# davnords/octic-vits

Measured on AMD Instinct MI355X. Metric: images/sec Hybrid Octic ViT-H/14 224² bf16 train step @1/2/4/8 MI355X, higher is better.
Workload: dtype bf16; 1 GPU; hybrid_deit_huge_patch14 (16 octic + 16 standard blocks, drop_path 0.5) DeiT-III train step: bf16-autocast fwd + bwd + LAMB + EMA, 224x224, batch 64/GPU (BASELINE configs[1]), data parallel over 1 GPU(s); global_batch=64, per_gpu_batch=64, accum_steps=1, parallelism=dp1, library_gemm_table=True, launch=hipGraph replay (whole step)

## Files before the change

### include/octic_hip.h

```cpp
#ifndef OCTIC_HIP_H
#define OCTIC_HIP_H

#include <stdint.h>

#ifdef __cplusplus
extern "C" {
#endif

#define OCTIC_ABI_VERSION 20

enum { OCTIC_F32 = 0, OCTIC_BF16 = 1, OCTIC_U8 = 2  };

enum {
  OCTIC_OK = 0,
  OCTIC_ESHAPE = -1,
  OCTIC_EALIGN = -2,
  OCTIC_EDTYPE = -3,
  OCTIC_ENULL = -4,
  OCTIC_EWORKSPACE = -5
};

typedef struct {
  void* ptr[5];
  int64_t ld[5];
// ... 154 lines not shown
int octic_attn_fwd_packed(const void* qkv, void* o, float* lse, int64_t B, int H, int T, int c, int64_t ld_qkv,
                          int64_t ld_o, float scale, void* stream);
int octic_attn_bwd_packed(const void* qkv, const void* o, const void* dout, const float* lse, float* delta, void* dqkv,
                          int64_t B, int H, int T, int c, int64_t ld_qkv, int64_t ld_o, int64_t ld_g, float scale,
                          int phase, void* stream);

enum {
  OCTIC_ATTN_FWD_PERSIST = 0,
  OCTIC_ATTN_FWD_A80_ONESHOT = 1,
  OCTIC_ATTN_FWD_A80_ONLINE = 2,
  OCTIC_ATTN_FWD_RESIDENT = 3,
  OCTIC_ATTN_FWD_STREAM = 4,
  OCTIC_ATTN_FWD_F32 = 5
};
enum {
  OCTIC_ATTN_BWD_SINGLE = 0,
  OCTIC_ATTN_BWD_PAIR = 1,
  OCTIC_ATTN_BWD_STREAM = 2,
  OCTIC_ATTN_BWD_F32 = 3
};
int octic_attn_plan(int dtype, int T, int hd, int64_t ld_in, int64_t ld_out, int64_t ld_grad, int out[4]);
int octic_attn_skip_plan(int dtype, int T, int hd, int64_t ld_in, int64_t ld_out, int64_t ld_grad, int out[4]);

int octic_attn_fwd_skip(const void* q, const void* k, const void* v, void* o, float* lse, int64_t B, int H, int T, int hd,
                        int64_t sB, int64_t sH, int64_t sT, int64_t oB, int64_t oH, int64_t oT, float scale,
                        const float* sample_scale, void* stream);
int octic_attn_bwd_skip(const void* q, const void* k, const void* v, const void* o, const void* dout, const float* lse,
                        float* delta, void* dq, void* dk, void* dv, int64_t B, int H, int T, int hd, int64_t sB, int64_t sH,
                        int64_t sT, int64_t oB, int64_t oH, int64_t oT, int64_t gB, int64_t gH, int64_t gT, float scale,
                        int phase, const float* sample_scale, void* stream);
int octic_attn_fwd_packed_skip(const void* qkv, void* o, float* lse, int64_t B, int H, int T, int c, int64_t ld_qkv,
                               int64_t ld_o, float scale, const float* sample_scale, void* stream);
int octic_attn_bwd_packed_skip(const void* qkv, const void* o, const void* dout, const float* lse, float* delta, void* dqkv,
                               int64_t B, int H, int T, int c, int64_t ld_qkv, int64_t ld_o, int64_t ld_g, float scale,
                               int phase, const float* sample_scale, void* stream);

int octic_handoff_cat_fwd(const octic_view* x, void* dense, int64_t M, int c, int out_dtype, void* stream);
int octic_handoff_cat_bwd(const float* ddense, const octic_view* dx, int64_t M, int c, void* stream);
int octic_power_spectrum_fwd(const octic_view* x, void* dense, int64_t M, int c, int out_dtype, void* stream);
int octic_power_spectrum_bwd(const float* ddense, const octic_view* x, const octic_view* dx, int64_t M, int c,
                             void* stream);

int octic_im2col_patches(const float* img, void* patches, int64_t B, int Cin, int Himg, int Wimg, int p,
                         int Kpad, int dtype, void* stream);
int octic_lift_gemm(const void* patches, const void* w, const float* bias, const float* pos, float* out,
                    int64_t B, int64_t n_patches, int tok0, int Kpad, int D, int dtype, void* stream);
int64_t octic_lift_wgrad_workspace_bytes(int Kpad, int D, int splits);
int octic_lift_wgrad(const void* patches, const void* dout, float* dw, float* workspace, int splits, int64_t rows,
                     int Kpad, int D, int dtype, void* stream);

int64_t octic_lamb_workspace_floats(int ntensors, int nchunks);
int octic_lamb_step(void* const* p, void* const* g, void* const* m, void* const* v, void* const* ema, const float* wd,
                    const int* chunk_tensor, const int64_t* chunk_off, const int* chunk_len,
                    const int* tensor_chunk_begin, int ntensors, int nchunks, float* workspace, float lr, float beta1,
                    float beta2, float eps, float max_grad_norm, int step, float ema_decay, void* const* bf16_shadow,
                    void* stream);
int octic_adamw_step(void* const* p, void* const* g, void* const* m, void* const* v, void* const* ema, const float* wd,
                     const int* chunk_tensor, const int64_t* chunk_off, const int* chunk_len,
                     const int* tensor_chunk_begin, int ntensors, int nchunks, float* workspace, float lr, float beta1,
                     float beta2, float eps, float max_grad_norm, int step, float ema_decay, void* const* bf16_shadow,
                     void* stream);
int octic_lamb_step_hp(void* const* p, void* const* g, void* const* m, void* const* v, void* const* ema, const float* wd,
                       const int* chunk_tensor, const int64_t* chunk_off, const int* chunk_len,
                       const int* tensor_chunk_begin, int ntensors, int nchunks, float* workspace, const float* lr,
                       float beta1, float beta2, float eps, float max_grad_norm, int step, const float* ema_decay,
                       void* const* bf16_shadow, void* stream);
int octic_adamw_step_hp(void* const* p, void* const* g, void* const* m, void* const* v, void* const* ema, const float* wd,
                        const int* chunk_tensor, const int64_t* chunk_off, const int* chunk_len,
                        const int* tensor_chunk_begin, int ntensors, int nchunks, float* workspace, const float* lr,
                        float beta1, float beta2, float eps, float max_grad_norm, int step, const float* ema_decay,
                        void* const* bf16_shadow, void* stream);

int octic_dense_blocks(int64_t rows);
int octic_dense_resid_layernorm_fwd(const float* x, const void* yb, int yb_dtype, const float* gamma, const float* rs,
                                    int64_t rows_per_scale, float* xout, void* y, int y_dtype, const float* w,
                                    const float* b, float* stats, int64_t rows, int d, float eps, void* stream);
int octic_dense_layernorm_fwd(const float* x, void* y, int y_dtype, const float* w, const float* b, float* stats,
                              int64_t rows, int d, float eps, void* stream);
int octic_dense_layernorm_bwd(const void* gy, int g_dtype, const float* x, const float* w, const float* stats,
                              const float* dres, float* dx, float* partials, int64_t rows, int d, void* stream);
int octic_dense_finish(const float* partials, int nblocks, int d, float* out0, float* out1, const float* scale1,
                       void* stream);
typedef struct octic_finish_job {
  const float* partials;
  float* out0;
  float* out1;
  const float* scale1;
  int nblocks;
  int d;
} octic_finish_job;
int octic_dense_finish_batch(const octic_finish_job* jobs, int njobs, void* stream);
int octic_dense_layernorm_bwd_tail(const void* gy, const float* x, const float* w, const float* stats, const float* dres,
                                   float* dx, float* partials, const void* yb, const float* gamma, const float* rs,
                                   int64_t rows_per_scale, void* gyb, float* partials2, int64_t rows, int d, void* stream);
int octic_dense_layernorm_bwd_tail_skip(const void* gy, const float* x, const float* w, const float* stats,
                                        const float* dres, float* dx, float* partials, const void* yb, const float* gamma,
                                        const float* rs, int64_t rows_per_scale, void* gyb, float* partials2, int64_t rows,
                                        int d, const float* sample_scale, int64_t rows_per_sample, void* stream);
int octic_dense_gelu_blocks(void);
int octic_dense_gelu_bwd(const void* h, const void* g, void* dh, float* partials, int64_t rows, int d, void* stream);
int octic_dense_colsum(const void* g, int64_t rows, int d, int64_t ld, float* partials, void* stream);
int octic_dense_colsum_skip(const void* g, int64_t rows, int d, int64_t ld, float* partials, const float* sample_scale,
                            int64_t rows_per_sample, void* stream);
int octic_swiglu_blocks(void);
int octic_swiglu_fwd(const void* x12, int64_t ld12, void* a, int64_t lda, int64_t rows, int H, void* stream);
int octic_swiglu_bwd(const void* x12, int64_t ld12, const void* ga, int64_t ldg, void* dx12, int64_t ldd, float* partials,
                     int64_t rows, int H, void* stream);
int octic_scale_residual_fwd(const float* x, const void* y, int y_dtype, const float* gamma, const float* rs,
                             int64_t rows_per_scale, float* out, int64_t rows, int d, void* stream);
int octic_scale_residual_bwd(const float* gout, const void* y, int y_dtype, const float* gamma, const float* rs,
                             int64_t rows_per_scale, void* gy, float* partials, int64_t rows, int d, void* stream);

int octic_dense_layernorm_fwd_rows(const float* x, void* y, int y_dtype, const float* w, const float* b, float* stats,
                                   int64_t rows, int d, float eps, const int* rowmap, float* xcopy, void* stream);
int octic_dense_layernorm_bwd_rows(const void* gy, int g_dtype, const float* x, const float* w, const float* stats,
                                   const float* dres, float* dx, float* partials, int64_t rows, int d, const int* rowmap,
                                   void* stream);
int octic_scale_residual_fwd_rows(const float* x, const void* y, int y_dtype, const float* gamma, const float* rs,
                                  int64_t rows_per_scale, float* out, int64_t rows, int d, const int* rowmap, void* stream);
int octic_scale_residual_bwd_rows(const float* gout, const void* y, int y_dtype, const float* gamma, const float* rs,
                                  int64_t rows_per_scale, void* gy, float* partials, int64_t rows, int d, const int* rowmap,
                                  void* stream);

typedef struct octic_dense_prep_item {
  const void* src;
  void* wb;
  void* wt;
  int32_t N, K;
  int32_t block_begin, pad;
} octic_dense_prep_item;
int octic_dense_prep_batch_blocks(int N, int K);
int octic_dense_prep_batch(const octic_dense_prep_item* items_dev, int n_items, int total_blocks, int src_dtype, void* stream);

int64_t octic_dense_gemm_workspace_bytes(int M, int N, int K);
int octic_dense_gemm_colsum_rows(int M, int N, int K);
int octic_dense_gemm_tile(int M, int N, int K, int mode);
int octic_dense_gemm_nt(const void* A, const void* B, int M, int N, int K, int64_t lda, int64_t ldb, int mode, void* C,
                        void* C2, int64_t ldc, const float* bias, const float* gamma, const float* rs,
                        int64_t rows_per_sample, const float* X, float* OUT, const void* H, float* colsum,
                        void* workspace, void* stream);
int octic_dense_gemm_nt_tokens(const void* A, const void* B, int M, int N, int K, int64_t lda, int64_t ldb, int mode, void* C,
                               void* C2, int64_t ldc, const float* bias, const float* gamma, const float* rs,
                               int64_t rows_per_sample, const float* X, float* OUT, const void* H, float* colsum,
                               void* workspace, int tokens, void* stream);
int octic_dense_gemm_plan(int M, int N, int K, int mode, int tokens, int* out4);
int octic_dense_gemm_nt_tokens_skip(const void* A, const void* B, int M, int N, int K, int64_t lda, int64_t ldb, int mode, void* C,
                                    void* C2, int64_t ldc, const float* bias, const float* gamma, const float* rs,
                                    int64_t rows_per_sample_rs, const float* X, float* OUT, const void* H, float* colsum,
                                    const float* sample_scale, int rows_per_sample, void* workspace, int tokens,
                                    void* stream);
int octic_dense_gemm_plan_dropped(int M, int N, int K, int mode, int tokens, int rows_per_sample, int* out4);
int octic_dense_gemm_order_dropped(int M, int N, int K, int mode, int tokens, const float* sample_scale, int rows_per_sample,
                                   int cap, int* out_tm, int* out_tn, int* out_part, int* out_split, int* out_dead);

int64_t octic_dense_wgrad_workspace_bytes(int M, int N, int K);
int octic_dense_wgrad_tile(int M, int N, int K);
int octic_dense_wgrad_plan(int M, int N0, int N1, int K, int64_t ld_max, int out[4]);
int octic_dense_wgrad_tn(const void* dY, const void* X, int M, int N, int K, int64_t ldy, int64_t ldx, float* dW,
                         void* workspace, void* stream);
int64_t octic_dense_wgrad_pair_workspace_bytes(int M, int N0, int N1, int K);
int octic_dense_wgrad_tn_pair(const void* dY0, const void* X0, int N0, int64_t ldy0, int64_t ldx0, float* dW0,
                              const void* dY1, const void* X1, int N1, int64_t ldy1, int64_t ldx1, float* dW1, int M, int K,
                              void* workspace, void* stream);
int octic_dense_wgrad_tn_skip(const void* dY, const void* X, int M, int N, int K, int64_t ldy, int64_t ldx, float* dW,
                              const float* sample_scale, int rows_per_sample, void* workspace, void* stream);
int octic_dense_wgrad_tn_pair_skip(const void* dY0, const void* X0, int N0, int64_t ldy0, int64_t ldx0, float* dW0,
                                   const void* dY1, const void* X1, int N1, int64_t ldy1, int64_t ldx1, float* dW1, int M, int K,
                                   const float* sample_scale, int rows_per_sample, void* workspace, void* stream);

int octic_softmax_center(const void* t, int t_dtype, int64_t ldt, const float* center, float inv_temp, float* out,
                         int64_t rows, int K, void* stream);
int octic_soft_ce_fwd(const void* s, int s_dtype, int64_t lds, const float* tprob, int64_t t_rows, float inv_temp,
                      float* loss, float* lse, float* tsum, int64_t rows, int K, void* stream);
int octic_soft_ce_bwd(const void* s, int s_dtype, int64_t lds, const float* tprob, int64_t t_rows, float inv_temp,
                      const float* g, const float* lse, const float* tsum, void* ds, int64_t ldd, int64_t rows, int K,
                      void* stream);

typedef struct {
  float* w;
  float* b;
  float* mw;
  float* mb;
  int32_t col0;
  int32_t K;
  int32_t lr_index;
  int32_t tile0;
} octic_probe_head;
int octic_probe_features(const void* const* cls, const int64_t* cls_ld, int n, const void* patch, int64_t patch_ld_b,
                         int64_t patch_ld_t, int dtype, int64_t B, int P, int D, float* F, int64_t ldf, void* stream);
int octic_probe_forward(const octic_probe_head* heads, int nheads, const float* F, int64_t ldf, int B, int C, float* logits,
                        void* stream);
int octic_probe_ce(const float* logits, const int64_t* labels, int nheads, int B, int C, float* dlogits, float* rowloss,
                   int* rowrank, float* loss_mean, float* loss_sum, int* topk, void* stream);
int octic_probe_sgd(const octic_probe_head* heads, int nheads, int total_ktiles, const float* F, int64_t ldf,
                    const float* dlogits, int B, int C, const float* lr, float momentum, void* stream);

int octic_seg_ldd(int C);
int octic_seg_slabs(int64_t N, int D, int C);
int64_t octic_seg_workspace_bytes(int64_t N, int D, int C);
int octic_seg_value_dlogits(const float* X, int64_t ldx, int64_t N, int D, const float* W, const float* b, int C,
                            const int32_t* y, float* dlogits, double* value, void* workspace, void* stream);
int octic_seg_predict(const float* X, int64_t ldx, int64_t N, int D, const float* W, const float* b, int C, int32_t* pred,
                      void* stream);
int octic_seg_wgrad(const float* X, int64_t ldx, int64_t N, int D, const float* dlogits, int C, const float* W, double scale,
                    double lambda, float* dW, float* db, void* workspace, void* stream);
int64_t octic_seg_colstats_workspace_bytes(int64_t N, int D);
int octic_seg_colstats(const float* X, int64_t ldx, int64_t N, int D, double* mean, double* var, void* workspace, void* stream);
int octic_seg_standardize(float* X, int64_t ldx, int64_t N, int D, const double* mean, const double* scale, void* stream);
int octic_seg_patch_mode(const void* labels, int esize, int64_t R, int L, int32_t* mode, void* stream);
int octic_seg_confusion(const void* labels, int esize, int64_t R, int L, const int32_t* pred, const uint8_t* ignore,
                        int64_t* counts, void* stream);

int octic_seg_knn_plan(int64_t n, int64_t M, int D, int kmax, int metrics, int* out);
int64_t octic_seg_knn_workspace_bytes(int64_t n, int64_t M, int D, int kmax, int metrics, int splits);
int octic_seg_rownorms(const float* X, int64_t ldx, int64_t N, int D, float* norms, void* stream);
int octic_seg_knn(const float* Q, int64_t ldq, int64_t n, const float* K, int64_t ldk, int64_t M, int D, const float* qnorm,
                  const float* knorm, const uint8_t* skip, int kmax, int metrics, int splits, int32_t* idx_l2, float* dist_l2,
                  int32_t* idx_cos, float* dist_cos, int64_t ldo, void* workspace, void* stream);
int octic_seg_knn_vote(const int32_t* idx, int64_t ldi, int64_t n, const void* labels, int esize, int64_t R, int L, const int* ks,
                       int nk, uint8_t* out, void* stream);

#define OCTIC_KNN_KMAX 256
int octic_knn_topk_plan(int64_t n, int64_t M, int D, int kmax, int* out);
int64_t octic_knn_topk_workspace_bytes(int64_t n, int64_t M, int D, int kmax, int splits);
int octic_knn_topk(const float* Q, int64_t ldq, int64_t n, const float* K, int64_t ldk, int64_t M, int D, int kmax, int splits,
                   int32_t* idx, float* sim, int64_t ldo, void* workspace, void* stream);
int octic_knn_vote(const float* sim, const int32_t* idx, int64_t ldi, int64_t n, int kmax, const int64_t* labels, int64_t M,
                   int C, float inv_T, const int* ks, int nk, float* probas, const int64_t* targets, int64_t* counters,
                   void* stream);

typedef struct {
  int32_t partner;
  float lam;
  int32_t cut;
  int32_t yl, yh;
  int32_t xl, xh;
  int32_t pad;
} octic_mix_row;
int octic_mix_images(const float* src, float* dst, const octic_mix_row* table, int B, int C, int H, int W, void* stream);
int octic_mix_targets(const int64_t* labels, const octic_mix_row* table, int B, int row0, int rows, int num_classes, float on,
                      float off, int binarize, float* targets, void* stream);
int octic_mix_bce(const void* logits, int dtype, int64_t ldl, const int64_t* labels, const octic_mix_row* table, int B, int row0,
                  int rows, int num_classes, float on, float off, int binarize, float* loss, const float* gscale,
                  void* dlogits, int64_t ldd, void* workspace, void* stream);

typedef struct {
  int32_t flip;
  int32_t op;
  int32_t blur_r, blur_ww, blur_fw;
  int32_t order[4];
  float brightness, contrast, saturation;
  int32_t pad[4];
} octic_aug_row;
int64_t octic_augment_workspace_bytes(int B, int H, int W);
int octic_augment_u8(const uint8_t* src, void* dst, int dtype_out, const octic_aug_row* table, float mean0, float mean1,
                     float mean2, float std0, float std1, float std2, int B, int H, int W, void* workspace, void* stream);

typedef struct {
  int64_t src_offset;
  int32_t src_h, src_w;
  int32_t top, left, h, w;
  int32_t flip;
  int32_t hcoef, htaps, vcoef, vtaps;
  int32_t order[4];
  float brightness, contrast, saturation;
  int32_t hue_shift;
  int32_t gray, blur, solarize;
  float blur_w[9];
  int32_t pad[7];
} octic_dino_row;
int octic_dino_resize_coeffs(int n, int S, int taps, int32_t* bounds, int32_t* k);
int octic_dino_resize_max_taps(int S);
int octic_dino_resize_u8(const uint8_t* data, int64_t data_bytes, const octic_dino_row* rows, const int32_t* coef,
                         int64_t coef_len, int N, int S, uint8_t* crops, void* stream);
int64_t octic_dino_color_workspace_bytes(int N, int H, int W);
int octic_dino_color_u8(const uint8_t* crops, void* dst, int dtype_out, const octic_dino_row* rows, float mean0, float mean1,
                        float mean2, float std0, float std1, float std2, int N, int H, int W, void* workspace, void* stream);

#ifdef __cplusplus
}
#endif
#endif
```

### octic_vits_amd/_lib.py

```python
import ctypes
import os
import re

HERE = os.path.dirname(os.path.abspath(__file__))
LIB_PATH = os.environ.get("OCTIC_LIB") or os.path.join(HERE, "liboctic_hip.so")
HEADER_PATH = os.path.join(HERE, "..", "include", "octic_hip.h")

F32, BF16, U8 = 0, 1, 2
ABI_VERSION = 20
(ROUTE_DENSE_TILE, ROUTE_DENSE_SPLIT, ROUTE_WGRAD_SLABS, ROUTE_WGRAD_TILE, ROUTE_LINEAR_RING, ROUTE_RING_EVEN,
 ROUTE_ATTN_LEGACY, ROUTE_ATTN_ONLINE, ROUTE_ATTN_BWD_PAIR, ROUTE_DENSE_IMAGE, ROUTE_DENSE_CLS2, ROUTE_ATTN_STREAM) = range(12)

(ATTN_FWD_PERSIST, ATTN_FWD_A80_ONESHOT, ATTN_FWD_A80_ONLINE, ATTN_FWD_RESIDENT, ATTN_FWD_STREAM, ATTN_FWD_F32) = range(6)
ATTN_BWD_SINGLE, ATTN_BWD_PAIR, ATTN_BWD_STREAM, ATTN_BWD_F32 = range(4)
LINEAR_WREG, LINEAR_RING, LINEAR_CLASSIC = range(3)
WGRAD_RING, WGRAD_TILED = range(2)

c_i64, c_int, c_float, c_void_p = ctypes.c_int64, ctypes.c_int, ctypes.c_float, ctypes.c_void_p
c_double = ctypes.c_double


class OcticView(ctypes.Structure):
    _fields_ = [("ptr", c_void_p * 5), ("ld", c_i64 * 5)]


PtrArray5 = c_void_p * 5
VP = ctypes.POINTER(OcticView)

_PROTOS = {
    "octic_abi_version": (c_int, []),
    "octic_strerror": (ctypes.c_char_p, [c_int]),
    "octic_route_override": (c_int, [c_int, c_int]),
    "octic_gelu_d8_fwd": (c_int, [VP, VP, c_i64, c_int, c_int, c_void_p]),
    "octic_gelu_d8_bwd": (c_int, [VP, VP, VP, c_i64, c_int, c_int, c_void_p]),
    "octic_gelu_d8_fwd_skip": (c_int, [VP, VP, c_i64, c_int, c_int, c_void_p, c_i64, c_void_p]),
    "octic_gelu_d8_bwd_skip": (c_int, [VP, VP, VP, c_i64, c_int, c_int, c_void_p, c_i64, c_void_p]),
    "octic_layernorm_d8_fwd": (c_int, [VP, VP, c_void_p, c_void_p, c_void_p, c_i64, c_int, c_float, c_int, c_void_p]),
    "octic_layernorm_d8_bwd_blocks": (c_int, [c_i64]),
    "octic_layernorm_d8_bwd": (c_int, [VP, VP, c_void_p, c_void_p, VP, VP, c_void_p, c_i64, c_int, c_int, c_void_p]),
    "octic_layernorm_d8_bwd_cast": (c_int, [VP, VP, c_void_p, c_void_p, VP, VP, c_void_p, c_i64, c_int, c_void_p, c_i64,
                                            c_void_p, c_void_p]),
    "octic_layernorm_d8_bwd_skip": (c_int, [VP, VP, c_void_p, c_void_p, VP, VP, c_void_p, c_i64, c_int, c_int, c_void_p, c_i64,
                                            c_void_p]),
    "octic_layernorm_d8_bwd_cast_skip": (c_int, [VP, VP, c_void_p, c_void_p, VP, VP, c_void_p, c_i64, c_int, c_void_p, c_i64,
                                                 c_void_p, c_void_p, c_i64, c_void_p]),
    "octic_layernorm_d8_bwd_finish": (c_int, [c_void_p, c_int, c_int, c_void_p, c_void_p, c_void_p]),
    "octic_layernorm_d8_bwd_finish_batch": (c_int, [c_void_p, c_int, c_void_p]),
    "octic_sample_blocks": (c_int, [c_void_p, c_void_p, c_void_p, c_i64, c_i64, c_int, c_void_p]),
    "octic_linear_d8_fwd": (c_int, [VP, c_void_p, c_void_p, VP, VP, c_void_p, c_i64, c_void_p, c_i64, c_int, c_int,
                                    c_int, c_int, c_void_p]),
    "octic_linear_d8_fwd_skip": (c_int, [VP, c_void_p, c_void_p, VP, VP, c_void_p, c_i64, c_void_p, c_i64, c_int, c_int,
                                         c_int, c_int, c_void_p, c_i64, c_void_p]),
    "octic_linear_d8_fwd_dropped": (c_int, [VP, c_void_p, c_void_p, VP, VP, c_void_p, c_i64, c_void_p, c_i64, c_int, c_int,
                                            c_int, c_int, c_void_p, c_i64, c_void_p]),
    "octic_linear_d8_tile_n": (c_int, [c_i64, c_int, c_int]),
    "octic_linear_d8_plan": (c_int, [c_i64, c_int, c_int, c_int, c_int, c_int, ctypes.POINTER(c_int)]),
    "octic_linear_d8_ring_order": (c_int, [c_void_p, c_void_p, c_void_p, c_int, c_void_p, c_void_p]),
    "octic_linear_d8_ring_order_dropped": (c_int, [c_int, c_void_p, c_void_p, c_int, c_void_p, c_void_p, c_void_p, c_void_p,
                                                   c_void_p, c_void_p]),
    "octic_linear_d8_wgrad_tile": (c_int, [c_i64, c_int, c_int]),
    "octic_linear_d8_wgrad_workspace_bytes": (c_i64, [c_int, c_int, c_int]),
    "octic_linear_d8_wgrad_splits": (c_int, [c_i64, c_int, c_int]),
    "octic_linear_d8_wgrad": (c_int, [VP, VP, c_i64, c_int, c_int, c_int, c_void_p, c_int, c_void_p]),
    "octic_linear_d8_wgrad_finish": (c_int, [c_void_p, c_int, c_int, c_int, c_void_p, c_void_p, c_void_p, c_void_p,
                                             c_void_p, c_void_p, c_void_p, c_void_p]),
    "octic_linear_d8_wgrad_finish_batch": (c_int, [c_void_p, c_int, c_void_p]),
    "octic_linear_d8_wgrad_has_colsum": (c_int, [c_int, c_int, c_int]),
    "octic_linear_d8_wgrad_plan": (c_int, [c_i64, c_int, c_int, c_int, ctypes.POINTER(c_int)]),
    "octic_lamb_workspace_floats": (c_i64, [c_int, c_int]),
    "octic_lamb_step": (c_int, [c_void_p] * 10 + [c_int, c_int, c_void_p, c_float, c_float, c_float, c_float, c_float,
                                                  c_int, c_float, c_void_p, c_void_p]),
    "octic_adamw_step": (c_int, [c_void_p] * 10 + [c_int, c_int, c_void_p, c_float, c_float, c_float, c_float, c_float,
                                                   c_int, c_float, c_void_p, c_void_p]),
    "octic_lamb_step_hp": (c_int, [c_void_p] * 10 + [c_int, c_int, c_void_p, c_void_p, c_float, c_float, c_float, c_float,
                                                     c_int, c_void_p, c_void_p, c_void_p]),
    "octic_adamw_step_hp": (c_int, [c_void_p] * 10 + [c_int, c_int, c_void_p, c_void_p, c_float, c_float, c_float, c_float,
                                                      c_int, c_void_p, c_void_p, c_void_p]),
    "octic_dense_blocks": (c_int, [c_i64]),
    "octic_dense_layernorm_fwd": (c_int, [c_void_p, c_void_p, c_int, c_void_p, c_void_p, c_void_p, c_i64, c_int,
                                          c_float, c_void_p]),
    "octic_dense_resid_layernorm_fwd": (c_int, [c_void_p, c_void_p, c_int, c_void_p, c_void_p, c_i64, c_void_p, c_void_p, c_int,
                                                c_void_p, c_void_p, c_void_p, c_i64, c_int, c_float, c_void_p]),
    "octic_dense_layernorm_bwd": (c_int, [c_void_p, c_int, c_void_p, c_void_p, c_void_p, c_void_p, c_void_p, c_void_p,
                                          c_i64, c_int, c_void_p]),
    "octic_dense_layernorm_bwd_tail": (c_int, [c_void_p] * 10 + [c_i64, c_void_p, c_void_p, c_i64, c_int, c_void_p]),
    "octic_dense_layernorm_bwd_tail_skip": (c_int, [c_void_p] * 10 + [c_i64, c_void_p, c_void_p, c_i64, c_int, c_void_p, c_i64,
                                                                      c_void_p]),
    "octic_dense_finish": (c_int, [c_void_p, c_int, c_int, c_void_p, c_void_p, c_void_p, c_void_p]),
    "octic_dense_finish_batch": (c_int, [c_void_p, c_int, c_void_p]),
    "octic_dense_gelu_blocks": (c_int, []),
    "octic_dense_gelu_bwd": (c_int, [c_void_p, c_void_p, c_void_p, c_void_p, c_i64, c_int, c_void_p]),
    "octic_swiglu_blocks": (c_int, []),
    "octic_swiglu_fwd": (c_int, [c_void_p, c_i64, c_void_p, c_i64, c_i64, c_int, c_void_p]),
    "octic_swiglu_bwd": (c_int, [c_void_p, c_i64, c_void_p, c_i64, c_void_p, c_i64, c_void_p, c_i64, c_int, c_void_p]),
    "octic_dense_layernorm_fwd_rows": (c_int, [c_void_p, c_void_p, c_int, c_void_p, c_void_p, c_void_p, c_i64, c_int, c_float,
                                               c_void_p, c_void_p, c_void_p]),
    "octic_dense_layernorm_bwd_rows": (c_int, [c_void_p, c_int, c_void_p, c_void_p, c_void_p, c_void_p, c_void_p, c_void_p, c_i64,
                                               c_int, c_void_p, c_void_p]),
    "octic_scale_residual_fwd_rows": (c_int, [c_void_p, c_void_p, c_int, c_void_p, c_void_p, c_i64, c_void_p, c_i64, c_int,
                                              c_void_p, c_void_p]),
    "octic_scale_residual_bwd_rows": (c_int, [c_void_p, c_void_p, c_int, c_void_p, c_void_p, c_i64, c_void_p, c_void_p, c_i64,
                                              c_int, c_void_p, c_void_p]),
    "octic_softmax_center": (c_int, [c_void_p, c_int, c_i64, c_void_p, c_float, c_void_p, c_i64, c_int, c_void_p]),
    "octic_soft_ce_fwd": (c_int, [c_void_p, c_int, c_i64, c_void_p, c_i64, c_float, c_void_p, c_void_p, c_void_p, c_i64, c_int,
                                  c_void_p]),
    "octic_soft_ce_bwd": (c_int, [c_void_p, c_int, c_i64, c_void_p, c_i64, c_float, c_void_p, c_void_p, c_void_p, c_void_p, c_i64,
                                  c_i64, c_int, c_void_p]),
    "octic_scale_residual_fwd": (c_int, [c_void_p, c_void_p, c_int, c_void_p, c_void_p, c_i64, c_void_p, c_i64, c_int,
                                         c_void_p]),
    "octic_scale_residual_bwd": (c_int, [c_void_p, c_void_p, c_int, c_void_p, c_void_p, c_i64, c_void_p, c_void_p,
                                         c_i64, c_int, c_void_p]),
    "octic_colsum_blocks": (c_int, [c_i64]),
    "octic_colsum_a1": (c_int, [VP, c_i64, c_int, c_int, c_void_p, c_void_p, c_void_p]),
    "octic_cast_rowscale": (c_int, [VP, VP, c_void_p, c_i64, c_i64, c_int, c_int, c_void_p]),
    "octic_linear_d8_prep": (c_int, [c_void_p, c_void_p, c_int, c_int, c_void_p, c_void_p, c_int, c_void_p]),
    "octic_linear_d8_prep_batch_blocks": (c_int, [c_int, c_int]),
    "octic_linear_d8_prep_batch": (c_int, [c_void_p, c_int, c_int, c_int, c_void_p]),
    "octic_attn_fwd": (c_int, [c_void_p, c_void_p, c_void_p, c_void_p, c_void_p, c_i64, c_int, c_int, c_int,
                               c_i64, c_i64, c_i64, c_i64, c_i64, c_i64, c_float, c_void_p]),
    "octic_attn_fwd_packed": (c_int, [c_void_p] * 3 + [c_i64, c_int, c_int, c_int, c_i64, c_i64, c_float, c_void_p]),
    "octic_attn_bwd_packed": (c_int, [c_void_p] * 6 + [c_i64, c_int, c_int, c_int, c_i64, c_i64, c_i64, c_float, c_int, c_void_p]),
    "octic_attn_bwd": (c_int, [c_void_p] * 10 + [c_i64, c_int, c_int, c_int] + [c_i64] * 9 + [c_float, c_int, c_void_p]),
    "octic_attn_fwd_skip": (c_int, [c_void_p] * 5 + [c_i64, c_int, c_int, c_int] + [c_i64] * 6 + [c_float, c_void_p, c_void_p]),
    "octic_attn_bwd_skip": (c_int, [c_void_p] * 10 + [c_i64, c_int, c_int, c_int] + [c_i64] * 9 + [c_float, c_int, c_void_p, c_void_p]),
    "octic_attn_fwd_packed_skip": (c_int, [c_void_p] * 3 + [c_i64, c_int, c_int, c_int, c_i64, c_i64, c_float, c_void_p, c_void_p]),
    "octic_attn_bwd_packed_skip": (c_int, [c_void_p] * 6 + [c_i64, c_int, c_int, c_int, c_i64, c_i64, c_i64, c_float, c_int, c_void_p, c_void_p]),
    "octic_attn_fwd_f32": (c_int, [c_void_p] * 5 + [c_i64, c_int, c_int, c_int] + [c_i64] * 6 + [c_float, c_void_p]),
    "octic_attn_bwd_f32": (c_int, [c_void_p] * 10 + [c_i64, c_int, c_int, c_int] + [c_i64] * 9 + [c_float, c_int, c_void_p]),
    "octic_attn_plan": (c_int, [c_int, c_int, c_int, c_i64, c_i64, c_i64, ctypes.POINTER(c_int)]),
    "octic_attn_skip_plan": (c_int, [c_int, c_int, c_int, c_i64, c_i64, c_i64, ctypes.POINTER(c_int)]),
    "octic_attn_pack_heads": (c_int, [VP, c_void_p, c_i64, c_i64, c_int, c_int, c_int, c_int, c_void_p]),
    "octic_attn_unpack_heads": (c_int, [c_void_p, VP, c_i64, c_i64, c_int, c_int, c_int, c_int, c_void_p]),
    "octic_handoff_cat_fwd": (c_int, [VP, c_void_p, c_i64, c_int, c_int, c_void_p]),
    "octic_handoff_cat_bwd": (c_int, [c_void_p, VP, c_i64, c_int, c_void_p]),
    "octic_power_spectrum_fwd": (c_int, [VP, c_void_p, c_i64, c_int, c_int, c_void_p]),
    "octic_power_spectrum_bwd": (c_int, [c_void_p, VP, VP, c_i64, c_int, c_void_p]),
    "octic_im2col_patches": (c_int, [c_void_p, c_void_p, c_i64, c_int, c_int, c_int, c_int, c_int, c_int, c_void_p]),
    "octic_lift_gemm": (c_int, [c_void_p, c_void_p, c_void_p, c_void_p, c_void_p, c_i64, c_i64, c_int, c_int, c_int,
                                c_int, c_void_p]),
    "octic_lift_wgrad_workspace_bytes": (c_i64, [c_int, c_int, c_int]),
    "octic_lift_wgrad": (c_int, [c_void_p, c_void_p, c_void_p, c_void_p, c_int, c_i64, c_int, c_int, c_int, c_void_p]),
    "octic_dense_prep_batch_blocks": (c_int, [c_int, c_int]),
    "octic_dense_prep_batch": (c_int, [c_void_p, c_int, c_int, c_int, c_void_p]),
    "octic_dense_gemm_workspace_bytes": (c_i64, [c_int, c_int, c_int]),
    "octic_dense_gemm_colsum_rows": (c_int, [c_int, c_int, c_int]),
    "octic_dense_gemm_tile": (c_int, [c_int, c_int, c_int, c_int]),
    "octic_dense_gemm_nt": (c_int, [c_void_p, c_void_p, c_int, c_int, c_int, c_i64, c_i64, c_int, c_void_p, c_void_p, c_i64,
                                    c_void_p, c_void_p, c_void_p, c_i64, c_void_p, c_void_p, c_void_p, c_void_p, c_void_p,
                                    c_void_p]),
    "octic_dense_gemm_nt_tokens": (c_int, [c_void_p, c_void_p, c_int, c_int, c_int, c_i64, c_i64, c_int, c_void_p, c_void_p,
                                           c_i64, c_void_p, c_void_p, c_void_p, c_i64, c_void_p, c_void_p, c_void_p, c_void_p,
                                           c_void_p, c_int, c_void_p]),
    "octic_dense_gemm_plan": (c_int, [c_int, c_int, c_int, c_int, c_int, ctypes.POINTER(c_int)]),
    "octic_dense_gemm_nt_tokens_skip": (c_int, [c_void_p, c_void_p, c_int, c_int, c_int, c_i64, c_i64, c_int, c_void_p, c_void_p,
                                                c_i64, c_void_p, c_void_p, c_void_p, c_i64, c_void_p, c_void_p, c_void_p, c_void_p,
                                                c_void_p, c_int, c_void_p, c_int, c_void_p]),
    "octic_dense_gemm_plan_dropped": (c_int, [c_int, c_int, c_int, c_int, c_int, c_int, ctypes.POINTER(c_int)]),
    "octic_dense_gemm_order_dropped": (c_int, [c_int, c_int, c_int, c_int, c_int, c_void_p, c_int, c_int, c_void_p, c_void_p,
                                               c_void_p, c_void_p, c_void_p]),
    "octic_dense_colsum": (c_int, [c_void_p, c_i64, c_int, c_i64, c_void_p, c_void_p]),
    "octic_dense_colsum_skip": (c_int, [c_void_p, c_i64, c_int, c_i64, c_void_p, c_void_p, c_i64, c_void_p]),
    "octic_dense_wgrad_workspace_bytes": (c_i64, [c_int, c_int, c_int]),
    "octic_dense_wgrad_tile": (c_int, [c_int, c_int, c_int]),
    "octic_dense_wgrad_plan": (c_int, [c_int, c_int, c_int, c_int, c_i64, ctypes.POINTER(c_int)]),
    "octic_dense_wgrad_tn": (c_int, [c_void_p, c_void_p, c_int, c_int, c_int, c_i64, c_i64, c_void_p, c_void_p, c_void_p]),
    "octic_dense_wgrad_pair_workspace_bytes": (c_i64, [c_int, c_int, c_int, c_int]),
    "octic_dense_wgrad_tn_pair": (c_int, [c_void_p, c_void_p, c_int, c_i64, c_i64, c_void_p, c_void_p, c_void_p, c_int, c_i64, c_i64,
                                          c_void_p, c_int, c_int, c_void_p, c_void_p]),
    "octic_dense_wgrad_tn_skip": (c_int, [c_void_p, c_void_p, c_int, c_int, c_int, c_i64, c_i64, c_void_p, c_void_p, c_int, c_void_p,
                                          c_void_p]),
    "octic_dense_wgrad_tn_pair_skip": (c_int, [c_void_p, c_void_p, c_int, c_i64, c_i64, c_void_p, c_void_p, c_void_p, c_int, c_i64,
                                               c_i64, c_void_p, c_int, c_int, c_void_p, c_int, c_void_p, c_void_p]),
    "octic_probe_features": (c_int, [c_void_p, c_void_p, c_int, c_void_p, c_i64, c_i64, c_int, c_i64, c_int, c_int, c_void_p,
                                     c_i64, c_void_p]),
    "octic_probe_forward": (c_int, [c_void_p, c_int, c_void_p, c_i64, c_int, c_int, c_void_p, c_void_p]),
    "octic_probe_ce": (c_int, [c_void_p, c_void_p, c_int, c_int, c_int, c_void_p, c_void_p, c_void_p, c_void_p, c_void_p,
                               c_void_p, c_void_p]),
    "octic_probe_sgd": (c_int, [c_void_p, c_int, c_int, c_void_p, c_i64, c_void_p, c_int, c_int, c_void_p, c_float, c_void_p]),
    "octic_seg_ldd": (c_int, [c_int]),
    "octic_seg_slabs": (c_int, [c_i64, c_int, c_int]),
    "octic_seg_workspace_bytes": (c_i64, [c_i64, c_int, c_int]),
    "octic_seg_value_dlogits": (c_int, [c_void_p, c_i64, c_i64, c_int, c_void_p, c_void_p, c_int, c_void_p, c_void_p, c_void_p,
                                        c_void_p, c_void_p]),
    "octic_seg_predict": (c_int, [c_void_p, c_i64, c_i64, c_int, c_void_p, c_void_p, c_int, c_void_p, c_void_p]),
    "octic_seg_wgrad": (c_int, [c_void_p, c_i64, c_i64, c_int, c_void_p, c_int, c_void_p, c_double, c_double, c_void_p, c_void_p,
                                c_void_p, c_void_p]),
    "octic_seg_colstats_workspace_bytes": (c_i64, [c_i64, c_int]),
    "octic_seg_colstats": (c_int, [c_void_p, c_i64, c_i64, c_int, c_void_p, c_void_p, c_void_p, c_void_p]),
    "octic_seg_standardize": (c_int, [c_void_p, c_i64, c_i64, c_int, c_void_p, c_void_p, c_void_p]),
    "octic_seg_patch_mode": (c_int, [c_void_p, c_int, c_i64, c_int, c_void_p, c_void_p]),
    "octic_seg_confusion": (c_int, [c_void_p, c_int, c_i64, c_int, c_void_p, c_void_p, c_void_p, c_void_p]),
    "octic_seg_knn_plan": (c_int, [c_i64, c_i64, c_int, c_int, c_int, ctypes.POINTER(c_int)]),
    "octic_seg_knn_workspace_bytes": (c_i64, [c_i64, c_i64, c_int, c_int, c_int, c_int]),
    "octic_seg_rownorms": (c_int, [c_void_p, c_i64, c_i64, c_int, c_void_p, c_void_p]),
    "octic_seg_knn": (c_int, [c_void_p, c_i64, c_i64, c_void_p, c_i64, c_i64, c_int, c_void_p, c_void_p, c_void_p, c_int, c_int,
                              c_int, c_void_p, c_void_p, c_void_p, c_void_p, c_i64, c_void_p, c_void_p]),
    "octic_seg_knn_vote": (c_int, [c_void_p, c_i64, c_i64, c_void_p, c_int, c_i64, c_int, ctypes.POINTER(c_int), c_int, c_void_p,
                                   c_void_p]),
    "octic_knn_topk_plan": (c_int, [c_i64, c_i64, c_int, c_int, ctypes.POINTER(c_int)]),
    "octic_knn_topk_workspace_bytes": (c_i64, [c_i64, c_i64, c_int, c_int, c_int]),
    "octic_knn_topk": (c_int, [c_void_p, c_i64, c_i64, c_void_p, c_i64, c_i64, c_int, c_int, c_int, c_void_p, c_void_p, c_i64,
                               c_void_p, c_void_p]),
    "octic_knn_vote": (c_int, [c_void_p, c_void_p, c_i64, c_i64, c_int, c_void_p, c_i64, c_int, c_float, ctypes.POINTER(c_int),
                               c_int, c_void_p, c_void_p, c_void_p, c_void_p]),
    "octic_mix_images": (c_int, [c_void_p, c_void_p, c_void_p, c_int, c_int, c_int, c_int, c_void_p]),
    "octic_mix_targets": (c_int, [c_void_p, c_void_p, c_int, c_int, c_int, c_int, c_float, c_float, c_int, c_void_p, c_void_p]),
    "octic_mix_bce": (c_int, [c_void_p, c_int, c_i64, c_void_p, c_void_p, c_int, c_int, c_int, c_int, c_float, c_float, c_int,
                              c_void_p, c_void_p, c_void_p, c_i64, c_void_p, c_void_p]),
    "octic_augment_workspace_bytes": (c_i64, [c_int, c_int, c_int]),
    "octic_augment_u8": (c_int, [c_void_p, c_void_p, c_int, c_void_p] + [c_float] * 6 + [c_int, c_int, c_int, c_void_p, c_void_p]),
    "octic_dino_resize_coeffs": (c_int, [c_int, c_int, c_int, c_void_p, c_void_p]),
    "octic_dino_resize_max_taps": (c_int, [c_int]),
    "octic_dino_resize_u8": (c_int, [c_void_p, c_i64, c_void_p, c_void_p, c_i64, c_int, c_int, c_void_p, c_void_p]),
    "octic_dino_color_workspace_bytes": (c_i64, [c_int, c_int, c_int]),
    "octic_dino_color_u8": (c_int, [c_void_p, c_void_p, c_int, c_void_p] + [c_float] * 6 + [c_int, c_int, c_int, c_void_p, c_void_p]),
}


def header_symbols():
    with open(HEADER_PATH) as f:
        text = re.sub(r"/\*.*?\*/", "", f.read(), flags=re.S)
    return sorted(set(re.findall(r"\b(octic_[a-z0-9_]+)\s*\(", text)))


_LIB = None


def lib():
    global _LIB
    if _LIB is None:
        if not os.path.exists(LIB_PATH):
            raise RuntimeError(
                f"octic_vits_amd: HIP library {LIB_PATH} is missing. Build it with "
                "`python -m octic_vits_amd.build` (hipcc, --offload-arch=gfx950). There is no CPU fallback.")
        L = ctypes.CDLL(LIB_PATH)
        for name, (res, args) in _PROTOS.items():
            fn = getattr(L, name)
            fn.restype, fn.argtypes = res, args
        if L.octic_abi_version() != ABI_VERSION:
            raise RuntimeError("octic_vits_amd: ABI version mismatch between _lib.py and liboctic_hip.so")
        _LIB = L
    return _LIB


def route_override(knob: int, value: int) -> int:
    old = lib().octic_route_override(knob, value)
    if old < 0:
        raise ValueError(f"octic_route_override: unknown knob {knob}")
    _PLANS.clear()
    for drop in _ON_OVERRIDE:
        drop()
    return old


_ON_OVERRIDE = []


def on_route_override(drop):
    if drop not in _ON_OVERRIDE:
        _ON_OVERRIDE.append(drop)
    return drop


_PLANS = {}


def plan(query, *args):
    key = (query, args)
    answer = _PLANS.get(key, 0)
    if answer == 0:
        out = (c_int * 4)()
        code = getattr(lib(), query)(*args, out)
        if code not in (0, -1):
            check(code)
        _PLANS[key] = answer = tuple(out) if code == 0 else None
    return answer


def attn_plan(T, hd, dtype=BF16, ld_in=0, ld_out=0, ld_grad=0):
    answer = plan("octic_attn_plan", dtype, T, hd, ld_in, ld_out, ld_grad)
    if answer is None:
        check(-1)
    return answer


def check(code: int):
    if code != 0:
        raise RuntimeError(f"octic HIP call failed ({code}): {lib().octic_strerror(code).decode()}")
```

### octic_vits_amd/csrc/dense_gemm.hip

```cpp
#include <cmath>
#include <type_traits>
#include "octic_common.hpp"

namespace octic {

constexpr int DG_BM = 256, DG_BK = 64;
constexpr int DG_UNIT = 128 * 128;
constexpr int DG_SLOTS = 8;
constexpr int DG_D = 6;
static_assert(DG_D >= 4 && DG_D <= DG_SLOTS - 2, "prefetch distance");
template <int NT> struct DgGeom {
  static constexpr int NA = NT - 2;
  static constexpr int BN = 64 * NT;
  static constexpr int WCOLS = 16 * NT;
  static constexpr int U1 = NA * 8192;
  static constexpr int KT = 3 * DG_UNIT + U1;
  static constexpr int RING = 2 * KT;
  static constexpr int SRS = WCOLS * 2 + 16;
  static constexpr int EPI_PASSES = NT == 4 ? 1 : 2;
  static constexpr int EPI_ROWS = 128 / EPI_PASSES;
  static constexpr int EPI = 8 * EPI_ROWS * SRS;
  static constexpr int LDS = RING > EPI ? RING : EPI;
  static constexpr int INFLIGHT = 2 * (DG_D - 2) + (NA - 2);
  static_assert(DG_D == 6 || NT == 4, "unequal units: the steady vmcnt assumes the 4 youngest units are one of each kind");
  __host__ __device__ static constexpr int unit_off(int kind) { return kind == 0 ? 0 : kind == 1 ? DG_UNIT : kind == 2 ? DG_UNIT + U1 : 2 * DG_UNIT + U1; }
  __host__ __device__ static constexpr int unit_instr(int kind) { return kind == 1 ? NA : 2; }
};

struct DgArgs {
  const bf16* A;
  const bf16* B;
  int64_t lda, ldb;
  int M, N, K;
  bf16* C;
  bf16* C2;
  int64_t ldc;
  const float* bias;
  const float* gamma;
  const float* rs;
  int64_t rps;
  const float* X;
  float* OUT;
  const bf16* H;
  float* colsum;
  int m_stride, m_base;
  int tiles_m, tiles_n;
  int full_tiles;
  int split;
  int tail_pad;
  float* slabs;
  int* tickets;
  const float* sample_scale;
  int rows_per_sample;
};

enum DgMode { DG_PLAIN = 0, DG_GELU = 1, DG_RESID = 2, DG_DGELU = 3,
              DG_GELUF = 4,
              DG_DFACT = 5,
              DG_GELUO = 6 };

constexpr int kDgMaskCap = 1024;
constexpr int kDgMaskWords = kDgMaskCap / 64;

__host__ __device__ inline bool dg_panel_live(const float* scale, int rps, int M, int m_stride, int m_base, int tm) {
  const int m0 = tm * m_stride + m_base;
  if (m0 >= M) return false;
  const int m1 = (m0 + DG_BM < M ? m0 + DG_BM : M) - 1;
  const int b1 = m1 / rps;
  for (int b = m0 / rps; b <= b1; ++b)
    if (scale[b] != 0.0f) return true;
  return false;
}
__host__ __device__ inline int dg_group_bits(const unsigned long long* bm, int g, int gsz, bool live) {
  int b = (int)((bm[g >> 3] >> ((g & 7) * 8)) & 0xffull);
  if (!live) b = ~b;
  return b & ((1 << gsz) - 1);
}
__host__ __device__ inline int dg_group_count(int bits, int gsz, int tiles_n, int cut) {
  if (cut == gsz * tiles_n) return tiles_n * __builtin_popcount(bits);
  const int cols = cut / gsz, rest = cut - cols * gsz;
  return cols * __builtin_popcount(bits) + __builtin_popcount(bits & ((1 << rest) - 1));
}
__host__ __device__ inline int dg_live_full(const unsigned long long* bm, int tiles_m, int tiles_n, int full) {
  const int per_group = 8 * tiles_n;
  int L = 0;
  for (int g = 0; g * per_group < full; ++g) {
    const int gsz = tiles_m - 8 * g < 8 ? tiles_m - 8 * g : 8;
    const int left = full - g * per_group, cut = left < gsz * tiles_n ? left : gsz * tiles_n;
    L += dg_group_count(dg_group_bits(bm, g, gsz, true), gsz, tiles_n, cut);
  }
  return L;
}
__host__ __device__ inline int dg_select_full(const unsigned long long* bm, int tiles_m, int tiles_n, int full, int k, bool live) {
  const int per_group = 8 * tiles_n;
  for (int g = 0; g * per_group < full; ++g) {
    const int gsz = tiles_m - 8 * g < 8 ? tiles_m - 8 * g : 8;
    const int left = full - g * per_group, cut = left < gsz * tiles_n ? left : gsz * tiles_n;
    int bits = dg_group_bits(bm, g, gsz, live);
    const int cnt = dg_group_count(bits, gsz, tiles_n, cut);
    if (k < cnt) {
      const int lg = __builtin_popcount(bits);
      const int col = k / lg;
      int idx = k - col * lg, pos = 0;
      for (; pos < 8; ++pos) {
        if (bits & 1) {
          if (idx == 0) break;
          --idx;
        }
        bits >>= 1;
      }
      return g * per_group + col * gsz + pos;
    }
    k -= cnt;
  }
  return 0;
}
__host__ __device__ inline void dg_tile_panel(int tiles_m, int tiles_n, int tile, int& tm, int& tn) {
  const int per_group = 8 * tiles_n, gidx = tile / per_group, first_m = gidx * 8;
  const int gsz = (tiles_m - first_m) < 8 ? (tiles_m - first_m) : 8;
  const int in_g = tile - gidx * per_group;
  tm = first_m + in_g % gsz;
  tn = in_g / gsz;
}
__host__ __device__ inline void dense_item_masked(int tiles_m, int tiles_n, int full, int split, int tail_pad, int bid,
                                                  const unsigned long long* bm, int& tile, int& rem_idx, int& part, bool& dead) {
  tile = -1; rem_idx = -1; part = 0; dead = false;
  if (bid < tail_pad) {
    if (bid >= (tiles_m * tiles_n - full) * split) return;
    rem_idx = bid / split;
    part = bid - rem_idx * split;
    tile = full + rem_idx;
    int tm, tn;
    dg_tile_panel(tiles_m, tiles_n, tile, tm, tn);
    dead = ((bm[tm >> 6] >> (tm & 63)) & 1ull) == 0;
    return;
  }
  const int j = bid - tail_pad;
  const int L = dg_live_full(bm, tiles_m, tiles_n, full), D = full - L;
  if (j < D) {
    tile = dg_select_full(bm, tiles_m, tiles_n, full, j, false);
    dead = true;
    return;
  }
  const int i = j - D, x = i & 7, q8 = L >> 3, r8 = L & 7;
  const int rank = (x < r8 ? x * (q8 + 1) : r8 * (q8 + 1) + (x - r8) * q8) + (i >> 3);
  tile = dg_select_full(bm, tiles_m, tiles_n, full, rank, true);
}

__device__ inline void dg_wait_vmcnt(int n) {
  switch (n) {
    case 2: asm volatile("s_waitcnt vmcnt(2)" ::: "memory"); break;
    case 4: asm volatile("s_waitcnt vmcnt(4)" ::: "memory"); break;
    case 6: asm volatile("s_waitcnt vmcnt(6)" ::: "memory"); break;
    case 8: asm volatile("s_waitcnt vmcnt(8)" ::: "memory"); break;
    case 10: asm volatile("s_waitcnt vmcnt(10)" ::: "memory"); break;
    case 12: asm volatile("s_waitcnt vmcnt(12)" ::: "memory"); break;
    case 14: asm volatile("s_waitcnt vmcnt(14)" ::: "memory"); break;
    case 16: asm volatile("s_waitcnt vmcnt(16)" ::: "memory"); break;
    case 3: asm volatile("s_waitcnt vmcnt(3)" ::: "memory"); break;
    case 5: asm volatile("s_waitcnt vmcnt(5)" ::: "memory"); break;
    case 7: asm volatile("s_waitcnt vmcnt(7)" ::: "memory"); break;
    case 9: asm volatile("s_waitcnt vmcnt(9)" ::: "memory"); break;
    default: asm volatile("s_waitcnt vmcnt(0)" ::: "memory"); break;
  }
}

#ifdef DG_TRACE
__device__ unsigned long long g_dg_trace[8 * 256];
extern "C" void* octic_dbg_dense_trace(void) {
  void* p = nullptr;
  (void)hipGetSymbolAddress(&p, HIP_SYMBOL(g_dg_trace));
  return p;
}
#define DGT()                                                                                        \
  do {                                                                                               \
    if (blockIdx.x == 0 && lane == 0 && dgt_i < 256) g_dg_trace[wid * 256 + dgt_i++] = __builtin_readcyclecounter(); \
    if (blockIdx.x == 0 && lane == 0 && dgt_i == 200) g_dg_trace[wid * 256 + 255] = __builtin_amdgcn_s_memrealtime(); \
  } while (0)
#else
#define DGT() do {} while (0)
#endif
#ifdef DG_TRACE2
__device__ unsigned long long g_dg_trace2[4096 * 8];
extern "C" void* octic_dbg_dense_trace2(void) {
  void* p = nullptr;
  (void)hipGetSymbolAddress(&p, HIP_SYMBOL(g_dg_trace2));
  return p;
}
#define DGT2(slot)                                                                                            \
  do {                                                                                                        \
    if (wid == 0 && lane == 0 && blockIdx.x < 4096) g_dg_trace2[blockIdx.x * 8 + (slot)] = __builtin_amdgcn_s_memrealtime(); \
  } while (0)
#else
#define DGT2(slot) do {} while (0)
#endif

__device__ inline float dg_erf(float x) {
  const float ax = fabsf(x);
  const float t = __builtin_amdgcn_rcpf(1.0f + 0.3275911f * ax);
  const float poly = t * (0.254829592f + t * (-0.284496736f + t * (1.421413741f + t * (-1.453152027f + t * 1.061405429f))));
  const float r = 1.0f - poly * __expf(-ax * ax);
  return copysignf(r, x);
}
__device__ inline float dg_gelu(float x) { return 0.5f * x * (1.0f + dg_erf(x * kSqrt1Over2)); }
__device__ inline float dg_gelu_grad(float x) {
  return 0.5f * (1.0f + dg_erf(x * kSqrt1Over2)) + x * kInvSqrt2Pi * __expf(-0.5f * x * x);
}
__device__ inline void dg_gelu_both(float x, float& g, float& d) {
  const float ax = fabsf(x) * kSqrt1Over2;
  const float t = __builtin_amdgcn_rcpf(1.0f + 0.3275911f * ax);
  const float poly = t * (0.254829592f + t * (-0.284496736f + t * (1.421413741f + t * (-1.453152027f + t * 1.061405429f))));
  const float e = __expf(-ax * ax);
  const float phi = 0.5f * (1.0f + copysignf(1.0f - poly * e, x));
  g = x * phi;
  d = phi + x * kInvSqrt2Pi * e;
}

template <int N>
__device__ inline void dg_wait_imm() {
  if constexpr (N == 8) asm volatile("s_waitcnt vmcnt(8)" ::: "memory");
  else if constexpr (N == 10) asm volatile("s_waitcnt vmcnt(10)" ::: "memory");
  else if constexpr (N == 12) asm volatile("s_waitcnt vmcnt(12)" ::: "memory");
  else if constexpr (N == 14) asm volatile("s_waitcnt vmcnt(14)" ::: "memory");
  else if constexpr (N == 16) asm volatile("s_waitcnt vmcnt(16)" ::: "memory");
  else if constexpr (N == 6) asm volatile("s_waitcnt vmcnt(6)" ::: "memory");
  else if constexpr (N == 9) asm volatile("s_waitcnt vmcnt(9)" ::: "memory");
  else asm volatile("s_waitcnt vmcnt(0)" ::: "memory");
}

template <int MODE, int NT, bool SKIP = false>
__global__ __launch_bounds__(512, 1) void dense_nt_kernel(DgArgs a) {
  extern __shared__ __attribute__((aligned(16))) char lds[];
  using GE = DgGeom<NT>;
  constexpr int NA = GE::NA, DG_BN = GE::BN;
  static_assert(NT == 4 || MODE == DG_PLAIN, "the fused tails exist for the 256-wide tile only");
  static_assert(!SKIP || MODE != DG_RESID, "the fused residual tail never takes a mask");

  const int lane = threadIdx.x & 63;
  const int wid = __builtin_amdgcn_readfirstlane(threadIdx.x >> 6);
  const int wr = wid >> 2, wc = wid & 3;
  const bool hi = wr != 0;
  const int fr = lane & 15, kg = lane >> 4;
#ifdef DG_TRACE
  int dgt_i = 0;
  if (blockIdx.x == 0 && lane == 0) g_dg_trace[wid * 256 + 254] = __builtin_amdgcn_s_memrealtime();
#endif
  DGT();
  DGT2(0);
#ifdef DG_TRACE2
  if (wid == 0 && lane == 0 && blockIdx.x < 4096) {
    unsigned xcc, hwid;
    asm volatile("s_getreg_b32 %0, hwreg(HW_REG_XCC_ID)" : "=s"(xcc));
    asm volatile("s_getreg_b32 %0, hwreg(HW_REG_HW_ID)" : "=s"(hwid));
    g_dg_trace2[blockIdx.x * 8 + 7] = ((unsigned long long)hwid << 32) | xcc;
  }
#endif

  const int bid = blockIdx.x;
  int tile, kt_begin, kt_end, part = 0, rem_idx = -1;
  const int nkt_all = a.K / DG_BK;
  bool dead_item = false;
  if constexpr (SKIP) {
    unsigned long long* const live_bm = (unsigned long long*)(lds + GE::LDS);
    const int words = (a.tiles_m + 63) >> 6;
    for (int w = wid; w < words; w += 8) {
      const int p = w * 64 + lane;
      const bool live = p < a.tiles_m && dg_panel_live(a.sample_scale, a.rows_per_sample, a.M, a.m_stride, a.m_base, p);
      const unsigned long long m = __ballot(live);
      if (lane == 0) live_bm[w] = m;
    }
    __syncthreads();
    dense_item_masked(a.tiles_m, a.tiles_n, a.full_tiles, a.split, a.tail_pad, bid, live_bm, tile, rem_idx, part, dead_item);
    tile = __builtin_amdgcn_readfirstlane(tile);
    rem_idx = __builtin_amdgcn_readfirstlane(rem_idx);
    part = __builtin_amdgcn_readfirstlane(part);
    dead_item = __builtin_amdgcn_readfirstlane((int)dead_item) != 0;
    if (tile < 0) return;
    kt_begin = rem_idx >= 0 ? (int)(((int64_t)nkt_all * part) / a.split) : 0;
    kt_end = rem_idx >= 0 ? (int)(((int64_t)nkt_all * (part + 1)) / a.split) : nkt_all;
  } else
  if (bid >= a.tail_pad) {
    const int j = bid - a.tail_pad;
    const int nf = a.full_tiles;
    const int xcd = j & 7, q8 = nf >> 3, r8 = nf & 7;
    tile = (xcd < r8 ? xcd * (q8 + 1) : r8 * (q8 + 1) + (xcd - r8) * q8) + (j >> 3);
    kt_begin = 0;
    kt_end = nkt_all;
  } else {
    const int r = bid;
    if (r >= (a.tiles_m * a.tiles_n - a.full_tiles) * a.split) return;
    rem_idx = r / a.split;
    part = r - rem_idx * a.split;
    tile = a.full_tiles + rem_idx;
    kt_begin = (int)(((int64_t)nkt_all * part) / a.split);
    kt_end = (int)(((int64_t)nkt_all * (part + 1)) / a.split);
  }
  int tm, tn;
  {
    const int G = 8;
    const int per_group = G * a.tiles_n;
    const int gidx = tile / per_group;
    const int first_m = gidx * G;
    const int gsz = (a.tiles_m - first_m) < G ? (a.tiles_m - first_m) : G;
    const int in_g = tile - gidx * per_group;
    tm = first_m + in_g % gsz;
    tn = in_g / gsz;
  }
  const int m0 = tm * a.m_stride + a.m_base, n0 = tn * DG_BN;
  if constexpr (SKIP) {
    if (dead_item) {
      if (part != 0) return;
      constexpr int CPR = DG_BN / 8;
      const u32x4 z = {0, 0, 0, 0};
#pragma unroll 4
      for (int p = threadIdx.x; p < DG_BM * CPR; p += 512) {
        const int r = p / CPR, c = p - r * CPR;
        const int m = m0 + r, n = n0 + c * 8;
        if (m < a.M && n < a.N) {
          *(u32x4*)(a.C + (int64_t)m * a.ldc + n) = z;
          if (MODE == DG_GELU || MODE == DG_GELUF) *(u32x4*)(a.C2 + (int64_t)m * a.ldc + n) = z;
        }
      }
      if ((MODE == DG_DGELU || MODE == DG_DFACT) && a.colsum != nullptr) {
        const int t = threadIdx.x;
        const int row = t / (DG_BN / 4), n = n0 + (t - row * (DG_BN / 4)) * 4;
        if (row < 2 && n < a.N) *(f32x4*)(a.colsum + (int64_t)(tm * 2 + row) * a.N + n) = f32x4{0, 0, 0, 0};
      }
      return;
    }
  }
  const int nkt = kt_end - kt_begin;
  const int nunits = 4 * nkt;

  const int drow = lane >> 3;
  const int dch = (lane & 7) ^ drow;
  const __amdgpu_buffer_rsrc_t rsA = __builtin_amdgcn_make_buffer_rsrc((void*)a.A, 0, (int)((int64_t)a.M * a.lda * 2), 0x27000);
  const __amdgpu_buffer_rsrc_t rsB = __builtin_amdgcn_make_buffer_rsrc((void*)a.B, 0, (int)((int64_t)a.N * a.ldb * 2), 0x27000);
  const int r0 = 16 * wid + drow;
  const int am0 = m0, an0 = n0;
  const unsigned voA = (unsigned)(((int64_t)(am0 + (r0 >> 6) * 128 + (r0 & 63)) * a.lda + dch * 8) * 2);
  const int rb1 = 8 * NA * wid + drow;
  const unsigned voB1 = (unsigned)(((int64_t)(an0 + (rb1 / (16 * NA)) * GE::WCOLS + (rb1 % (16 * NA))) * a.ldb + dch * 8) * 2);
  const unsigned voB2 = (unsigned)(((int64_t)(an0 + (r0 >> 5) * GE::WCOLS + 16 * NA + (r0 & 31)) * a.ldb + dch * 8) * 2);
  const int rowA8 = (int)(a.lda * 16), rowB8 = (int)(a.ldb * 16);
  const int halfA = (int)(a.lda * 128);
  const int kbase = kt_begin * (DG_BK * 2);

  int u_issue = 0;
  auto issue_unit = [&](auto kind_c) {
    constexpr int KIND = decltype(kind_c)::value;
    constexpr bool isA = KIND == 0 || KIND == 3;
    char* dst = lds + ((u_issue >> 2) & 1) * GE::KT + GE::unit_off(KIND) + wid * (GE::unit_instr(KIND) * 1024);
    const int so = kbase + (u_issue >> 2) * (DG_BK * 2) + (KIND == 3 ? halfA : 0);
    if constexpr (isA) {
      __builtin_amdgcn_raw_ptr_buffer_load_lds(rsA, (__attribute__((address_space(3))) void*)dst, 16, voA, so, 0, 0);
      __builtin_amdgcn_raw_ptr_buffer_load_lds(rsA, (__attribute__((address_space(3))) void*)(dst + 1024), 16, voA, so + rowA8, 0, 0);
    } else if constexpr (KIND == 1) {
      __builtin_amdgcn_raw_ptr_buffer_load_lds(rsB, (__attribute__((address_space(3))) void*)dst, 16, voB1, so, 0, 0);
      __builtin_amdgcn_raw_ptr_buffer_load_lds(rsB, (__attribute__((address_space(3))) void*)(dst + 1024), 16, voB1, so + rowB8, 0, 0);
      if constexpr (NA == 3)
        __builtin_amdgcn_raw_ptr_buffer_load_lds(rsB, (__attribute__((address_space(3))) void*)(dst + 2048), 16, voB1, so + 2 * rowB8, 0, 0);
    } else {
      __builtin_amdgcn_raw_ptr_buffer_load_lds(rsB, (__attribute__((address_space(3))) void*)dst, 16, voB2, so, 0, 0);
      __builtin_amdgcn_raw_ptr_buffer_load_lds(rsB, (__attribute__((address_space(3))) void*)(dst + 1024), 16, voB2, so + rowB8, 0, 0);
    }
    ++u_issue;
  };
  auto young_instr = [&](int n) {
    const int k1 = ((u_issue + 2) >> 2) - ((u_issue - n + 2) >> 2);
    return 2 * n + (NA - 2) * k1;
  };
#define DG_IC(v) std::integral_constant<int, v>()

  const int sw = lane & 7;
  const int rdo0 = fr * 128 + ((kg ^ sw) << 4);
  const int rdo1 = fr * 128 + (((4 + kg) ^ sw) << 4);
  const int a_row0 = wr * 64;

  bf16x8 Af[1][2][4];
  bf16x8 Bf0[2][NA], Bf1[2][2];
  f32x4 acc0[2][4][NA], acc1[2][4][2];
#pragma unroll
  for (int i = 0; i < 2; ++i)
#pragma unroll
    for (int p = 0; p < 4; ++p) {
#pragma unroll
      for (int q = 0; q < NA; ++q) acc0[i][p][q] = f32x4{0, 0, 0, 0};
#pragma unroll
      for (int q = 0; q < 2; ++q) acc1[i][p][q] = f32x4{0, 0, 0, 0};
    }
  int rt_hi = (a.M - m0 - wr * 128 + 15) >> 4;
  rt_hi = rt_hi < 0 ? 0 : (rt_hi > 8 ? 8 : rt_hi);
  const int live_mask = __builtin_amdgcn_readfirstlane((rt_hi > 0 ? 1 : 0) | (rt_hi > 4 ? 2 : 0));

  auto readA = [&](int mh, int unit) {
    const char* base = lds + ((unit >> 2) & 1) * GE::KT + GE::unit_off(mh ? 3 : 0) + a_row0 * 128;
#pragma unroll
    for (int mi = 0; mi < 4; ++mi) {
      Af[0][0][mi] = *(const bf16x8*)(base + mi * 2048 + rdo0);
      Af[0][1][mi] = *(const bf16x8*)(base + mi * 2048 + rdo1);
    }
  };
  auto readB = [&](int nh, int unit) {
    if (nh == 0) {
      const char* base = lds + ((unit >> 2) & 1) * GE::KT + GE::unit_off(1) + wc * (16 * NA) * 128;
#pragma unroll
      for (int ni = 0; ni < NA; ++ni) {
        Bf0[0][ni] = *(const bf16x8*)(base + ni * 2048 + rdo0);
        Bf0[1][ni] = *(const bf16x8*)(base + ni * 2048 + rdo1);
      }
    } else {
      const char* base = lds + ((unit >> 2) & 1) * GE::KT + GE::unit_off(2) + wc * 32 * 128;
#pragma unroll
      for (int ni = 0; ni < 2; ++ni) {
        Bf1[0][ni] = *(const bf16x8*)(base + ni * 2048 + rdo0);
        Bf1[1][ni] = *(const bf16x8*)(base + ni * 2048 + rdo1);
      }
    }
  };
  auto mma = [&](int mh, int nh, auto kind_c) {
    asm volatile("s_waitcnt lgkmcnt(0)" ::: "memory");
    __builtin_amdgcn_sched_barrier(0);
    if (live_mask & (mh ? 2 : 1)) {
#pragma unroll
    for (int ks = 0; ks < 2; ++ks) {
#pragma unroll
      for (int mi = 0; mi < 4; ++mi) {
        if (nh == 0) {
#pragma unroll
          for (int ni = 0; ni < NA; ++ni)
            acc0[mh][mi][ni] = __builtin_amdgcn_mfma_f32_16x16x32_bf16(Bf0[ks][ni], Af[0][ks][mi], acc0[mh][mi][ni], 0, 0, 0);
        } else {
#pragma unroll
          for (int ni = 0; ni < 2; ++ni)
            acc1[mh][mi][ni] = __builtin_amdgcn_mfma_f32_16x16x32_bf16(Bf1[ks][ni], Af[0][ks][mi], acc1[mh][mi][ni], 0, 0, 0);
        }
      }
    }
    }
    __builtin_amdgcn_sched_barrier(0);
  };

  int g = 0;
  auto wait_landed = [&]() {
    int need = g + 2;
    need = need < nunits - 1 ? need : nunits - 1;
    const int ok = (u_issue - 1) - need;
    if (ok == DG_D - 2) dg_wait_imm<GE::INFLIGHT>();
    else dg_wait_vmcnt(ok > 0 ? young_instr(ok) : 0);
  };

#define DG_PRO(i) if constexpr ((i) < DG_D) { if (u_issue < nunits) issue_unit(DG_IC((i) & 3)); }
  DG_PRO(0) DG_PRO(1) DG_PRO(2) DG_PRO(3) DG_PRO(4) DG_PRO(5) DG_PRO(6) DG_PRO(7) DG_PRO(8) DG_PRO(9)
#undef DG_PRO
  {
    const int ok = (u_issue - 1) - 1;
    dg_wait_vmcnt(ok > 0 ? young_instr(ok) : 0);
  }
  if (hi) __builtin_amdgcn_s_barrier();
  DGT2(1);

  auto ktile = [&](int t, auto steady_c) {
    constexpr bool STEADY = decltype(steady_c)::value != 0;
    const int u0 = 4 * t;
    auto dma = [&](auto kind_c) {
      if (STEADY || u_issue < nunits) issue_unit(kind_c);
    };
    auto landed = [&]() {
      if constexpr (STEADY) dg_wait_imm<GE::INFLIGHT>();
      else wait_landed();
    };
#define DG_RP(x) do { __builtin_amdgcn_s_setprio(x); } while (0)
#define DG_R(q, reads) do { DG_RP(2); dma(DG_IC(((q) + DG_D) & 3)); reads; DG_RP(0); } while (0)
    __builtin_amdgcn_s_barrier();
    DGT();
    DG_R(0, readA(0, u0); readB(0, u0 + 1));
    if (hi) landed();
    DGT();
    __builtin_amdgcn_s_barrier();
    DGT();
    mma(0, 0, DG_IC((0 + DG_D) & 3));
    DGT();
    if (!hi) landed();
    ++g;
    __builtin_amdgcn_s_barrier();
    DGT();
    DG_R(1, readB(1, u0 + 2));
    if (hi) landed();
    DGT();
    __builtin_amdgcn_s_barrier();
    DGT();
    mma(0, 1, DG_IC((1 + DG_D) & 3));
    DGT();
    if (!hi) landed();
    ++g;
    __builtin_amdgcn_s_barrier();
    DGT();
    DG_R(2, readA(1, u0 + 3));
    if (hi) landed();
    DGT();
    __builtin_amdgcn_s_barrier();
    DGT();
    mma(1, 1, DG_IC((2 + DG_D) & 3));
    DGT();
    if (!hi) landed();
    ++g;
    __builtin_amdgcn_s_barrier();
    DGT();
    DG_R(3, (void)0);
    if (hi) landed();
    DGT();
    __builtin_amdgcn_s_barrier();
    DGT();
    mma(1, 0, DG_IC((3 + DG_D) & 3));
    DGT();
    if (!hi) landed();
    ++g;
#undef DG_R
#undef DG_RP
  };
  const int t_steady = (nunits - 4 - DG_D) >= 0 ? (nunits - 4 - DG_D) / 4 + 1 : 0;
  int t = 0;
#pragma unroll 1
  for (; t < t_steady; ++t) ktile(t, DG_IC(1));
#pragma unroll 1
  for (; t < nkt; ++t) ktile(t, DG_IC(0));
  if (!hi) __builtin_amdgcn_s_barrier();
  __builtin_amdgcn_s_barrier();
  DGT2(2);

  const int rt_lo = 0;
  auto ACC = [&](int mh, int mi, int j) -> f32x4& { return j < NA ? acc0[mh][mi][j] : acc1[mh][mi][j - NA]; };
  if (rem_idx >= 0 && a.split > 1) {
    float* slab = a.slabs + ((int64_t)rem_idx * a.split + part) * (DG_BM * DG_BN);
    f32x4* sw4 = (f32x4*)slab + (int64_t)wid * (8 * NT) * 64 + lane;
#pragma unroll
    for (int mh = 0; mh < 2; ++mh)
#pragma unroll
      for (int mi = 0; mi < 4; ++mi) {
        if (mh * 4 + mi >= rt_hi) continue;
#pragma unroll
        for (int j = 0; j < NT; ++j) sw4[((mh * 4 + mi) * NT + j) * 64] = ACC(mh, mi, j);
      }
    asm volatile("s_waitcnt vmcnt(0)" ::: "memory");
    __syncthreads();
    DGT2(5);
    int* flag = (int*)lds;
    if (threadIdx.x == 0) {
      __builtin_amdgcn_fence(__ATOMIC_RELEASE, "agent");
      asm volatile("s_waitcnt vmcnt(0)" ::: "memory");
      const int old = __hip_atomic_fetch_add(a.tickets + rem_idx, 1, __ATOMIC_RELAXED, __HIP_MEMORY_SCOPE_AGENT);
      flag[0] = (old == a.split - 1) ? 1 : 0;
      if (old == a.split - 1) {
        __builtin_amdgcn_fence(__ATOMIC_ACQUIRE, "agent");
        asm volatile("s_waitcnt vmcnt(0)" ::: "memory");
        __hip_atomic_store(a.tickets + rem_idx, 0, __ATOMIC_RELAXED, __HIP_MEMORY_SCOPE_AGENT);
      }
    }
    __syncthreads();
    const int last = flag[0];
    __syncthreads();
    if (last == 0) return;
    DGT2(6);
    for (int p = 0; p < a.split; ++p) {
      const f32x4* o4 = (const f32x4*)(a.slabs + ((int64_t)rem_idx * a.split + p) * (DG_BM * DG_BN)) +
                        (int64_t)wid * (8 * NT) * 64 + lane;
#pragma unroll
      for (int mh = 0; mh < 2; ++mh)
#pragma unroll
        for (int mi = 0; mi < 4; ++mi) {
          if (mh * 4 + mi >= rt_hi) continue;
#pragma unroll
          for (int j = 0; j < NT; ++j) {
            const f32x4 o = o4[((mh * 4 + mi) * NT + j) * 64];
            ACC(mh, mi, j) = p == 0 ? o : ACC(mh, mi, j) + o;
          }
        }
    }
  }

  if constexpr (NT != 4) {
    constexpr int SRS = GE::SRS;
    char* const stg = lds + wid * (GE::EPI_ROWS * SRS);
    const int er = lane / 10, ech = lane - er * 10;
    const int n = n0 + wc * GE::WCOLS + ech * 8;
    const bool nok = n < a.N && lane < 60;
#pragma unroll
    for (int mh = 0; mh < 2; ++mh) {
      if (mh * 4 >= rt_hi) break;
#pragma unroll
      for (int j = 0; j < NT; ++j) {
        const int nl = j * 16 + kg * 4;
        const int nb = n0 + wc * GE::WCOLS + nl;
        f32x4 bv = {0, 0, 0, 0};
        if (a.bias && nb < a.N) bv = *(const f32x4*)(a.bias + nb);
#pragma unroll
        for (int mi = 0; mi < 4; ++mi) {
          if (mh * 4 + mi >= rt_hi) continue;
          const f32x4 v = ACC(mh, mi, j) + bv;
          const bf16x4 cb = {(bf16)v[0], (bf16)v[1], (bf16)v[2], (bf16)v[3]};
          *(bf16x4*)(stg + (mi * 16 + fr) * SRS + nl * 2) = cb;
        }
      }
      asm volatile("s_waitcnt lgkmcnt(0)" ::: "memory");
#pragma unroll
      for (int it = 0; it < 11; ++it) {
        const int row = it * 6 + er;
        const int m = m0 + wr * 128 + mh * 64 + row;
        if (row >= 64 || m >= a.M || !nok || mh * 4 + (row >> 4) >= rt_hi) continue;
        const u32x4 raw = *(const u32x4*)(stg + row * SRS + ech * 16);
        *(u32x4*)(a.C + (int64_t)m * a.ldc + n) = raw;
      }
    }
  } else {
  constexpr int SRS = GE::SRS;
  char* const stg = lds + wid * (128 * SRS);
#pragma unroll
  for (int j = 0; j < NT; ++j) {
      const int nl = j * 16 + kg * 4;
      const int n = n0 + wc * 64 + nl;
      f32x4 bv = {0, 0, 0, 0};
      if (a.bias && n < a.N) bv = *(const f32x4*)(a.bias + n);
#pragma unroll
      for (int mh = 0; mh < 2; ++mh)
#pragma unroll
        for (int mi = 0; mi < 4; ++mi) {
          if (mh * 4 + mi < rt_lo || mh * 4 + mi >= rt_hi) continue;
          const f32x4 v = ACC(mh, mi, j) + bv;
          const bf16x4 cb = {(bf16)v[0], (bf16)v[1], (bf16)v[2], (bf16)v[3]};
          *(bf16x4*)(stg + (mh * 64 + mi * 16 + fr) * SRS + nl * 2) = cb;
        }
    }
  asm volatile("s_waitcnt lgkmcnt(0)" ::: "memory");
  const int srow = lane >> 3, sch = lane & 7;
  const int n = n0 + wc * 64 + sch * 8;
  const bool nok = n < a.N;
  f32x4 gm0 = {1, 1, 1, 1}, gm1 = {1, 1, 1, 1};
  if (MODE == DG_RESID && a.gamma && nok) {
    gm0 = *(const f32x4*)(a.gamma + n);
    gm1 = *(const f32x4*)(a.gamma + n + 4);
  }
  f32x4 xin[MODE == DG_RESID ? 16 : 1][2];
  bf16x8 hin[(MODE == DG_DGELU || MODE == DG_DFACT) ? 16 : 1];
  float csum[8] = {0, 0, 0, 0, 0, 0, 0, 0};
  if (MODE == DG_RESID || MODE == DG_DGELU || MODE == DG_DFACT) {
#pragma unroll
    for (int it = 0; it < 16; ++it) {
      const int m = m0 + wr * 128 + it * 8 + srow;
      const bool ok = m < a.M && nok && (it >> 1) >= rt_lo && (it >> 1) < rt_hi;
      if (MODE == DG_RESID) {
        const float* xp = a.X + (int64_t)(ok ? m : 0) * a.N + (ok ? n : 0);
        xin[it][0] = *(const f32x4*)xp;
        xin[it][1] = *(const f32x4*)(xp + 4);
      } else {
        hin[it] = *(const bf16x8*)(a.H + (int64_t)(ok ? m : 0) * a.ldc + (ok ? n : 0));
      }
    }
  }
#pragma unroll
  for (int it = 0; it < 16; ++it) {
    const int row = it * 8 + srow;
    const int m = m0 + wr * 128 + row;
    if (m >= a.M || !nok || (it >> 1) < rt_lo || (it >> 1) >= rt_hi) continue;
    const u32x4 raw = *(const u32x4*)(stg + row * SRS + sch * 16);
    const bf16x8 cb = __builtin_bit_cast(bf16x8, raw);
    bf16* cp = a.C + (int64_t)m * a.ldc + n;
    if (MODE == DG_PLAIN) {
      *(u32x4*)cp = raw;
    } else if (MODE == DG_GELU) {
      *(u32x4*)cp = raw;
      bf16x8 y;
#pragma unroll
      for (int e = 0; e < 8; ++e) y[e] = (bf16)dg_gelu((float)cb[e]);
      *(bf16x8*)(a.C2 + (int64_t)m * a.ldc + n) = y;
    } else if (MODE == DG_GELUO) {
      bf16x8 y;
#pragma unroll
      for (int e = 0; e < 8; ++e) y[e] = (bf16)dg_gelu((float)cb[e]);
      *(bf16x8*)cp = y;
    } else if (MODE == DG_GELUF) {
      bf16x8 y, f;
#pragma unroll
      for (int e = 0; e < 8; ++e) {
        float gv, dv;
        dg_gelu_both((float)cb[e], gv, dv);
        y[e] = (bf16)gv;
        f[e] = (bf16)dv;
      }
      *(bf16x8*)cp = f;
      *(bf16x8*)(a.C2 + (int64_t)m * a.ldc + n) = y;
    } else if (MODE == DG_RESID) {
      *(u32x4*)cp = raw;
      const float rsv = a.rs ? a.rs[m / a.rps] : 1.0f;
      f32x4 x0 = xin[it][0], x1 = xin[it][1];
#pragma unroll
      for (int e = 0; e < 4; ++e) {
        x0[e] += rsv * gm0[e] * (float)cb[e];
        x1[e] += rsv * gm1[e] * (float)cb[4 + e];
      }
      float* op = a.OUT + (int64_t)m * a.N + n;
      *(f32x4*)op = x0;
      *(f32x4*)(op + 4) = x1;
    } else {
      const bf16x8 h = hin[it];
      bf16x8 d;
#pragma unroll
      for (int e = 0; e < 8; ++e) {
        d[e] = (bf16)((MODE == DG_DFACT ? (float)h[e] : dg_gelu_grad((float)h[e])) * (float)cb[e]);
        csum[e] += (float)d[e];
      }
      *(bf16x8*)cp = d;
    }
  }
  if ((MODE == DG_DGELU || MODE == DG_DFACT) && a.colsum != nullptr) {
#pragma unroll
    for (int e = 0; e < 8; ++e) {
      float v = csum[e];
      v += __shfl_xor(v, 8, 64);
      v += __shfl_xor(v, 16, 64);
      v += __shfl_xor(v, 32, 64);
      csum[e] = v;
    }
    if (srow == 0 && nok) {
      float* base = a.colsum + (int64_t)(tm * 2 + wr) * a.N + n;
      *(f32x4*)base = f32x4{csum[0], csum[1], csum[2], csum[3]};
      *(f32x4*)(base + 4) = f32x4{csum[4], csum[5], csum[6], csum[7]};
    }
  }
  }
#ifdef DG_TRACE2
  DGT2(3);
  asm volatile("s_waitcnt vmcnt(0)" ::: "memory");
  DGT2(4);
#endif
}

template <int MODE>
__global__ __launch_bounds__(1024) void dense_cls_kernel(DgArgs a, int tokens, int nrows, int colsum_row0) {
  __shared__ f32x4 part[16][64];
  const int lane = threadIdx.x & 63;
  const int wid = __builtin_amdgcn_readfirstlane(threadIdx.x >> 6);
  const int nw = blockDim.x >> 6;
  const int fr = lane & 15, kg = lane >> 4;
  const int ntn = a.N >> 4;
  const int tn = blockIdx.x % ntn, tb = blockIdx.x / ntn;
  const int n0 = tn * 16, b0 = tb * 16;
  const int kw = a.K / nw;
  const int nks = kw >> 5;
  int brow = b0 + fr;
  const bool rok = brow < nrows;
  brow = rok ? brow : nrows - 1;
  const bf16* wp = a.B + (int64_t)(n0 + fr) * a.ldb + wid * kw + kg * 8;
  const bf16* xp = a.A + (int64_t)brow * tokens * a.lda + wid * kw + kg * 8;
  const int n = n0 + 4 * kg;
  const int64_t m = (int64_t)(b0 + fr) * tokens;
  f32x4 bv = {0, 0, 0, 0};
  bf16x4 hv = {0, 0, 0, 0};
  if (wid == 0) {
    if (a.bias) bv = *(const f32x4*)(a.bias + n);
    if ((MODE == DG_DGELU || MODE == DG_DFACT) && rok) hv = *(const bf16x4*)(a.H + m * a.ldc + n);
  }
  f32x4 acc = {0, 0, 0, 0};
  constexpr int U = 10;
  bf16x8 wf[U], xf[U];
#pragma unroll 1
  for (int ks0 = 0; ks0 < nks; ks0 += U) {
#pragma unroll
    for (int j = 0; j < U; ++j)
      if (ks0 + j < nks) {
        wf[j] = *(const bf16x8*)(wp + (ks0 + j) * 32);
        xf[j] = *(const bf16x8*)(xp + (ks0 + j) * 32);
      }
#pragma unroll
    for (int j = 0; j < U; ++j)
      if (ks0 + j < nks) acc = __builtin_amdgcn_mfma_f32_16x16x32_bf16(wf[j], xf[j], acc, 0, 0, 0);
  }
  part[wid][lane] = acc;
  __syncthreads();
  if (wid != 0) return;
  f32x4 v = part[0][lane];
  for (int w = 1; w < nw; ++w) v = v + part[w][lane];
  v = v + bv;
  const bf16x4 cb = {(bf16)v[0], (bf16)v[1], (bf16)v[2], (bf16)v[3]};
  bf16* cp = a.C + m * a.ldc + n;
  float cs[4] = {0, 0, 0, 0};
  if (rok) {
    if (MODE == DG_PLAIN) {
      *(bf16x4*)cp = cb;
    } else if (MODE == DG_GELU || MODE == DG_GELUO || MODE == DG_GELUF) {
      bf16x4 y, f;
#pragma unroll
      for (int e = 0; e < 4; ++e) {
        float gv, dv;
        if (MODE == DG_GELUF) dg_gelu_both((float)cb[e], gv, dv);
        else { gv = dg_gelu((float)cb[e]); dv = 0.0f; }
        y[e] = (bf16)gv;
        f[e] = (bf16)dv;
      }
      if (MODE == DG_GELUO) *(bf16x4*)cp = y;
      else {
        *(bf16x4*)cp = MODE == DG_GELUF ? f : cb;
        *(bf16x4*)(a.C2 + m * a.ldc + n) = y;
      }
    } else if (MODE == DG_DGELU || MODE == DG_DFACT) {
      const bf16x4 h = hv;
      bf16x4 d;
#pragma unroll
      for (int e = 0; e < 4; ++e) {
        d[e] = (bf16)((MODE == DG_DFACT ? (float)h[e] : dg_gelu_grad((float)h[e])) * (float)cb[e]);
        cs[e] = (float)d[e];
      }
      *(bf16x4*)cp = d;
    }
  }
  if ((MODE == DG_DGELU || MODE == DG_DFACT) && a.colsum != nullptr) {
#pragma unroll
    for (int e = 0; e < 4; ++e) {
      float t = cs[e];
      t += __shfl_xor(t, 1, 64);
      t += __shfl_xor(t, 2, 64);
      t += __shfl_xor(t, 4, 64);
      t += __shfl_xor(t, 8, 64);
      cs[e] = t;
    }
    if (fr == 0) *(f32x4*)(a.colsum + (int64_t)(colsum_row0 + tb) * a.N + n) = f32x4{cs[0], cs[1], cs[2], cs[3]};
  }
}


constexpr int CLS_KSLICE = 320;
__global__ __launch_bounds__(320) void dense_cls_part_kernel(DgArgs a, int tokens, int nrows, int rows_pad, float* part) {
  const int lane = threadIdx.x & 63;
  const int wid = __builtin_amdgcn_readfirstlane(threadIdx.x >> 6);
  const int fr = lane & 15, kg = lane >> 4;
  const int bw = (blockDim.x >> 6) * 16;
  const int nnb = a.N / bw, nks = a.K / CLS_KSLICE;
  const int nb = blockIdx.x % nnb, ks = (blockIdx.x / nnb) % nks, rb = blockIdx.x / (nnb * nks);
  const int n0 = nb * bw + wid * 16;
  const bf16* wp = a.B + (int64_t)(n0 + fr) * a.ldb + ks * CLS_KSLICE + kg * 8;
  const bf16* xp[4];
#pragma unroll
  for (int i = 0; i < 4; ++i) {
    int r = rb * 64 + i * 16 + fr;
    r = r < nrows ? r : nrows - 1;
    xp[i] = a.A + (int64_t)r * tokens * a.lda + ks * CLS_KSLICE + kg * 8;
  }
  constexpr int U = CLS_KSLICE / 32;
  bf16x8 wf[U], xf[4][U];
#pragma unroll
  for (int j = 0; j < U; ++j) {
    wf[j] = *(const bf16x8*)(wp + j * 32);
#pragma unroll
    for (int i = 0; i < 4; ++i) xf[i][j] = *(const bf16x8*)(xp[i] + j * 32);
  }
  f32x4 acc[4] = {{0, 0, 0, 0}, {0, 0, 0, 0}, {0, 0, 0, 0}, {0, 0, 0, 0}};
#pragma unroll
  for (int j = 0; j < U; ++j)
#pragma unroll
    for (int i = 0; i < 4; ++i) acc[i] = __builtin_amdgcn_mfma_f32_16x16x32_bf16(wf[j], xf[i][j], acc[i], 0, 0, 0);
#pragma unroll
  for (int i = 0; i < 4; ++i) {
    const int r = rb * 64 + i * 16 + fr;
    *(f32x4*)(part + ((int64_t)ks * rows_pad + r) * a.N + n0 + 4 * kg) = acc[i];
  }
}

__global__ __launch_bounds__(256) void dense_cls_sum_kernel(DgArgs a, int tokens, int nrows, int rows_pad, const float* part) {
  const int n4 = a.N >> 2;
  const int idx = blockIdx.x * 256 + threadIdx.x;
  const int r = idx / n4, n = (idx - r * n4) * 4;
  if (r >= nrows) return;
  const int nks = a.K / CLS_KSLICE;
  f32x4 v = *(const f32x4*)(part + (int64_t)r * a.N + n);
  for (int ks = 1; ks < nks; ++ks) v = v + *(const f32x4*)(part + ((int64_t)ks * rows_pad + r) * a.N + n);
  if (a.bias) v = v + *(const f32x4*)(a.bias + n);
  *(bf16x4*)(a.C + (int64_t)r * tokens * a.ldc + n) = bf16x4{(bf16)v[0], (bf16)v[1], (bf16)v[2], (bf16)v[3]};
}

struct DgPlan { int nt, tiles_m, tiles_n, full, rem, split, tail_pad, grid; double cost; };

inline DgPlan dense_plan_nt(int M, int N, int K, int cus, int nt, int force_split = 0, bool front_unsplit = false) {
  DgPlan p;
  const int bn = 64 * nt;
  const double wf = nt / 4.0;
  p.nt = nt;
  p.tiles_m = (M + DG_BM - 1) / DG_BM;
  p.tiles_n = (N + bn - 1) / bn;
  const int tiles = p.tiles_m * p.tiles_n;
  const int rounds = tiles / cus;
  const int nkt = K / DG_BK;
  p.full = rounds * cus;
  p.rem = tiles - p.full;
  p.split = 1;
  double f = 1.0;
  if (p.rem > 0) {
    int s = cus / p.rem;
    const int smax = nkt / 4 > 0 ? nkt / 4 : 1;
    s = s < 1 ? 1 : (s > smax ? smax : s);
    s = s > 8 ? 8 : s;
    if (p.rem * 10 >= cus * 8) s = 1;
    {
      int64_t rows = 0;
      for (int tile = p.full; tile < tiles; ++tile) {
        const int G = 8, per_group = G * p.tiles_n, gidx = tile / per_group, first_m = gidx * G;
        const int gsz = (p.tiles_m - first_m) < G ? (p.tiles_m - first_m) : G;
        const int tm = first_m + (tile - gidx * per_group) % gsz;
        const int left = M - tm * DG_BM;
        rows += left < DG_BM ? left : DG_BM;
      }
      f = (double)rows / ((double)p.rem * DG_BM);
    }
    if (s > 1 && (double)nkt / s + 17.0 * f * wf + 1.0 >= (double)nkt) s = 1;
    if (force_split > 0) s = force_split > smax ? smax : force_split;
    p.split = s;
    if (s == 1 && !(front_unsplit && f < 0.5 && rounds >= 1)) {
      p.full = tiles;
      p.rem = 0;
    }
  }
  p.tail_pad = (p.rem * p.split + 7) & ~7;
  p.grid = p.tail_pad + p.full;
  const double tile_cost = nkt * wf + 3.0;
  p.cost = (double)((p.full + cus - 1) / cus) * tile_cost;
  if (p.rem > 0) {
    const double kt = (f < 0.5 ? 0.5 : 1.0) * wf;
    p.cost += (double)nkt / p.split * kt + 17.0 * f * wf + 3.0;
  }
  return p;
}

constexpr int DG_TICKET_BYTES = 8192;

static inline int dense_force_nt() { const int v = route(OCTIC_ROUTE_DENSE_TILE); return (v == 4 || v == 5) ? v : 0; }
static inline int dense_force_split() { const int v = route(OCTIC_ROUTE_DENSE_SPLIT); return v > 0 ? v : 0; }

inline DgPlan dense_plan(int M, int N, int K, int cus, int mode) {
  const DgPlan p4 = dense_plan_nt(M, N, K, cus, 4, dense_force_split(), dense_force_split() == 1);
  if (mode != DG_PLAIN || (N % 320) != 0 || dense_force_nt() == 4) return p4;
  const DgPlan p5 = dense_plan_nt(M, N, K, cus, 5, dense_force_split(), dense_force_split() == 1);
  if (dense_force_nt() == 5) return p5;
  return p5.cost < p4.cost ? p5 : p4;
}

inline int dense_cls_waves(int K) {
  if (K % 320 == 0 && K / 320 <= 16) return K / 320;
  for (int w = 16; w > 1; --w)
    if (K % (32 * w) == 0) return w;
  return 1;
}

struct DgTokPlan { DgPlan p; bool image; int images; };
#ifndef DG_CLS2_US
#define DG_CLS2_US 15.0
#endif
inline bool dense_cls_two_launches(int mode, int N, int K) {
  const int v = route(OCTIC_ROUTE_DENSE_CLS2);
  const bool legal = mode == DG_PLAIN && (K % CLS_KSLICE) == 0 && (N % 64) == 0;
  return legal && v != 1 && (v == 2 || K >= 3840);
}
inline double dense_cls_cost(int B, int N, int K, int mode) {
  double us = 7.0 * sqrt((double)N / 1280.0) * pow((double)K / 1280.0, 0.8);
  if (dense_cls_two_launches(mode, N, K)) us = DG_CLS2_US;
  return us * (B <= 64 ? 1.0 : (double)B / 64.0) / 1.54;
}
inline DgTokPlan dense_plan_tokens(int M, int N, int K, int cus, int mode, int tokens) {
  DgTokPlan t;
  t.p = dense_plan(M, N, K, cus, mode);
  t.image = false;
  t.images = 0;
  const int force = route(OCTIC_ROUTE_DENSE_IMAGE);
  if (tokens != 257 || M % tokens != 0 || mode == DG_RESID || (K % 128) != 0 || (N % 16) != 0 || force == 2) return t;
  const int B = M / tokens;
  const DgPlan pi = dense_plan(B * DG_BM, N, K, cus, mode);
  const double margin = 1.0;
  const bool pays = mode != DG_DGELU && mode != DG_DFACT && pi.cost + dense_cls_cost(B, N, K, mode) + margin < t.p.cost;
  if (force == 1 || (force == 0 && pays) || (force == 3 && pays && mode == DG_PLAIN)) {
    t.p = pi;
    t.image = true;
    t.images = B;
  }
  return t;
}

}

using namespace octic;

extern "C" {

static int dense_cus() { return device_cus(); }

int64_t octic_dense_gemm_workspace_bytes(int M, int N, int K) {
  int64_t need = 256;
  if ((M % 257) == 0 && (K % CLS_KSLICE) == 0) {
    const int64_t rows_pad = ((int64_t)(M / 257) + 63) / 64 * 64;
    need = DG_TICKET_BYTES + (int64_t)(K / CLS_KSLICE) * rows_pad * N * 4 + 256;
  }
  const int Ms[2] = {M, (M % 257) == 0 ? M / 257 * DG_BM : 0};
  for (int i = 0; i < 2; ++i) {
    if (Ms[i] <= 0) continue;
    for (int nt = 4; nt <= 5; ++nt) {
      if (nt == 5 && (N % 320) != 0) continue;
      DgPlan p = dense_plan_nt(Ms[i], N, K, dense_cus(), nt);
      if (dense_force_split() > 1) p = dense_plan_nt(Ms[i], N, K, dense_cus(), nt, 8);
      if (p.split <= 1) continue;
      const int64_t b = (int64_t)p.rem * p.split * DG_BM * (64 * nt) * 4 + DG_TICKET_BYTES + 256;
      need = b > need ? b : need;
    }
  }
  return need;
}

int octic_dense_gemm_plan(int M, int N, int K, int mode, int tokens, int* out) {
  if (!out) return OCTIC_ENULL;
  if (M <= 0 || N <= 0 || K < 2 * DG_BK) { out[0] = 256; out[1] = 0; out[2] = 0; out[3] = 0; return OCTIC_OK; }
  const DgTokPlan t = dense_plan_tokens(M, N, K, dense_cus(), mode, tokens);
  out[0] = t.p.nt == 5 ? 320 : 256;
  out[1] = t.image ? 2 * t.images + (t.images + 15) / 16 : 2 * ((M + DG_BM - 1) / DG_BM);
  out[2] = t.image ? 1 : 0;
  out[3] = t.p.grid;
  return OCTIC_OK;
}

int octic_dense_gemm_tile(int M, int N, int K, int mode) {
  if (M <= 0 || N <= 0 || K < 2 * DG_BK) return 256;
  return dense_plan(M, N, K, dense_cus(), mode).nt == 5 ? 320 : 256;
}

int octic_dense_gemm_colsum_rows(int M, int N, int K) {
  (void)N; (void)K;
  return 2 * ((M + DG_BM - 1) / DG_BM);
}

int octic_dense_gemm_nt_tokens_skip(const void* A, const void* B, int M, int N, int K, int64_t lda, int64_t ldb, int mode, void* C,
                                    void* C2, int64_t ldc, const float* bias, const float* gamma, const float* rs, int64_t rps,
                                    const float* X, float* OUT, const void* H, float* colsum, const float* sample_scale,
                                    int rows_per_sample, void* workspace, int tokens, void* stream) {
  if (!A || !B || !C) return OCTIC_ENULL;
  if (sample_scale && (rows_per_sample <= 0 || M <= 0 || (M % rows_per_sample) != 0)) return OCTIC_ESHAPE;
  if (sample_scale && (((uintptr_t)sample_scale) & 3)) return OCTIC_EALIGN;
  if (M <= 0 || N <= 0 || K <= 0 || (K % DG_BK) || K < 2 * DG_BK || (N % 8) || (lda % 8) || (ldb % 8) || (ldc % 8)) return OCTIC_ESHAPE;
  if ((int64_t)M * lda * 2 >= (1ll << 31) || (int64_t)N * ldb * 2 >= (1ll << 31)) return OCTIC_ESHAPE;
  if ((((uintptr_t)A) | ((uintptr_t)B)) & 15) return OCTIC_EALIGN;
  if ((mode == DG_GELU || mode == DG_GELUF) && !C2) return OCTIC_ENULL;
  if (mode == DG_RESID && (!X || !OUT || (rs && rps <= 0))) return OCTIC_ENULL;
  if ((mode == DG_DGELU || mode == DG_DFACT) && !H) return OCTIC_ENULL;
  DgArgs a = {};
  a.A = (const bf16*)A; a.B = (const bf16*)B; a.lda = lda; a.ldb = ldb; a.M = M; a.N = N; a.K = K;
  a.C = (bf16*)C; a.C2 = (bf16*)C2; a.ldc = ldc; a.bias = bias; a.gamma = gamma; a.rs = rs; a.rps = rs ? rps : 1;
  a.X = X; a.OUT = OUT; a.H = (const bf16*)H; a.colsum = (mode == DG_DGELU || mode == DG_DFACT) ? colsum : nullptr;
  const DgTokPlan tp = dense_plan_tokens(M, N, K, dense_cus(), mode, tokens);
  const DgPlan p = tp.p;
  a.tiles_m = p.tiles_m; a.tiles_n = p.tiles_n; a.full_tiles = p.full; a.split = p.split; a.tail_pad = p.tail_pad;
  a.m_stride = tp.image ? tokens : DG_BM;
  a.m_base = tp.image ? 1 : 0;
  const bool skip = sample_scale != nullptr && mode != DG_RESID && p.tiles_m <= kDgMaskCap;
  a.sample_scale = skip ? sample_scale : nullptr;
  a.rows_per_sample = skip ? rows_per_sample : 0;
  hipStream_t s = (hipStream_t)stream;
  if (p.split > 1) {
    if (!workspace) return OCTIC_ENULL;
    if (p.rem * 4 > DG_TICKET_BYTES) return OCTIC_ESHAPE;
    a.tickets = (int*)workspace;
    a.slabs = (float*)((char*)workspace + DG_TICKET_BYTES);
  }
  const int smem = DgGeom<4>::LDS, smem5 = DgGeom<5>::LDS, bmb = kDgMaskWords * 8;
  static DeviceOnce once;
  if (once.first()) {
    (void)hipFuncSetAttribute((const void*)dense_nt_kernel<DG_PLAIN, 4>, hipFuncAttributeMaxDynamicSharedMemorySize, smem);
    (void)hipFuncSetAttribute((const void*)dense_nt_kernel<DG_PLAIN, 5>, hipFuncAttributeMaxDynamicSharedMemorySize, smem5);
    (void)hipFuncSetAttribute((const void*)dense_nt_kernel<DG_GELU, 4>, hipFuncAttributeMaxDynamicSharedMemorySize, smem);
    (void)hipFuncSetAttribute((const void*)dense_nt_kernel<DG_RESID, 4>, hipFuncAttributeMaxDynamicSharedMemorySize, smem);
    (void)hipFuncSetAttribute((const void*)dense_nt_kernel<DG_DGELU, 4>, hipFuncAttributeMaxDynamicSharedMemorySize, smem);
    (void)hipFuncSetAttribute((const void*)dense_nt_kernel<DG_GELUF, 4>, hipFuncAttributeMaxDynamicSharedMemorySize, smem);
    (void)hipFuncSetAttribute((const void*)dense_nt_kernel<DG_DFACT, 4>, hipFuncAttributeMaxDynamicSharedMemorySize, smem);
    (void)hipFuncSetAttribute((const void*)dense_nt_kernel<DG_GELUO, 4>, hipFuncAttributeMaxDynamicSharedMemorySize, smem);
    (void)hipFuncSetAttribute((const void*)dense_nt_kernel<DG_PLAIN, 4, true>, hipFuncAttributeMaxDynamicSharedMemorySize, smem + bmb);
    (void)hipFuncSetAttribute((const void*)dense_nt_kernel<DG_PLAIN, 5, true>, hipFuncAttributeMaxDynamicSharedMemorySize, smem5 + bmb);
    (void)hipFuncSetAttribute((const void*)dense_nt_kernel<DG_GELU, 4, true>, hipFuncAttributeMaxDynamicSharedMemorySize, smem + bmb);
    (void)hipFuncSetAttribute((const void*)dense_nt_kernel<DG_DGELU, 4, true>, hipFuncAttributeMaxDynamicSharedMemorySize, smem + bmb);
    (void)hipFuncSetAttribute((const void*)dense_nt_kernel<DG_GELUF, 4, true>, hipFuncAttributeMaxDynamicSharedMemorySize, smem + bmb);
    (void)hipFuncSetAttribute((const void*)dense_nt_kernel<DG_DFACT, 4, true>, hipFuncAttributeMaxDynamicSharedMemorySize, smem + bmb);
    (void)hipFuncSetAttribute((const void*)dense_nt_kernel<DG_GELUO, 4, true>, hipFuncAttributeMaxDynamicSharedMemorySize, smem + bmb);
    (void)hipGetLastError();
  }
  if (skip) {
    switch (mode) {
      case DG_PLAIN:
        if (p.nt == 5) dense_nt_kernel<DG_PLAIN, 5, true><<<p.grid, 512, smem5 + bmb, s>>>(a);
        else dense_nt_kernel<DG_PLAIN, 4, true><<<p.grid, 512, smem + bmb, s>>>(a);
        break;
      case DG_GELU: dense_nt_kernel<DG_GELU, 4, true><<<p.grid, 512, smem + bmb, s>>>(a); break;
      case DG_DGELU: dense_nt_kernel<DG_DGELU, 4, true><<<p.grid, 512, smem + bmb, s>>>(a); break;
      case DG_GELUF: dense_nt_kernel<DG_GELUF, 4, true><<<p.grid, 512, smem + bmb, s>>>(a); break;
      case DG_DFACT: dense_nt_kernel<DG_DFACT, 4, true><<<p.grid, 512, smem + bmb, s>>>(a); break;
      case DG_GELUO: dense_nt_kernel<DG_GELUO, 4, true><<<p.grid, 512, smem + bmb, s>>>(a); break;
      default: return OCTIC_ESHAPE;
    }
  } else
  switch (mode) {
    case DG_PLAIN:
      if (p.nt == 5) dense_nt_kernel<DG_PLAIN, 5><<<p.grid, 512, smem5, s>>>(a);
      else dense_nt_kernel<DG_PLAIN, 4><<<p.grid, 512, smem, s>>>(a);
      break;
    case DG_GELU: dense_nt_kernel<DG_GELU, 4><<<p.grid, 512, smem, s>>>(a); break;
    case DG_RESID: dense_nt_kernel<DG_RESID, 4><<<p.grid, 512, smem, s>>>(a); break;
    case DG_DGELU: dense_nt_kernel<DG_DGELU, 4><<<p.grid, 512, smem, s>>>(a); break;
    case DG_GELUF: dense_nt_kernel<DG_GELUF, 4><<<p.grid, 512, smem, s>>>(a); break;
    case DG_DFACT: dense_nt_kernel<DG_DFACT, 4><<<p.grid, 512, smem, s>>>(a); break;
    case DG_GELUO: dense_nt_kernel<DG_GELUO, 4><<<p.grid, 512, smem, s>>>(a); break;
    default: return OCTIC_ESHAPE;
  }
  if (tp.image && dense_cls_two_launches(mode, N, K) && workspace && p.split <= 1) {
    const int rows_pad = (tp.images + 63) / 64 * 64;
    float* part = (float*)((char*)workspace + DG_TICKET_BYTES);
    const int cus = dense_cus(), per64 = (N / 64) * (K / CLS_KSLICE) * (rows_pad / 64);
    const int nw = (per64 > cus && (N % 80) == 0 && (N / 80) * (K / CLS_KSLICE) * (rows_pad / 64) <= cus) ? 5 : 4;
    dense_cls_part_kernel<<<(N / (16 * nw)) * (K / CLS_KSLICE) * (rows_pad / 64), 64 * nw, 0, s>>>(a, tokens, tp.images, rows_pad, part);
    dense_cls_sum_kernel<<<(tp.images * (N / 4) + 255) / 256, 256, 0, s>>>(a, tokens, tp.images, rows_pad, part);
  } else if (tp.image) {
    const int grid = (N / 16) * ((tp.images + 15) / 16), cr0 = 2 * tp.images, thr = 64 * dense_cls_waves(K);
    switch (mode) {
      case DG_PLAIN: dense_cls_kernel<DG_PLAIN><<<grid, thr, 0, s>>>(a, tokens, tp.images, cr0); break;
      case DG_GELU: dense_cls_kernel<DG_GELU><<<grid, thr, 0, s>>>(a, tokens, tp.images, cr0); break;
      case DG_DGELU: dense_cls_kernel<DG_DGELU><<<grid, thr, 0, s>>>(a, tokens, tp.images, cr0); break;
      case DG_GELUF: dense_cls_kernel<DG_GELUF><<<grid, thr, 0, s>>>(a, tokens, tp.images, cr0); break;
      case DG_DFACT: dense_cls_kernel<DG_DFACT><<<grid, thr, 0, s>>>(a, tokens, tp.images, cr0); break;
      case DG_GELUO: dense_cls_kernel<DG_GELUO><<<grid, thr, 0, s>>>(a, tokens, tp.images, cr0); break;
      default: return OCTIC_ESHAPE;
    }
  }
  return launch_status();
}

int octic_dense_gemm_nt_tokens(const void* A, const void* B, int M, int N, int K, int64_t lda, int64_t ldb, int mode, void* C,
                               void* C2, int64_t ldc, const float* bias, const float* gamma, const float* rs, int64_t rps,
                               const float* X, float* OUT, const void* H, float* colsum, void* workspace, int tokens,
                               void* stream) {
  return octic_dense_gemm_nt_tokens_skip(A, B, M, N, K, lda, ldb, mode, C, C2, ldc, bias, gamma, rs, rps, X, OUT, H, colsum,
                                         nullptr, 0, workspace, tokens, stream);
}

int octic_dense_gemm_plan_dropped(int M, int N, int K, int mode, int tokens, int rows_per_sample, int* out) {
  if (!out) return OCTIC_ENULL;
  if (rows_per_sample <= 0 || M <= 0 || (M % rows_per_sample) != 0) return OCTIC_ESHAPE;
  return octic_dense_gemm_plan(M, N, K, mode, tokens, out);
}

int octic_dense_gemm_order_dropped(int M, int N, int K, int mode, int tokens, const float* sample_scale, int rows_per_sample,
                                   int cap, int* out_tm, int* out_tn, int* out_part, int* out_split, int* out_dead) {
  if (!sample_scale) return OCTIC_ENULL;
  if (M <= 0 || N <= 0 || K < 2 * DG_BK || rows_per_sample <= 0 || (M % rows_per_sample) != 0 || mode == DG_RESID) return OCTIC_ESHAPE;
  const DgTokPlan tp = dense_plan_tokens(M, N, K, dense_cus(), mode, tokens);
  const DgPlan p = tp.p;
  if (p.tiles_m > kDgMaskCap || cap < p.grid) return OCTIC_ESHAPE;
  unsigned long long bm[kDgMaskWords] = {};
  for (int tm = 0; tm < p.tiles_m; ++tm)
    if (dg_panel_live(sample_scale, rows_per_sample, M, tp.image ? tokens : DG_BM, tp.image ? 1 : 0, tm)) bm[tm >> 6] |= 1ull << (tm & 63);
  for (int bid = 0; bid < p.grid; ++bid) {
    int tile, rem_idx, part, tm = -1, tn = -1;
    bool dead;
    dense_item_masked(p.tiles_m, p.tiles_n, p.full, p.split, p.tail_pad, bid, bm, tile, rem_idx, part, dead);
    if (tile >= 0) dg_tile_panel(p.tiles_m, p.tiles_n, tile, tm, tn);
    if (out_tm) out_tm[bid] = tm;
    if (out_tn) out_tn[bid] = tn;
    if (out_part) out_part[bid] = part;
    if (out_split) out_split[bid] = rem_idx >= 0 ? 1 : 0;
    if (out_dead) out_dead[bid] = dead ? 1 : 0;
  }
  return p.grid;
}

int octic_dense_gemm_nt(const void* A, const void* B, int M, int N, int K, int64_t lda, int64_t ldb, int mode, void* C,
                        void* C2, int64_t ldc, const float* bias, const float* gamma, const float* rs, int64_t rps,
                        const float* X, float* OUT, const void* H, float* colsum, void* workspace, void* stream) {
  return octic_dense_gemm_nt_tokens(A, B, M, N, K, lda, ldb, mode, C, C2, ldc, bias, gamma, rs, rps, X, OUT, H, colsum,
                                    workspace, 0, stream);
}

}
```

### octic_vits_amd/functional.py

```python
import os

import torch

from . import ops


class Octic(tuple):

    def __new__(cls, packed: torch.Tensor, c: int):
        self = super().__new__(cls, ops.split_packed(packed, c))
        self.packed, self.c = packed, c
        return self


def as_packed(xs):
    if isinstance(xs, Octic):
        return xs.packed, xs.c
    if len(xs) != 5:
        raise AssertionError("Input should be a 5-tuple")
    c = xs[0].shape[-1]
    if xs[4].shape[-2:] != (2, 2 * c):
        raise ValueError(f"E irrep must be [..., 2, {2 * c}], got {tuple(xs[4].shape)}")
    return torch.cat([xs[0], xs[1], xs[2], xs[3], xs[4].flatten(-2)], dim=-1), c

# ... 241 lines not shown
        x, wb, M, y, b32, cs32, rs32 = _linear_d8_fwd_prep(ctx, x, w5, cs5, bias, rs, cin, cout, rps, dtype, out_dtype, prep)
        rv = ops.pview(_c(resid), cout) if fused else None
        plain = not fused and rs32 is None and cs32 is None
        ss_out = linear_skip_scale(skip_out, rps, M) if plain else None
        dropped = ring_skip_scale(rs32, rps, M) if fused else None
        ops.linear_fwd(ops.pview(x, cin), wb, b32, ops.pview(y, cout), M, cin, cout, dtype, out_dtype, x,
                       resid_v=rv, rs=rs32, rps=rps, cs5=cs32, sample_scale=ss_out, skip_rps=rps, dropped=dropped, dropped_rps=rps)
        ss_dx = linear_skip_scale(skip_dx, rps, M)
        z_dx = ring_skip_scale(zero_dx, rps, M) if (plain and ss_dx is None) else None
        row_skip_fill(handed, row_skip_scale(zero_dx, rps, M) if (plain and ss_dx is None) else None, rps, M)
        ctx.save_for_backward(x, rs32, b32, ss_dx, z_dx, *w5, *(cs32 or []))
        ctx.fused = fused
        return y

    @staticmethod
    def backward(ctx, dy):
        cin, cout, rps, dtype, has_cs = ctx.lin[:5]
        x, rs32, b32, ss_dx, z_dx, *rest = ctx.saved_tensors
        w5, cs32 = rest[:5], (rest[5:] if has_cs else None)
        dy = _c(dy)
        if ctx.fused or rs32 is not None or dy.dtype != dtype:
            g = ops.cast_rowscale(_c(dy.float()), rs32, rps, dtype, cout)
        else:
            g = dy
        dx, dw, dbias, dcs = _linear_d8_grads(ctx, x, g, w5, cs32, b32, ss_dx, z_dx)
        return (dx, *dw, dbias, dy if ctx.fused else None, None, *dcs, None, None, None, None, None, None, None, None)


class LinearD8NormFn(torch.autograd.Function):

    @staticmethod
    def forward(ctx, x, wA1, wA2, wB1, wB2, wE, bias, resid, rs, sA1, sA2, sB1, sB2, sE, cin, cout, rps, dtype, prep,
                a1, a2, b1, b2, ae, beta, eps, skip_dx=None):
        w5 = (wA1, wA2, wB1, wB2, wE)
        cs5 = None if sA1 is None else (sA1, sA2, sB1, sB2, sE)
        x, wb, M, y, b32, cs32, rs32 = _linear_d8_fwd_prep(ctx, x, w5, cs5, bias, rs, cin, cout, rps, dtype, resid.dtype, prep)
        ops.linear_fwd(ops.pview(x, cin), wb, b32, ops.pview(y, cout), M, cin, cout, dtype, resid.dtype, x,
                       resid_v=ops.pview(_c(resid), cout), rs=rs32, rps=rps, cs5=cs32, dropped=ring_skip_scale(rs32, rps, M),
                       dropped_rps=rps)
        alpha = None if a1 is None else [_c(t.float()) for t in (a1, a2, b1, b2, ae)]
        yn, stats = ops.layernorm_fwd(y, alpha, None if beta is None else _c(beta.float()), eps, dtype, cout)
        ctx.save_for_backward(x, rs32, b32, y, stats, linear_skip_scale(skip_dx, rps, M), *w5, *(cs32 or []), *(alpha or []))
        ctx.has_affine, ctx.has_beta = alpha is not None, beta is not None
        ctx.set_materialize_grads(False)
        row_skip_attach(ctx, yn)
        return y, yn

    @staticmethod
    def backward(ctx, dy, dyn):
        cin, cout, rps, dtype, has_cs = ctx.lin[:5]
        has_affine = ctx.has_affine
        x, rs32, b32, y, stats, ss_dx, *rest = ctx.saved_tensors
        w5 = rest[:5]
        cs32 = rest[5:10] if has_cs else None
        alpha = rest[(10 if has_cs else 5):] if has_affine else None
        M = x.numel() // (8 * cin)
        dal, dbeta, g = [None] * 5, None, None
        if dyn is not None:
            dres = None if dy is None else _c(dy.float())
            gn = _c(dyn)
            ns, nrps = row_skip_get(ctx, M)
            if ops.layernorm_bwd_cast_ok(gn, y, cout) and dtype == torch.bfloat16:
                dy, dal_, dbeta, g = ops.layernorm_bwd_cast(gn, y, stats, alpha, dres, cout, rs32, rps,
                                                            want_param_grads=has_affine, sample_scale=ns, rows_per_sample=nrps)
            else:
                dy, dal_, dbeta = ops.layernorm_bwd(gn, y, stats, alpha, dres, cout, want_param_grads=has_affine,
                                                    sample_scale=ns, rows_per_sample=nrps)
            dal = dal_ if dal_ is not None else dal
        dy = _c(dy)
        if g is None:
            g = ops.cast_rowscale(_c(dy.float()), rs32, rps, dtype, cout)
        dx, dw, dbias, dcs = _linear_d8_grads(ctx, x, g, w5, cs32, b32, ss_dx)
        return (dx, *dw, dbias, dy, None, *dcs, None, None, None, None, None, *dal, dbeta if ctx.has_beta else None, None, None)


class PackHeadsFn(torch.autograd.Function):

    @staticmethod
    def forward(ctx, qkv, H, c):
        B, T = qkv.shape[0], qkv.shape[1]
        ctx.meta = (B, T, H, c)
        q, k, v = ops.pack_heads(_c(qkv), B, T, H, c, 3)
        return q, k, v

    @staticmethod
    def backward(ctx, gq, gk, gv):
        B, T, H, c = ctx.meta
        return ops.unpack_heads([gq, gk, gv], B, T, H, c), None, None


class UnpackHeadsFn(torch.autograd.Function):
    @staticmethod
    def forward(ctx, o, c):
        B, H, T, _ = o.shape
        ctx.meta = (B, T, H, c)
        return ops.unpack_heads([o], B, T, H, c)

    @staticmethod
    def backward(ctx, g):
        B, T, H, c = ctx.meta
        return ops.pack_heads(_c(g), B, T, H, c, 1)[0], None


class AttnFn(torch.autograd.Function):

    @staticmethod
    def forward(ctx, q, k, v, scale):
        q, k, v = _c(q), _c(k), _c(v)
        o, lse = ops.attn_fwd(q, k, v, scale)
        ctx.save_for_backward(q, k, v, o, lse)
        ctx.scale = scale
        return o

    @staticmethod
    def backward(ctx, do):
        q, k, v, o, lse = ctx.saved_tensors
        do = _c(do)
        dq, dk, dv = torch.empty_like(q), torch.empty_like(k), torch.empty_like(v)
        ops.attn_bwd(q, k, v, o, do, lse, ctx.scale, dq, dk, dv)
        return dq, dk, dv, None


def _skip_from_env(name):
    return os.environ.get(name, "1").strip() != "0"


ATTN_SKIP_DROPPED = _skip_from_env("OCTIC_ATTN_SKIP")


def skip_scale(rs, B):
    if (not ATTN_SKIP_DROPPED or rs is None or not rs.is_cuda or rs.dtype != torch.float32 or rs.dim() != 1
            or rs.numel() != B or not rs.is_contiguous()):
        return None
    return rs.detach()


WGRAD_SKIP_DROPPED = _skip_from_env("OCTIC_WGRAD_SKIP")


def whole_sample_mask(rs, rps, M, rows_to=None):
    if (rs is None or rows_to is not None or torch.compiler.is_compiling() or not rs.is_cuda
            or rs.dtype != torch.float32 or rs.dim() != 1 or not rs.is_contiguous() or rps < 2 or rs.numel() * rps != M):
        return None
    return rs.detach()


def wgrad_skip_scale(rs, rps, M, rows_to=None):
    return whole_sample_mask(rs, rps, M, rows_to) if WGRAD_SKIP_DROPPED else None


DENSE_NT_SKIP_DROPPED = _skip_from_env("OCTIC_DENSE_SKIP")


def dense_skip_scale(rs, rps, M, rows_to=None):
    return whole_sample_mask(rs, rps, M, rows_to) if DENSE_NT_SKIP_DROPPED else None


LINEAR_SKIP_DROPPED = _skip_from_env("OCTIC_LINEAR_SKIP")


def linear_skip_scale(rs, rps, M, rows_to=None):
    return whole_sample_mask(rs, rps, M, rows_to) if LINEAR_SKIP_DROPPED else None


RING_SKIP_DROPPED = _skip_from_env("OCTIC_RING_SKIP")


def ring_skip_scale(rs, rps, M):
    return linear_skip_scale(rs, rps, M) if RING_SKIP_DROPPED else None


ROW_SKIP_DROPPED = _skip_from_env("OCTIC_ROW_SKIP")


def row_skip_scale(rs, rps, M, rows_to=None):
    return whole_sample_mask(rs, rps, M, rows_to) if ROW_SKIP_DROPPED else None


class RowSkipSlot:
    __slots__ = ("scale", "rps", "rows", "fills")

    def __init__(self):
        self.scale, self.rps, self.rows, self.fills = None, 0, 0, 0

    def get(self, rows):
        if self.fills != 1 or self.scale is None or self.rows != rows:
            return None, 0
        return self.scale, self.rps


def row_skip_attach(ctx, yn):
    ctx.row_skip = yn._octic_row_skip = RowSkipSlot()


def row_skip_fill(x, scale, rps, rows):
    slot = getattr(x, "_octic_row_skip", None)
    if slot is not None:
        slot.fills += 1
        slot.scale, slot.rps, slot.rows = scale, rps, rows


def row_skip_get(ctx, rows):
    slot = getattr(ctx, "row_skip", None)
    return (None, 0) if slot is None else slot.get(rows)


class AttnPackedFn(torch.autograd.Function):

    @staticmethod
    def forward(ctx, qkv, H, c, scale, sample_scale=None):
        qkv = _c(qkv)
        ss = skip_scale(sample_scale, qkv.shape[0])
        o, lse = ops.attn_fwd_packed(qkv, H, c, scale, sample_scale=ss)
        ctx.save_for_backward(qkv, o, lse, ss)
        ctx.meta = (H, c, scale)
        return o

    @staticmethod
    def backward(ctx, do):
        qkv, o, lse, ss = ctx.saved_tensors
        H, c, scale = ctx.meta
        return ops.attn_bwd_packed(qkv, o, _c(do), lse, H, c, scale, sample_scale=ss), None, None, None, None


class AttnFusedQKVFn(torch.autograd.Function):

    @staticmethod
    def forward(ctx, qkv, scale, sample_scale=None):
        qkv = _c(qkv)
        B, T, _, H, hd = qkv.shape
        ss = skip_scale(sample_scale, B) if qkv.dtype == torch.bfloat16 else None
        q, k, v = (qkv[:, :, i].permute(0, 2, 1, 3) for i in range(3))
        o = torch.empty((B, T, H, hd), dtype=qkv.dtype, device=qkv.device)
        ov = o.permute(0, 2, 1, 3)
        _, lse = ops.attn_fwd(q, k, v, scale, out=ov, sample_scale=ss)
        ctx.save_for_backward(qkv, o, lse, ss)
        ctx.scale = scale
        return o.view(B, T, H * hd)

    @staticmethod
    def backward(ctx, do):
        qkv, o, lse, ss = ctx.saved_tensors
        B, T, _, H, hd = qkv.shape
        do = _c(do).view(B, T, H, hd)
        dqkv = torch.empty_like(qkv)
        q, k, v = (qkv[:, :, i].permute(0, 2, 1, 3) for i in range(3))
        dq, dk, dv = (dqkv[:, :, i].permute(0, 2, 1, 3) for i in range(3))
        ops.attn_bwd(q, k, v, o.permute(0, 2, 1, 3), do.permute(0, 2, 1, 3), lse, ctx.scale, dq, dk, dv, sample_scale=ss)
        return dqkv, None, None


def attention_core(q, k, v, dropout_p=0.0):
    B, H, T, hd = q.shape
    if dropout_p == 0.0 and q.is_cuda and (ops.attn_supported(T, hd, q.dtype) or ops.attn_f32_supported(T, hd, q.dtype)):
        return AttnFn.apply(q, k, v, hd ** -0.5)
    o = torch.nn.functional.scaled_dot_product_attention(q, k, v, dropout_p=dropout_p)
    return o if o.dtype == q.dtype else o.to(q.dtype)


class DenseWeightCache:

    def __init__(self):
        self.key = None
        self.w = self.b = None
        self.wt = self.wt_key = None
        self.static = False
        self.static_wt = False

    def static_nt(self):
        if self.static and self.w is not None and self.w.dtype == torch.bfloat16:
            return self.w, (self.wt if self.static_wt else None)
        return None, None

    @staticmethod
    def _key(w, b, dtype):
        return (dtype, w.data_ptr(), w._version, None if b is None else (b.data_ptr(), b._version))

    def get(self, w, b, dtype):
        key = self._key(w, b, dtype)
        if key != self.key:
            with torch.no_grad():
                self.w = _c(w.detach().to(dtype))
                self.b = None if b is None else _c(b.detach().to(dtype))
            self.key = key
            self.wt, self.wt_key = None, None
            self.static = self.static_wt = False
        return self.w, self.b

    def adopt(self, w, b, w_copy, b_copy, dtype, wt_copy=None):
        self.w, self.b = w_copy, b_copy
        self.key = self._key(w, b, dtype)
        self.static = True
        self.static_wt = wt_copy is not None
        if wt_copy is not None:
            self.wt, self.wt_key = wt_copy, self.key

    def get_nt(self, w, b, need_wt=True):
        wb, _ = self.get(w, b, torch.bfloat16)
        if not need_wt:
            return wb, None
        if self.wt is None or self.wt_key != self.key:
            with torch.no_grad():
                self.wt = wb.t().contiguous()
            self.wt_key = self.key
        return wb, self.wt

# ... 618 lines not shown
```

### octic_vits_amd/ops.py

```python
import ctypes
import operator

import torch

from . import _lib
from ._lib import BF16, F32, OcticView, PtrArray5, check, lib

_DT = {torch.float32: F32, torch.bfloat16: BF16}
_DTN = {torch.float32: "f32", torch.bfloat16: "bf16"}


class KernelTimer:

    def __init__(self):
        self.on = False
        self.records = []
        self.overhead_us = 0.0

    def enable(self):
        self.on, self.records = True, []
        pairs = []
        for _ in range(64):
            e0, e1 = torch.cuda.Event(enable_timing=True), torch.cuda.Event(enable_timing=True)
            e0.record()
# ... 942 lines not shown
    return ds.view(s.shape)


def scale_residual_fwd(x, y, gamma, rs, rps):
    _require_cuda(x)
    d = x.shape[-1]
    rows = x.numel() // d
    out = torch.empty_like(x)
    t = KERNEL_TIMER.start()
    check(lib().octic_scale_residual_fwd(_p(x), _p(y), dt_code(y.dtype), _p(gamma), _p(rs), int(rps), _p(out), rows, d,
                                         _stream(x)))
    KERNEL_TIMER.stop(t, f"scale_residual_fwd_kernel<{_DTN[y.dtype]}>", rows * d * (8 + y.element_size()))
    return out


def scale_residual_fwd_rows_(stream, rowmap, x, y, gamma, rs, rps):
    _require_cuda(x)
    d = x.shape[-1]
    rows = rowmap.numel()
    _check_rowmap(rowmap, rows)
    t = KERNEL_TIMER.start()
    check(lib().octic_scale_residual_fwd_rows(_p(x), _p(y), dt_code(y.dtype), _p(gamma), _p(rs), int(rps), _p(stream), rows, d,
                                              _p(rowmap), _stream(x)))
    KERNEL_TIMER.stop(t, f"scale_residual_fwd_kernel<{_DTN[y.dtype]},rows>", rows * d * (8 + y.element_size()))
    return stream


def scale_residual_bwd(gout, y, gamma, rs, rps, want_gamma=True, want_colsum=True, rowmap=None):
    d = gout.shape[-1]
    rows = gout.numel() // d if rowmap is None else rowmap.numel()
    if rowmap is not None:
        _check_rowmap(rowmap, rows)
    gy = torch.empty(gout.shape if rowmap is None else y.shape, dtype=y.dtype, device=gout.device)
    nblk = lib().octic_dense_blocks(rows)
    want = want_gamma or want_colsum
    partials = torch.empty((nblk, 2, d), dtype=torch.float32, device=gout.device) if want else None
    t = KERNEL_TIMER.start()
    check(lib().octic_scale_residual_bwd_rows(_p(gout), _p(y), dt_code(y.dtype), _p(gamma), _p(rs), int(rps), _p(gy),
                                              _p(partials), rows, d, _p(rowmap), _stream(gout)))
    KERNEL_TIMER.stop(t, f"scale_residual_bwd_kernel<{_DTN[y.dtype]}>", rows * d * (4 + 2 * y.element_size()))
    if not want:
        return gy, None, None
    dgamma = torch.empty(d, dtype=torch.float32, device=gout.device) if want_gamma else None
    colsum = torch.empty(d, dtype=torch.float32, device=gout.device) if want_colsum else None
    _finish(partials, nblk, d, dgamma, colsum, gamma, _stream(gout))
    return gy, dgamma, colsum


def dense_gelu_bwd(h, g, want_colsum=True):
    _require_cuda(h)
    d = h.shape[-1]
    rows = h.numel() // d
    dh = torch.empty_like(h)
    nblk = lib().octic_dense_gelu_blocks()
    partials = torch.empty((nblk, d), dtype=torch.float32, device=h.device) if want_colsum else None
    t = KERNEL_TIMER.start()
    check(lib().octic_dense_gelu_bwd(_p(h), _p(g), _p(dh), _p(partials), rows, d, _stream(h)))
    KERNEL_TIMER.stop(t, "dense_gelu_bwd_kernel", rows * d * 6)
    if not want_colsum:
        return dh, None
    out = torch.empty(d, dtype=torch.float32, device=h.device)
    half = d // 2
    _finish(partials, nblk, half, out, None, None, _stream(h), out1_ptr=out.data_ptr() + 4 * half)
    return dh, out


def _swiglu_rows(t, width, what):
    if t.dim() != 2:
        t = t.reshape(-1, t.shape[-1]) if t.is_contiguous() else t.contiguous().view(-1, t.shape[-1])
    if t.dtype != torch.bfloat16 or t.shape[1] != width or t.stride(1) != 1:
        raise ValueError(f"swiglu: {what} must be bf16 [rows, {width}] with contiguous columns, got {tuple(t.shape)} {t.dtype}")
    return t


def swiglu_fwd(x12, H, out=None):
    _require_cuda(x12)
    lead = x12.shape[:-1]
    x2d = _swiglu_rows(x12, 2 * H, "x12")
    rows = x2d.shape[0]
    a = torch.empty((rows, H), dtype=torch.bfloat16, device=x12.device) if out is None else _swiglu_rows(out, H, "out")
    t = KERNEL_TIMER.start()
    check(lib().octic_swiglu_fwd(_p(x2d), x2d.stride(0), _p(a), a.stride(0), rows, H, _stream(x12)))
    KERNEL_TIMER.stop(t, "swiglu_fwd_kernel", rows * H * 6)
    return a.view(*lead, H) if out is None else out


def swiglu_bwd(x12, ga, want_colsum=True, out=None):
    _require_cuda(x12)
    H = ga.shape[-1]
    x2d, g2d = _swiglu_rows(x12, 2 * H, "x12"), _swiglu_rows(ga, H, "ga")
    rows = x2d.shape[0]
    if g2d.shape[0] != rows:
        raise ValueError("swiglu_bwd: x12 and ga differ in rows")
    d = torch.empty((rows, 2 * H), dtype=torch.bfloat16, device=x12.device) if out is None else _swiglu_rows(out, 2 * H, "out")
    nblk = lib().octic_swiglu_blocks()
    partials = torch.empty((nblk, 2 * H), dtype=torch.float32, device=x12.device) if want_colsum and rows else None
    t = KERNEL_TIMER.start()
    check(lib().octic_swiglu_bwd(_p(x2d), x2d.stride(0), _p(g2d), g2d.stride(0), _p(d), d.stride(0), _p(partials), rows, H,
                                 _stream(x12)))
    KERNEL_TIMER.stop(t, "swiglu_bwd_kernel", rows * H * 10)
    dx = d.view(x12.shape) if out is None else out
    if not want_colsum:
        return dx, None
    if partials is None:
        return dx, torch.zeros(2 * H, dtype=torch.float32, device=x12.device)
    db = torch.empty(2 * H, dtype=torch.float32, device=x12.device)
    _finish(partials, nblk, H, db, None, None, _stream(x12), out1_ptr=db.data_ptr() + 4 * H)
    return dx, db


_DG_WS = {}
_lib.on_route_override(_DG_WS.clear)


def _dense_ws(M, N, K, dev):
    key = (M, N, K, dev)
    ws = _DG_WS.get(key)
    if ws is None:
        ws = _DG_WS[key] = torch.zeros(int(lib().octic_dense_gemm_workspace_bytes(M, N, K)), dtype=torch.uint8, device=dev)
    return ws


def dense_colsum(g, sample_scale=None, rows_per_sample=0):
    _require_cuda(g)
    rows, d = g.shape
    if g.stride(1) != 1:
        raise ValueError("dense_colsum: rows must be contiguous along d")
    ss, srps = _sample_scale(sample_scale, rows_per_sample, rows, g, "dense_colsum")
    nblk = lib().octic_dense_gelu_blocks()
    partials = torch.empty((nblk, d), dtype=torch.float32, device=g.device)
    t = KERNEL_TIMER.start()
    check(lib().octic_dense_colsum_skip(_p(g), rows, d, g.stride(0), _p(partials), _p(ss), srps, _stream(g)))
    KERNEL_TIMER.stop(t, "dense_colsum_kernel", rows * d * 2)
    out = torch.empty(d, dtype=torch.float32, device=g.device)
    half = d // 2
    _finish(partials, nblk, half, out, None, None, _stream(g), out1_ptr=out.data_ptr() + 4 * half)
    return out


def dense_plan(M, N, K, mode, tokens):
    out = _lib.plan("octic_dense_gemm_plan", M, N, K, mode, int(tokens))
    if out is None:
        check(-1)
    return out[0], out[1], bool(out[2]), out[3]


def dense_plan_dropped(M, N, K, mode, tokens, rows_per_sample):
    out = _lib.plan("octic_dense_gemm_plan_dropped", M, N, K, mode, int(tokens), int(rows_per_sample))
    if out is None:
        check(-1)
    return out[0], out[1], bool(out[2]), out[3]


def dense_gemm_nt(a, b, mode=0, bias=None, gamma=None, rs=None, rps=1, x=None, h=None, name=None, want_colsum=False,
                  tokens=0, sample_scale=None, rows_per_sample=0):
    _require_cuda(a)
    M, K = a.shape
    N = b.shape[0]
    if a.stride(1) != 1 or b.stride(1) != 1 or b.shape[1] != K:
        raise ValueError("dense_gemm_nt: operands must be [M,K] / [N,K] with contiguous K")
    c = torch.empty((M, N), dtype=torch.bfloat16, device=a.device)
    c2 = torch.empty_like(c) if mode in (1, 4) else None
    out = torch.empty((M, N), dtype=torch.float32, device=a.device) if mode == 2 else None
    ws = _dense_ws(M, N, K, a.device)
    tokens = int(tokens) if (tokens and M % int(tokens) == 0) else 0
    if sample_scale is not None and mode == 2:
        raise ValueError("dense_gemm_nt: the fused residual tail (mode 2) takes no sample_scale")
    ss, srps = _sample_scale(sample_scale, rows_per_sample, M, a, "dense_gemm_nt")
    cs_rows = dense_plan(M, N, K, mode, tokens)[1] if (mode in (3, 5) and want_colsum) else 0
    cs = torch.empty((cs_rows, N), dtype=torch.float32, device=a.device) if cs_rows else None
    t = KERNEL_TIMER.start()
    check(lib().octic_dense_gemm_nt_tokens_skip(_p(a), _p(b), M, N, K, a.stride(0), b.stride(0), mode, _p(c), _p(c2), N, _p(bias),
                                                _p(gamma), _p(rs), int(rps), _p(x), _p(out), _p(h), _p(cs), _p(ss), srps,
                                                _p(ws), tokens, _stream(a)))
    if t is not None:
        nb = 2 * (M * K + N * K + M * N * (2 if mode in (1, 3, 4, 5) else 1)) + (8 * M * N if mode == 2 else 0)
        wide = "@320" if dense_plan(M, N, K, mode, tokens)[0] == 320 else ""
        KERNEL_TIMER.stop(t, (name or f"dense_nt_kernel<{mode}>") + wide, nb, 2.0 * M * N * K)
    if mode in (1, 4):
        return c, c2
    if mode == 2:
        return c, out
    if cs is not None:
        colsum = torch.empty(N, dtype=torch.float32, device=a.device)
        _finish(cs, cs_rows, N // 2, colsum, None, None, _stream(a), out1_ptr=colsum.data_ptr() + 2 * N)
        return c, colsum
    return c


def probe_features(pairs, F):
    n = len(pairs)
    patch, cls0 = pairs[-1][0], pairs[0][1]
    _require_cuda(patch)
    B, P, D = patch.shape
    dtype = patch.dtype
    for p, c in pairs:
        if c.dtype != dtype or p.dtype != dtype or tuple(c.shape) != (B, D) or c.stride(1) != 1:
            raise ValueError("probe_features: class tokens must be [B, D] rows of one dtype")
    if patch.stride(2) != 1 or F.dtype != torch.float32 or F.stride(1) != 1 or F.shape[0] < B:
        raise ValueError("probe_features: patch tokens / F must have contiguous channels")
    cls = (ctypes.c_void_p * n)(*[c.data_ptr() for _, c in pairs])
    cls_ld = (ctypes.c_int64 * n)(*[c.stride(0) for _, c in pairs])
    t = KERNEL_TIMER.start()
    check(lib().octic_probe_features(cls, cls_ld, n, _p(patch), patch.stride(0), patch.stride(1), dt_code(dtype), B, P, D,
                                     _p(F), F.stride(0), _stream(patch)))
    KERNEL_TIMER.stop(t, f"probe_features_kernel<{_DTN[dtype]}>", B * D * (P + n) * patch.element_size() + 4 * B * (n + 1) * D)
    return F


def probe_forward(table, nheads, F, B, C, logits, sumK):
    t = KERNEL_TIMER.start()
    check(lib().octic_probe_forward(_p(table), nheads, _p(F), F.stride(0), B, C, _p(logits), _stream(F)))
    KERNEL_TIMER.stop(t, "probe_forward_kernel", 4 * (C * sumK + nheads * B * C), 2.0 * B * C * sumK)


def probe_ce(logits, labels, nheads, B, C, dlogits, rowloss, rowrank, loss_mean=None, loss_sum=None, topk=None):
    if labels.dtype != torch.int64 or not labels.is_contiguous() or labels.numel() != B:
        raise ValueError("probe_ce: labels must be a contiguous int64 tensor of B class indices")
    t = KERNEL_TIMER.start()
    check(lib().octic_probe_ce(_p(logits), _p(labels), nheads, B, C, _p(dlogits), _p(rowloss), _p(rowrank), _p(loss_mean),
                               _p(loss_sum), _p(topk), _stream(logits)))
    KERNEL_TIMER.stop(t, "probe_ce_kernel", 4 * nheads * B * C * (3 if dlogits is not None else 2))


def probe_sgd(table, nheads, total_ktiles, F, dlogits, B, C, lr, momentum, sumK):
    t = KERNEL_TIMER.start()
    check(lib().octic_probe_sgd(_p(table), nheads, total_ktiles, _p(F), F.stride(0), _p(dlogits), B, C, _p(lr),
                                float(momentum), _stream(F)))
    KERNEL_TIMER.stop(t, "probe_sgd_kernel", 16 * C * sumK, 2.0 * B * C * sumK)


def _seg_rows(X):
    _require_cuda(X)
    if X.dim() != 2 or X.dtype != torch.float32 or X.stride(1) != 1:
        raise ValueError("segmentation ops take an f32 [N, D] matrix with contiguous channels")
    return X.shape[0], X.shape[1], X.stride(0)


def seg_ldd(C):
    ldd = lib().octic_seg_ldd(int(C))
    check(min(ldd, 0))
    return ldd


def seg_workspace(N, D, C, device):
    nbytes = lib().octic_seg_workspace_bytes(N, D, C)
    check(min(nbytes, 0))
    return torch.empty(nbytes, dtype=torch.uint8, device=device)


def seg_value_dlogits(X, W, b, y, dlogits, value, workspace):
    N, D, ldx = _seg_rows(X)
    C = W.shape[0]
    if (W.dtype != torch.float32 or not W.is_contiguous() or W.shape[1] != D or b.dtype != torch.float32 or b.numel() != C
            or not b.is_contiguous()):
        raise ValueError("seg_value_dlogits: W must be a contiguous f32 [C, D], b a contiguous f32 [C]")
    if y.dtype != torch.int32 or not y.is_contiguous() or y.numel() != N:
        raise ValueError("seg_value_dlogits: y must be a contiguous int32 tensor of N class indices")
    if (dlogits.dtype != torch.float32 or not dlogits.is_contiguous() or dlogits.numel() < N * max(seg_ldd(C), 0)
            or value.dtype != torch.float64):
        raise ValueError("seg_value_dlogits: dlogits must be a contiguous f32 [N, seg_ldd(C)], value an f64 scalar")
    t = KERNEL_TIMER.start()
    check(lib().octic_seg_value_dlogits(_p(X), ldx, N, D, _p(W), _p(b), C, _p(y), _p(dlogits), _p(value), _p(workspace),
                                        _stream(X)))
    KERNEL_TIMER.stop(t, "seg_forward_kernel", 4 * N * (D + seg_ldd(C)), 2.0 * N * C * D)


def seg_predict(X, W, b, pred):
    N, D, ldx = _seg_rows(X)
    C = W.shape[0]
    if W.dtype != torch.float32 or not W.is_contiguous() or W.shape[1] != D or b.dtype != torch.float32 or b.numel() != C:
        raise ValueError("seg_predict: W must be a contiguous f32 [C, D], b an f32 [C]")
    if pred.dtype != torch.int32 or not pred.is_contiguous() or pred.numel() != N:
        raise ValueError("seg_predict: pred must be a contiguous int32 [N]")
    t = KERNEL_TIMER.start()
    check(lib().octic_seg_predict(_p(X), ldx, N, D, _p(W), _p(b), C, _p(pred), _stream(X)))
    KERNEL_TIMER.stop(t, "seg_forward_kernel<predict>", 4 * N * (D + 1), 2.0 * N * C * D)


def seg_wgrad(X, dlogits, W, scale, lam, dW, db, workspace):
    N, D, ldx = _seg_rows(X)
    C = W.shape[0]
    if (dW.dtype != torch.float32 or not dW.is_contiguous() or tuple(dW.shape) != (C, D) or db.dtype != torch.float32
            or db.numel() != C or not W.is_contiguous() or W.dtype != torch.float32):
        raise ValueError("seg_wgrad: W / dW must be contiguous f32 [C, D], db an f32 [C]")
    t = KERNEL_TIMER.start()
    check(lib().octic_seg_wgrad(_p(X), ldx, N, D, _p(dlogits), C, _p(W), float(scale), float(lam), _p(dW), _p(db),
                                _p(workspace), _stream(X)))
    KERNEL_TIMER.stop(t, "seg_wgrad_kernel", 4 * N * D, 2.0 * N * C * D)


def seg_colstats(X):
    N, D, ldx = _seg_rows(X)
    nbytes = lib().octic_seg_colstats_workspace_bytes(N, D)
    check(min(nbytes, 0))
    ws = torch.empty(nbytes // 8, dtype=torch.float64, device=X.device)
    mean = torch.empty(D, dtype=torch.float64, device=X.device)
    var = torch.empty(D, dtype=torch.float64, device=X.device)
    t = KERNEL_TIMER.start()
    check(lib().octic_seg_colstats(_p(X), ldx, N, D, _p(mean), _p(var), _p(ws), _stream(X)))
    KERNEL_TIMER.stop(t, "seg_colstats_kernel", 4 * N * D)
    return mean, var


def seg_standardize_(X, mean, scale):
    N, D, ldx = _seg_rows(X)
    for v in (mean, scale):
        if v.dtype != torch.float64 or v.numel() != D or not v.is_contiguous() or v.device != X.device:
            raise ValueError("seg_standardize_: mean and scale must be contiguous f64 [D] on X's device")
    t = KERNEL_TIMER.start()
    check(lib().octic_seg_standardize(_p(X), ldx, N, D, _p(mean), _p(scale), _stream(X)))
    KERNEL_TIMER.stop(t, "seg_standardize_kernel", 8 * N * D)
    return X


_SEG_LABEL_DTYPES = (torch.uint8, torch.int16, torch.int32, torch.int64)


def _seg_labels(labels):
    _require_cuda(labels)
    if labels.dim() != 2 or labels.dtype not in _SEG_LABEL_DTYPES or not labels.is_contiguous():
        raise ValueError("segmentation labels must be a contiguous [R, L] tensor of uint8 / int16 / int32 / int64 values 0 .. 255")
    return labels.shape[0], labels.shape[1], labels.element_size()


def seg_patch_mode(labels):
    R, L, es = _seg_labels(labels)
# ... 357 lines not shown
```

Before: 1198 images/s.

## Add adaptive dense GEMM kernel choosing narrow tiles when few panels survive drop-path

```diff
diff --git a/include/octic_hip.h b/include/octic_hip.h
--- a/include/octic_hip.h
+++ b/include/octic_hip.h
@@ -330,6 +330,14 @@
 int octic_dense_gemm_plan_dropped(int M, int N, int K, int mode, int tokens, int rows_per_sample, int* out4);
 int octic_dense_gemm_order_dropped(int M, int N, int K, int mode, int tokens, const float* sample_scale, int rows_per_sample,
                                    int cap, int* out_tm, int* out_tn, int* out_part, int* out_split, int* out_dead);
+int octic_dense_gemm_nt_tokens_adaptive(const void* A, const void* B, int M, int N, int K, int64_t lda, int64_t ldb, int mode,
+                                        void* C, void* C2, int64_t ldc, const float* bias, const float* gamma, const float* rs,
+                                        int64_t rows_per_sample_rs, const float* X, float* OUT, const void* H, float* colsum,
+                                        const float* sample_scale, int rows_per_sample, void* workspace, int tokens,
+                                        void* stream);
+int octic_dense_gemm_plan_adaptive(int M, int N, int K, int mode, int tokens, int rows_per_sample, int* out5);
+int octic_dense_gemm_order_adaptive(int M, int N, int K, int mode, int tokens, const float* sample_scale, int rows_per_sample,
+                                    int cap, int* out_tm, int* out_tn, int* out_dead, int* out_width);
 
 int64_t octic_dense_wgrad_workspace_bytes(int M, int N, int K);
 int octic_dense_wgrad_tile(int M, int N, int K);
diff --git a/octic_vits_amd/_lib.py b/octic_vits_amd/_lib.py
--- a/octic_vits_amd/_lib.py
+++ b/octic_vits_amd/_lib.py
@@ -10,6 +10,8 @@
 ABI_VERSION = 20
 (ROUTE_DENSE_TILE, ROUTE_DENSE_SPLIT, ROUTE_WGRAD_SLABS, ROUTE_WGRAD_TILE, ROUTE_LINEAR_RING, ROUTE_RING_EVEN,
  ROUTE_ATTN_LEGACY, ROUTE_ATTN_ONLINE, ROUTE_ATTN_BWD_PAIR, ROUTE_DENSE_IMAGE, ROUTE_DENSE_CLS2, ROUTE_ATTN_STREAM) = range(12)
+
+DENSE_ADAPT_WIDE, DENSE_ADAPT_NARROW = 16, 32
 
 (ATTN_FWD_PERSIST, ATTN_FWD_A80_ONESHOT, ATTN_FWD_A80_ONLINE, ATTN_FWD_RESIDENT, ATTN_FWD_STREAM, ATTN_FWD_F32) = range(6)
 ATTN_BWD_SINGLE, ATTN_BWD_PAIR, ATTN_BWD_STREAM, ATTN_BWD_F32 = range(4)
@@ -158,6 +160,12 @@
     "octic_dense_gemm_plan_dropped": (c_int, [c_int, c_int, c_int, c_int, c_int, c_int, ctypes.POINTER(c_int)]),
     "octic_dense_gemm_order_dropped": (c_int, [c_int, c_int, c_int, c_int, c_int, c_void_p, c_int, c_int, c_void_p, c_void_p,
                                                c_void_p, c_void_p, c_void_p]),
+    "octic_dense_gemm_nt_tokens_adaptive": (c_int, [c_void_p, c_void_p, c_int, c_int, c_int, c_i64, c_i64, c_int, c_void_p, c_void_p,
+                                                    c_i64, c_void_p, c_void_p, c_void_p, c_i64, c_void_p, c_void_p, c_void_p,
+                                                    c_void_p, c_void_p, c_int, c_void_p, c_int, c_void_p]),
+    "octic_dense_gemm_plan_adaptive": (c_int, [c_int, c_int, c_int, c_int, c_int, c_int, ctypes.POINTER(c_int)]),
+    "octic_dense_gemm_order_adaptive": (c_int, [c_int, c_int, c_int, c_int, c_int, c_void_p, c_int, c_int, c_void_p, c_void_p,
+                                                c_void_p, c_void_p]),
     "octic_dense_colsum": (c_int, [c_void_p, c_i64, c_int, c_i64, c_void_p, c_void_p]),
     "octic_dense_colsum_skip": (c_int, [c_void_p, c_i64, c_int, c_i64, c_void_p, c_void_p, c_i64, c_void_p]),
     "octic_dense_wgrad_workspace_bytes": (c_i64, [c_int, c_int, c_int]),
diff --git a/octic_vits_amd/csrc/dense_gemm.hip b/octic_vits_amd/csrc/dense_gemm.hip
--- a/octic_vits_amd/csrc/dense_gemm.hip
+++ b/octic_vits_amd/csrc/dense_gemm.hip
@@ -52,6 +52,9 @@
   int* tickets;
   const float* sample_scale;
   int rows_per_sample;
+  int tiles_n_narrow;
+  int cus;
+  int narrow_force;
 };
 
 enum DgMode { DG_PLAIN = 0, DG_GELU = 1, DG_RESID = 2, DG_DGELU = 3,
@@ -147,6 +150,27 @@
   tile = dg_select_full(bm, tiles_m, tiles_n, full, rank, true);
 }
 
+__host__ __device__ inline bool dg_narrow_pays(int live_panels, int tiles_n_narrow, int cus) {
+  return live_panels * tiles_n_narrow <= cus;
+}
+__host__ __device__ inline bool dg_adaptive_narrow(int live_panels, int tiles_n_narrow, int cus, int force) {
+  return force == 2 || (force != 1 && dg_narrow_pays(live_panels, tiles_n_narrow, cus));
+}
+__host__ __device__ inline int dg_live_panels(const unsigned long long* bm, int tiles_m) {
+  int n = 0;
+  for (int w = 0; w < (tiles_m + 63) >> 6; ++w) n += __builtin_popcountll(bm[w]);
+  return n;
+}
+__host__ __device__ inline void dense_item_adaptive(int tiles_m, int tiles_n_wide, int tiles_n_narrow, int cus, int force, int bid,
+                                                    const unsigned long long* bm, bool& narrow, int& tile, bool& dead) {
+  narrow = dg_adaptive_narrow(dg_live_panels(bm, tiles_m), tiles_n_narrow, cus, force);
+  const int tiles_n = narrow ? tiles_n_narrow : tiles_n_wide, full = tiles_m * tiles_n;
+  tile = -1; dead = false;
+  if (bid >= full) return;
+  int rem_idx, part;
+  dense_item_masked(tiles_m, tiles_n, full, 1, 0, bid, bm, tile, rem_idx, part, dead);
+}
+
 __device__ inline void dg_wait_vmcnt(int n) {
   switch (n) {
     case 2: asm volatile("s_waitcnt vmcnt(2)" ::: "memory"); break;
@@ -228,9 +252,9 @@
   else asm volatile("s_waitcnt vmcnt(0)" ::: "memory");
 }
 
-template <int MODE, int NT, bool SKIP = false>
-__global__ __launch_bounds__(512, 1) void dense_nt_kernel(DgArgs a) {
-  extern __shared__ __attribute__((aligned(16))) char lds[];
+template <int MODE, int NT, bool SKIP>
+__device__ __forceinline__ void dense_nt_tile(const DgArgs a, char* lds, int tile, int kt_begin, int kt_end, int part, int rem_idx,
+                                              bool dead_item) {
   using GE = DgGeom<NT>;
   constexpr int NA = GE::NA, DG_BN = GE::BN;
   static_assert(NT == 4 || MODE == DG_PLAIN, "the fused tails exist for the 256-wide tile only");
@@ -243,9 +267,456 @@
   const int fr = lane & 15, kg = lane >> 4;
 #ifdef DG_TRACE
   int dgt_i = 0;
+#endif
+  DGT();
+  int tm, tn;
+  {
+    const int G = 8;
+    const int per_group = G * a.tiles_n;
+    const int gidx = tile / per_group;
+    const int first_m = gidx * G;
+    const int gsz = (a.tiles_m - first_m) < G ? (a.tiles_m - first_m) : G;
+    const int in_g = tile - gidx * per_group;
+    tm = first_m + in_g % gsz;
+    tn = in_g / gsz;
+  }
+  const int m0 = tm * a.m_stride + a.m_base, n0 = tn * DG_BN;
+  if constexpr (SKIP) {
+    if (dead_item) {
+      if (part != 0) return;
+      constexpr int CPR = DG_BN / 8;
+      const u32x4 z = {0, 0, 0, 0};
+#pragma unroll 4
+      for (int p = threadIdx.x; p < DG_BM * CPR; p += 512) {
+        const int r = p / CPR, c = p - r * CPR;
+        const int m = m0 + r, n = n0 + c * 8;
+        if (m < a.M && n < a.N) {
+          *(u32x4*)(a.C + (int64_t)m * a.ldc + n) = z;
+          if (MODE == DG_GELU || MODE == DG_GELUF) *(u32x4*)(a.C2 + (int64_t)m * a.ldc + n) = z;
+        }
+      }
+      if ((MODE == DG_DGELU || MODE == DG_DFACT) && a.colsum != nullptr) {
+        const int t = threadIdx.x;
+        const int row = t / (DG_BN / 4), n = n0 + (t - row * (DG_BN / 4)) * 4;
+        if (row < 2 && n < a.N) *(f32x4*)(a.colsum + (int64_t)(tm * 2 + row) * a.N + n) = f32x4{0, 0, 0, 0};
+      }
+      return;
+    }
+  }
+  const int nkt = kt_end - kt_begin;
+  const int nunits = 4 * nkt;
+
+  const int drow = lane >> 3;
+  const int dch = (lane & 7) ^ drow;
+  const __amdgpu_buffer_rsrc_t rsA = __builtin_amdgcn_make_buffer_rsrc((void*)a.A, 0, (int)((int64_t)a.M * a.lda * 2), 0x27000);
+  const __amdgpu_buffer_rsrc_t rsB = __builtin_amdgcn_make_buffer_rsrc((void*)a.B, 0, (int)((int64_t)a.N * a.ldb * 2), 0x27000);
+  const int r0 = 16 * wid + drow;
+  const int am0 = m0, an0 = n0;
+  const unsigned voA = (unsigned)(((int64_t)(am0 + (r0 >> 6) * 128 + (r0 & 63)) * a.lda + dch * 8) * 2);
+  const int rb1 = 8 * NA * wid + drow;
+  const unsigned voB1 = (unsigned)(((int64_t)(an0 + (rb1 / (16 * NA)) * GE::WCOLS + (rb1 % (16 * NA))) * a.ldb + dch * 8) * 2);
+  const unsigned voB2 = (unsigned)(((int64_t)(an0 + (r0 >> 5) * GE::WCOLS + 16 * NA + (r0 & 31)) * a.ldb + dch * 8) * 2);
+  const int rowA8 = (int)(a.lda * 16), rowB8 = (int)(a.ldb * 16);
+  const int halfA = (int)(a.lda * 128);
+  const int kbase = kt_begin * (DG_BK * 2);
+
+  int u_issue = 0;
+  auto issue_unit = [&](auto kind_c) {
+    constexpr int KIND = decltype(kind_c)::value;
+    constexpr bool isA = KIND == 0 || KIND == 3;
+    char* dst = lds + ((u_issue >> 2) & 1) * GE::KT + GE::unit_off(KIND) + wid * (GE::unit_instr(KIND) * 1024);
+    const int so = kbase + (u_issue >> 2) * (DG_BK * 2) + (KIND == 3 ? halfA : 0);
+    if constexpr (isA) {
+      __builtin_amdgcn_raw_ptr_buffer_load_lds(rsA, (__attribute__((address_space(3))) void*)dst, 16, voA, so, 0, 0);
+      __builtin_amdgcn_raw_ptr_buffer_load_lds(rsA, (__attribute__((address_space(3))) void*)(dst + 1024), 16, voA, so + rowA8, 0, 0);
+    } else if constexpr (KIND == 1) {
+      __builtin_amdgcn_raw_ptr_buffer_load_lds(rsB, (__attribute__((address_space(3))) void*)dst, 16, voB1, so, 0, 0);
+      __builtin_amdgcn_raw_ptr_buffer_load_lds(rsB, (__attribute__((address_space(3))) void*)(dst + 1024), 16, voB1, so + rowB8, 0, 0);
+      if constexpr (NA == 3)
+        __builtin_amdgcn_raw_ptr_buffer_load_lds(rsB, (__attribute__((address_space(3))) void*)(dst + 2048), 16, voB1, so + 2 * rowB8, 0, 0);
+    } else {
+      __builtin_amdgcn_raw_ptr_buffer_load_lds(rsB, (__attribute__((address_space(3))) void*)dst, 16, voB2, so, 0, 0);
+      __builtin_amdgcn_raw_ptr_buffer_load_lds(rsB, (__attribute__((address_space(3))) void*)(dst + 1024), 16, voB2, so + rowB8, 0, 0);
+    }
+    ++u_issue;
+  };
+  auto young_instr = [&](int n) {
+    const int k1 = ((u_issue + 2) >> 2) - ((u_issue - n + 2) >> 2);
+    return 2 * n + (NA - 2) * k1;
+  };
+#define DG_IC(v) std::integral_constant<int, v>()
+
+  const int sw = lane & 7;
+  const int rdo0 = fr * 128 + ((kg ^ sw) << 4);
+  const int rdo1 = fr * 128 + (((4 + kg) ^ sw) << 4);
+  const int a_row0 = wr * 64;
+
+  bf16x8 Af[1][2][4];
+  bf16x8 Bf0[2][NA], Bf1[2][2];
+  f32x4 acc0[2][4][NA], acc1[2][4][2];
+#pragma unroll
+  for (int i = 0; i < 2; ++i)
+#pragma unroll
+    for (int p = 0; p < 4; ++p) {
+#pragma unroll
+      for (int q = 0; q < NA; ++q) acc0[i][p][q] = f32x4{0, 0, 0, 0};
+#pragma unroll
+      for (int q = 0; q < 2; ++q) acc1[i][p][q] = f32x4{0, 0, 0, 0};
+    }
+  int rt_hi = (a.M - m0 - wr * 128 + 15) >> 4;
+  rt_hi = rt_hi < 0 ? 0 : (rt_hi > 8 ? 8 : rt_hi);
+  const int live_mask = __builtin_amdgcn_readfirstlane((rt_hi > 0 ? 1 : 0) | (rt_hi > 4 ? 2 : 0));
+
+  auto readA = [&](int mh, int unit) {
+    const char* base = lds + ((unit >> 2) & 1) * GE::KT + GE::unit_off(mh ? 3 : 0) + a_row0 * 128;
+#pragma unroll
+    for (int mi = 0; mi < 4; ++mi) {
+      Af[0][0][mi] = *(const bf16x8*)(base + mi * 2048 + rdo0);
+      Af[0][1][mi] = *(const bf16x8*)(base + mi * 2048 + rdo1);
+    }
+  };
+  auto readB = [&](int nh, int unit) {
+    if (nh == 0) {
+      const char* base = lds + ((unit >> 2) & 1) * GE::KT + GE::unit_off(1) + wc * (16 * NA) * 128;
+#pragma unroll
+      for (int ni = 0; ni < NA; ++ni) {
+        Bf0[0][ni] = *(const bf16x8*)(base + ni * 2048 + rdo0);
+        Bf0[1][ni] = *(const bf16x8*)(base + ni * 2048 + rdo1);
+      }
+    } else {
+      const char* base = lds + ((unit >> 2) & 1) * GE::KT + GE::unit_off(2) + wc * 32 * 128;
+#pragma unroll
+      for (int ni = 0; ni < 2; ++ni) {
+        Bf1[0][ni] = *(const bf16x8*)(base + ni * 2048 + rdo0);
+        Bf1[1][ni] = *(const bf16x8*)(base + ni * 2048 + rdo1);
+      }
+    }
+  };
+  auto mma = [&](int mh, int nh, auto kind_c) {
+    asm volatile("s_waitcnt lgkmcnt(0)" ::: "memory");
+    __builtin_amdgcn_sched_barrier(0);
+    if (live_mask & (mh ? 2 : 1)) {
+#pragma unroll
+    for (int ks = 0; ks < 2; ++ks) {
+#pragma unroll
+      for (int mi = 0; mi < 4; ++mi) {
+        if (nh == 0) {
+#pragma unroll
+          for (int ni = 0; ni < NA; ++ni)
+            acc0[mh][mi][ni] = __builtin_amdgcn_mfma_f32_16x16x32_bf16(Bf0[ks][ni], Af[0][ks][mi], acc0[mh][mi][ni], 0, 0, 0);
+        } else {
+#pragma unroll
+          for (int ni = 0; ni < 2; ++ni)
+            acc1[mh][mi][ni] = __builtin_amdgcn_mfma_f32_16x16x32_bf16(Bf1[ks][ni], Af[0][ks][mi], acc1[mh][mi][ni], 0, 0, 0);
+        }
+      }
+    }
+    }
+    __builtin_amdgcn_sched_barrier(0);
+  };
+
+  int g = 0;
+  auto wait_landed = [&]() {
+    int need = g + 2;
+    need = need < nunits - 1 ? need : nunits - 1;
+    const int ok = (u_issue - 1) - need;
+    if (ok == DG_D - 2) dg_wait_imm<GE::INFLIGHT>();
+    else dg_wait_vmcnt(ok > 0 ? young_instr(ok) : 0);
+  };
+
+#define DG_PRO(i) if constexpr ((i) < DG_D) { if (u_issue < nunits) issue_unit(DG_IC((i) & 3)); }
+  DG_PRO(0) DG_PRO(1) DG_PRO(2) DG_PRO(3) DG_PRO(4) DG_PRO(5) DG_PRO(6) DG_PRO(7) DG_PRO(8) DG_PRO(9)
+#undef DG_PRO
+  {
+    const int ok = (u_issue - 1) - 1;
+    dg_wait_vmcnt(ok > 0 ? young_instr(ok) : 0);
+  }
+  if (hi) __builtin_amdgcn_s_barrier();
+  DGT2(1);
+
+  auto ktile = [&](int t, auto steady_c) {
+    constexpr bool STEADY = decltype(steady_c)::value != 0;
+    const int u0 = 4 * t;
+    auto dma = [&](auto kind_c) {
+      if (STEADY || u_issue < nunits) issue_unit(kind_c);
+    };
+    auto landed = [&]() {
+      if constexpr (STEADY) dg_wait_imm<GE::INFLIGHT>();
+      else wait_landed();
+    };
+#define DG_RP(x) do { __builtin_amdgcn_s_setprio(x); } while (0)
+#define DG_R(q, reads) do { DG_RP(2); dma(DG_IC(((q) + DG_D) & 3)); reads; DG_RP(0); } while (0)
+    __builtin_amdgcn_s_barrier();
+    DGT();
+    DG_R(0, readA(0, u0); readB(0, u0 + 1));
+    if (hi) landed();
+    DGT();
+    __builtin_amdgcn_s_barrier();
+    DGT();
+    mma(0, 0, DG_IC((0 + DG_D) & 3));
+    DGT();
+    if (!hi) landed();
+    ++g;
+    __builtin_amdgcn_s_barrier();
+    DGT();
+    DG_R(1, readB(1, u0 + 2));
+    if (hi) landed();
+    DGT();
+    __builtin_amdgcn_s_barrier();
+    DGT();
+    mma(0, 1, DG_IC((1 + DG_D) & 3));
+    DGT();
+    if (!hi) landed();
+    ++g;
+    __builtin_amdgcn_s_barrier();
+    DGT();
+    DG_R(2, readA(1, u0 + 3));
+    if (hi) landed();
+    DGT();
+    __builtin_amdgcn_s_barrier();
+    DGT();
+    mma(1, 1, DG_IC((2 + DG_D) & 3));
+    DGT();
+    if (!hi) landed();
+    ++g;
+    __builtin_amdgcn_s_barrier();
+    DGT();
+    DG_R(3, (void)0);
+    if (hi) landed();
+    DGT();
+    __builtin_amdgcn_s_barrier();
+    DGT();
+    mma(1, 0, DG_IC((3 + DG_D) & 3));
+    DGT();
+    if (!hi) landed();
+    ++g;
+#undef DG_R
+#undef DG_RP
+  };
+  const int t_steady = (nunits - 4 - DG_D) >= 0 ? (nunits - 4 - DG_D) / 4 + 1 : 0;
+  int t = 0;
+#pragma unroll 1
+  for (; t < t_steady; ++t) ktile(t, DG_IC(1));
+#pragma unroll 1
+  for (; t < nkt; ++t) ktile(t, DG_IC(0));
+  if (!hi) __builtin_amdgcn_s_barrier();
+  __builtin_amdgcn_s_barrier();
+  DGT2(2);
+
+  const int rt_lo = 0;
+  auto ACC = [&](int mh, int mi, int j) -> f32x4& { return j < NA ? acc0[mh][mi][j] : acc1[mh][mi][j - NA]; };
+  if (rem_idx >= 0 && a.split > 1) {
+    float* slab = a.slabs + ((int64_t)rem_idx * a.split + part) * (DG_BM * DG_BN);
+    f32x4* sw4 = (f32x4*)slab + (int64_t)wid * (8 * NT) * 64 + lane;
+#pragma unroll
+    for (int mh = 0; mh < 2; ++mh)
+#pragma unroll
+      for (int mi = 0; mi < 4; ++mi) {
+        if (mh * 4 + mi >= rt_hi) continue;
+#pragma unroll
+        for (int j = 0; j < NT; ++j) sw4[((mh * 4 + mi) * NT + j) * 64] = ACC(mh, mi, j);
+      }
+    asm volatile("s_waitcnt vmcnt(0)" ::: "memory");
+    __syncthreads();
+    DGT2(5);
+    int* flag = (int*)lds;
+    if (threadIdx.x == 0) {
+      __builtin_amdgcn_fence(__ATOMIC_RELEASE, "agent");
+      asm volatile("s_waitcnt vmcnt(0)" ::: "memory");
+      const int old = __hip_atomic_fetch_add(a.tickets + rem_idx, 1, __ATOMIC_RELAXED, __HIP_MEMORY_SCOPE_AGENT);
+      flag[0] = (old == a.split - 1) ? 1 : 0;
+      if (old == a.split - 1) {
+        __builtin_amdgcn_fence(__ATOMIC_ACQUIRE, "agent");
+        asm volatile("s_waitcnt vmcnt(0)" ::: "memory");
+        __hip_atomic_store(a.tickets + rem_idx, 0, __ATOMIC_RELAXED, __HIP_MEMORY_SCOPE_AGENT);
+      }
+    }
+    __syncthreads();
+    const int last = flag[0];
+    __syncthreads();
+    if (last == 0) return;
+    DGT2(6);
+    for (int p = 0; p < a.split; ++p) {
+      const f32x4* o4 = (const f32x4*)(a.slabs + ((int64_t)rem_idx * a.split + p) * (DG_BM * DG_BN)) +
+                        (int64_t)wid * (8 * NT) * 64 + lane;
+#pragma unroll
+      for (int mh = 0; mh < 2; ++mh)
+#pragma unroll
+        for (int mi = 0; mi < 4; ++mi) {
+          if (mh * 4 + mi >= rt_hi) continue;
+#pragma unroll
+          for (int j = 0; j < NT; ++j) {
+            const f32x4 o = o4[((mh * 4 + mi) * NT + j) * 64];
+            ACC(mh, mi, j) = p == 0 ? o : ACC(mh, mi, j) + o;
+          }
+        }
+    }
+  }
+
+  if constexpr (NT != 4) {
+    constexpr int SRS = GE::SRS;
+    char* const stg = lds + wid * (GE::EPI_ROWS * SRS);
+    const int er = lane / 10, ech = lane - er * 10;
+    const int n = n0 + wc * GE::WCOLS + ech * 8;
+    const bool nok = n < a.N && lane < 60;
+#pragma unroll
+    for (int mh = 0; mh < 2; ++mh) {
+      if (mh * 4 >= rt_hi) break;
+#pragma unroll
+      for (int j = 0; j < NT; ++j) {
+        const int nl = j * 16 + kg * 4;
+        const int nb = n0 + wc * GE::WCOLS + nl;
+        f32x4 bv = {0, 0, 0, 0};
+        if (a.bias && nb < a.N) bv = *(const f32x4*)(a.bias + nb);
+#pragma unroll
+        for (int mi = 0; mi < 4; ++mi) {
+          if (mh * 4 + mi >= rt_hi) continue;
+          const f32x4 v = ACC(mh, mi, j) + bv;
+          const bf16x4 cb = {(bf16)v[0], (bf16)v[1], (bf16)v[2], (bf16)v[3]};
+          *(bf16x4*)(stg + (mi * 16 + fr) * SRS + nl * 2) = cb;
+        }
+      }
+      asm volatile("s_waitcnt lgkmcnt(0)" ::: "memory");
+#pragma unroll
+      for (int it = 0; it < 11; ++it) {
+        const int row = it * 6 + er;
+        const int m = m0 + wr * 128 + mh * 64 + row;
+        if (row >= 64 || m >= a.M || !nok || mh * 4 + (row >> 4) >= rt_hi) continue;
+        const u32x4 raw = *(const u32x4*)(stg + row * SRS + ech * 16);
+        *(u32x4*)(a.C + (int64_t)m * a.ldc + n) = raw;
+      }
+    }
+  } else {
+  constexpr int SRS = GE::SRS;
+  char* const stg = lds + wid * (128 * SRS);
+#pragma unroll
+  for (int j = 0; j < NT; ++j) {
+      const int nl = j * 16 + kg * 4;
+      const int n = n0 + wc * 64 + nl;
+      f32x4 bv = {0, 0, 0, 0};
+      if (a.bias && n < a.N) bv = *(const f32x4*)(a.bias + n);
+#pragma unroll
+      for (int mh = 0; mh < 2; ++mh)
+#pragma unroll
+        for (int mi = 0; mi < 4; ++mi) {
+          if (mh * 4 + mi < rt_lo || mh * 4 + mi >= rt_hi) continue;
+          const f32x4 v = ACC(mh, mi, j) + bv;
+          const bf16x4 cb = {(bf16)v[0], (bf16)v[1], (bf16)v[2], (bf16)v[3]};
+          *(bf16x4*)(stg + (mh * 64 + mi * 16 + fr) * SRS + nl * 2) = cb;
+        }
+    }
+  asm volatile("s_waitcnt lgkmcnt(0)" ::: "memory");
+  const int srow = lane >> 3, sch = lane & 7;
+  const int n = n0 + wc * 64 + sch * 8;
+  const bool nok = n < a.N;
+  f32x4 gm0 = {1, 1, 1, 1}, gm1 = {1, 1, 1, 1};
+  if (MODE == DG_RESID && a.gamma && nok) {
+    gm0 = *(const f32x4*)(a.gamma + n);
+    gm1 = *(const f32x4*)(a.gamma + n + 4);
+  }
+  f32x4 xin[MODE == DG_RESID ? 16 : 1][2];
+  bf16x8 hin[(MODE == DG_DGELU || MODE == DG_DFACT) ? 16 : 1];
+  float csum[8] = {0, 0, 0, 0, 0, 0, 0, 0};
+  if (MODE == DG_RESID || MODE == DG_DGELU || MODE == DG_DFACT) {
+#pragma unroll
+    for (int it = 0; it < 16; ++it) {
+      const int m = m0 + wr * 128 + it * 8 + srow;
+      const bool ok = m < a.M && nok && (it >> 1) >= rt_lo && (it >> 1) < rt_hi;
+      if (MODE == DG_RESID) {
+        const float* xp = a.X + (int64_t)(ok ? m : 0) * a.N + (ok ? n : 0);
+        xin[it][0] = *(const f32x4*)xp;
+        xin[it][1] = *(const f32x4*)(xp + 4);
+      } else {
+        hin[it] = *(const bf16x8*)(a.H + (int64_t)(ok ? m : 0) * a.ldc + (ok ? n : 0));
+      }
+    }
+  }
+#pragma unroll
+  for (int it = 0; it < 16; ++it) {
+    const int row = it * 8 + srow;
+    const int m = m0 + wr * 128 + row;
+    if (m >= a.M || !nok || (it >> 1) < rt_lo || (it >> 1) >= rt_hi) continue;
+    const u32x4 raw = *(const u32x4*)(stg + row * SRS + sch * 16);
+    const bf16x8 cb = __builtin_bit_cast(bf16x8, raw);
+    bf16* cp = a.C + (int64_t)m * a.ldc + n;
+    if (MODE == DG_PLAIN) {
+      *(u32x4*)cp = raw;
+    } else if (MODE == DG_GELU) {
+      *(u32x4*)cp = raw;
+      bf16x8 y;
+#pragma unroll
+      for (int e = 0; e < 8; ++e) y[e] = (bf16)dg_gelu((float)cb[e]);
+      *(bf16x8*)(a.C2 + (int64_t)m * a.ldc + n) = y;
+    } else if (MODE == DG_GELUO) {
+      bf16x8 y;
+#pragma unroll
+      for (int e = 0; e < 8; ++e) y[e] = (bf16)dg_gelu((float)cb[e]);
+      *(bf16x8*)cp = y;
+    } else if (MODE == DG_GELUF) {
+      bf16x8 y, f;
+#pragma unroll
+      for (int e = 0; e < 8; ++e) {
+        float gv, dv;
+        dg_gelu_both((float)cb[e], gv, dv);
+        y[e] = (bf16)gv;
+        f[e] = (bf16)dv;
+      }
+      *(bf16x8*)cp = f;
+      *(bf16x8*)(a.C2 + (int64_t)m * a.ldc + n) = y;
+    } else if (MODE == DG_RESID) {
+      *(u32x4*)cp = raw;
+      const float rsv = a.rs ? a.rs[m / a.rps] : 1.0f;
+      f32x4 x0 = xin[it][0], x1 = xin[it][1];
+#pragma unroll
+      for (int e = 0; e < 4; ++e) {
+        x0[e] += rsv * gm0[e] * (float)cb[e];
+        x1[e] += rsv * gm1[e] * (float)cb[4 + e];
+      }
+      float* op = a.OUT + (int64_t)m * a.N + n;
+      *(f32x4*)op = x0;
+      *(f32x4*)(op + 4) = x1;
+    } else {
+      const bf16x8 h = hin[it];
+      bf16x8 d;
+#pragma unroll
+      for (int e = 0; e < 8; ++e) {
+        d[e] = (bf16)((MODE == DG_DFACT ? (float)h[e] : dg_gelu_grad((float)h[e])) * (float)cb[e]);
+        csum[e] += (float)d[e];
+      }
+      *(bf16x8*)cp = d;
+    }
+  }
+  if ((MODE == DG_DGELU || MODE == DG_DFACT) && a.colsum != nullptr) {
+#pragma unroll
+    for (int e = 0; e < 8; ++e) {
+      float v = csum[e];
+      v += __shfl_xor(v, 8, 64);
+      v += __shfl_xor(v, 16, 64);
+      v += __shfl_xor(v, 32, 64);
+      csum[e] = v;
+    }
+    if (srow == 0 && nok) {
+      float* base = a.colsum + (int64_t)(tm * 2 + wr) * a.N + n;
+      *(f32x4*)base = f32x4{csum[0], csum[1], csum[2], csum[3]};
+      *(f32x4*)(base + 4) = f32x4{csum[4], csum[5], csum[6], csum[7]};
+    }
+  }
+  }
+#ifdef DG_TRACE2
+  DGT2(3);
+  asm volatile("s_waitcnt vmcnt(0)" ::: "memory");
+  DGT2(4);
+#endif
+}
+
+__device__ __forceinline__ void dg_trace_start() {
+#if defined(DG_TRACE) || defined(DG_TRACE2)
+  const int lane = threadIdx.x & 63;
+  const int wid = __builtin_amdgcn_readfirstlane(threadIdx.x >> 6);
+#endif
+#ifdef DG_TRACE
   if (blockIdx.x == 0 && lane == 0) g_dg_trace[wid * 256 + 254] = __builtin_amdgcn_s_memrealtime();
 #endif
-  DGT();
   DGT2(0);
 #ifdef DG_TRACE2
   if (wid == 0 && lane == 0 && blockIdx.x < 4096) {
@@ -255,6 +726,26 @@
     g_dg_trace2[blockIdx.x * 8 + 7] = ((unsigned long long)hwid << 32) | xcc;
   }
 #endif
+}
+
+__device__ __forceinline__ void dg_build_bitmap(const DgArgs& a, unsigned long long* live_bm) {
+  const int lane = threadIdx.x & 63;
+  const int wid = __builtin_amdgcn_readfirstlane(threadIdx.x >> 6);
+  const int words = (a.tiles_m + 63) >> 6;
+  for (int w = wid; w < words; w += 8) {
+    const int p = w * 64 + lane;
+    const bool live = p < a.tiles_m && dg_panel_live(a.sample_scale, a.rows_per_sample, a.M, a.m_stride, a.m_base, p);
+    const unsigned long long m = __ballot(live);
+    if (lane == 0) live_bm[w] = m;
+  }
+  __syncthreads();
+}
+
+template <int MODE, int NT, bool SKIP = false>
+__global__ __launch_bounds__(512, 1) void dense_nt_kernel(DgArgs a) {
+  extern __shared__ __attribute__((aligned(16))) char lds[];
+  using GE = DgGeom<NT>;
+  dg_trace_start();
 
   const int bid = blockIdx.x;
   int tile, kt_begin, kt_end, part = 0, rem_idx = -1;
@@ -262,14 +753,7 @@
   bool dead_item = false;
   if constexpr (SKIP) {
     unsigned long long* const live_bm = (unsigned long long*)(lds + GE::LDS);
-    const int words = (a.tiles_m + 63) >> 6;
-    for (int w = wid; w < words; w += 8) {
-      const int p = w * 64 + lane;
-      const bool live = p < a.tiles_m && dg_panel_live(a.sample_scale, a.rows_per_sample, a.M, a.m_stride, a.m_base, p);
-      const unsigned long long m = __ballot(live);
-      if (lane == 0) live_bm[w] = m;
-    }
-    __syncthreads();
+    dg_build_bitmap(a, live_bm);
     dense_item_masked(a.tiles_m, a.tiles_n, a.full_tiles, a.split, a.tail_pad, bid, live_bm, tile, rem_idx, part, dead_item);
     tile = __builtin_amdgcn_readfirstlane(tile);
     rem_idx = __builtin_amdgcn_readfirstlane(rem_idx);
@@ -295,444 +779,30 @@
     kt_begin = (int)(((int64_t)nkt_all * part) / a.split);
     kt_end = (int)(((int64_t)nkt_all * (part + 1)) / a.split);
   }
-  int tm, tn;
-  {
-    const int G = 8;
-    const int per_group = G * a.tiles_n;
-    const int gidx = tile / per_group;
-    const int first_m = gidx * G;
-    const int gsz = (a.tiles_m - first_m) < G ? (a.tiles_m - first_m) : G;
-    const int in_g = tile - gidx * per_group;
-    tm = first_m + in_g % gsz;
-    tn = in_g / gsz;
-  }
-  const int m0 = tm * a.m_stride + a.m_base, n0 = tn * DG_BN;
-  if constexpr (SKIP) {
-    if (dead_item) {
-      if (part != 0) return;
-      constexpr int CPR = DG_BN / 8;
-      const u32x4 z = {0, 0, 0, 0};
-#pragma unroll 4
-      for (int p = threadIdx.x; p < DG_BM * CPR; p += 512) {
-        const int r = p / CPR, c = p - r * CPR;
-        const int m = m0 + r, n = n0 + c * 8;
-        if (m < a.M && n < a.N) {
-          *(u32x4*)(a.C + (int64_t)m * a.ldc + n) = z;
-          if (MODE == DG_GELU || MODE == DG_GELUF) *(u32x4*)(a.C2 + (int64_t)m * a.ldc + n) = z;
-        }
-      }
-      if ((MODE == DG_DGELU || MODE == DG_DFACT) && a.colsum != nullptr) {
-        const int t = threadIdx.x;
-        const int row = t / (DG_BN / 4), n = n0 + (t - row * (DG_BN / 4)) * 4;
-        if (row < 2 && n < a.N) *(f32x4*)(a.colsum + (int64_t)(tm * 2 + row) * a.N + n) = f32x4{0, 0, 0, 0};
-      }
-      return;
-    }
-  }
-  const int nkt = kt_end - kt_begin;
-  const int nunits = 4 * nkt;
-
-  const int drow = lane >> 3;
-  const int dch = (lane & 7) ^ drow;
-  const __amdgpu_buffer_rsrc_t rsA = __builtin_amdgcn_make_buffer_rsrc((void*)a.A, 0, (int)((int64_t)a.M * a.lda * 2), 0x27000);
-  const __amdgpu_buffer_rsrc_t rsB = __builtin_amdgcn_make_buffer_rsrc((void*)a.B, 0, (int)((int64_t)a.N * a.ldb * 2), 0x27000);
-  const int r0 = 16 * wid + drow;
-  const int am0 = m0, an0 = n0;
-  const unsigned voA = (unsigned)(((int64_t)(am0 + (r0 >> 6) * 128 + (r0 & 63)) * a.lda + dch * 8) * 2);
-  const int rb1 = 8 * NA * wid + drow;
-  const unsigned voB1 = (unsigned)(((int64_t)(an0 + (rb1 / (16 * NA)) * GE::WCOLS + (rb1 % (16 * NA))) * a.ldb + dch * 8) * 2);
-  const unsigned voB2 = (unsigned)(((int64_t)(an0 + (r0 >> 5) * GE::WCOLS + 16 * NA + (r0 & 31)) * a.ldb + dch * 8) * 2);
-  const int rowA8 = (int)(a.lda * 16), rowB8 = (int)(a.ldb * 16);
-  const int halfA = (int)(a.lda * 128);
-  const int kbase = kt_begin * (DG_BK * 2);
-
-  int u_issue = 0;
-  auto issue_unit = [&](auto kind_c) {
-    constexpr int KIND = decltype(kind_c)::value;
-    constexpr bool isA = KIND == 0 || KIND == 3;
-    char* dst = lds + ((u_issue >> 2) & 1) * GE::KT + GE::unit_off(KIND) + wid * (GE::unit_instr(KIND) * 1024);
-    const int so = kbase + (u_issue >> 2) * (DG_BK * 2) + (KIND == 3 ? halfA : 0);
-    if constexpr (isA) {
-      __builtin_amdgcn_raw_ptr_buffer_load_lds(rsA, (__attribute__((address_space(3))) void*)dst, 16, voA, so, 0, 0);
-      __builtin_amdgcn_raw_ptr_buffer_load_lds(rsA, (__attribute__((address_space(3))) void*)(dst + 1024), 16, voA, so + rowA8, 0, 0);
-    } else if constexpr (KIND == 1) {
-      __builtin_amdgcn_raw_ptr_buffer_load_lds(rsB, (__attribute__((address_space(3))) void*)dst, 16, voB1, so, 0, 0);
-      __builtin_amdgcn_raw_ptr_buffer_load_lds(rsB, (__attribute__((address_space(3))) void*)(dst + 1024), 16, voB1, so + rowB8, 0, 0);
-      if constexpr (NA == 3)
-        __builtin_amdgcn_raw_ptr_buffer_load_lds(rsB, (__attribute__((address_space(3))) void*)(dst + 2048), 16, voB1, so + 2 * rowB8, 0, 0);
-    } else {
-      __builtin_amdgcn_raw_ptr_buffer_load_lds(rsB, (__attribute__((address_space(3))) void*)dst, 16, voB2, so, 0, 0);
-      __builtin_amdgcn_raw_ptr_buffer_load_lds(rsB, (__attribute__((address_space(3))) void*)(dst + 1024), 16, voB2, so + rowB8, 0, 0);
-    }
-    ++u_issue;
-  };
-  auto young_instr = [&](int n) {
-    const int k1 = ((u_issue + 2) >> 2) - ((u_issue - n + 2) >> 2);
-    return 2 * n + (NA - 2) * k1;
-  };
-#define DG_IC(v) std::integral_constant<int, v>()
-
-  const int sw = lane & 7;
-  const int rdo0 = fr * 128 + ((kg ^ sw) << 4);
-  const int rdo1 = fr * 128 + (((4 + kg) ^ sw) << 4);
-  const int a_row0 = wr * 64;
-
-  bf16x8 Af[1][2][4];
-  bf16x8 Bf0[2][NA], Bf1[2][2];
-  f32x4 acc0[2][4][NA], acc1[2][4][2];
-#pragma unroll
-  for (int i = 0; i < 2; ++i)
-#pragma unroll
-    for (int p = 0; p < 4; ++p) {
-#pragma unroll
-      for (int q = 0; q < NA; ++q) acc0[i][p][q] = f32x4{0, 0, 0, 0};
-#pragma unroll
-      for (int q = 0; q < 2; ++q) acc1[i][p][q] = f32x4{0, 0, 0, 0};
-    }
-  int rt_hi = (a.M - m0 - wr * 128 + 15) >> 4;
-  rt_hi = rt_hi < 0 ? 0 : (rt_hi > 8 ? 8 : rt_hi);
-  const int live_mask = __builtin_amdgcn_readfirstlane((rt_hi > 0 ? 1 : 0) | (rt_hi > 4 ? 2 : 0));
-
-  auto readA = [&](int mh, int unit) {
-    const char* base = lds + ((unit >> 2) & 1) * GE::KT + GE::unit_off(mh ? 3 : 0) + a_row0 * 128;
-#pragma unroll
-    for (int mi = 0; mi < 4; ++mi) {
-      Af[0][0][mi] = *(const bf16x8*)(base + mi * 2048 + rdo0);
-      Af[0][1][mi] = *(const bf16x8*)(base + mi * 2048 + rdo1);
-    }
-  };
-  auto readB = [&](int nh, int unit) {
-    if (nh == 0) {
-      const char* base = lds + ((unit >> 2) & 1) * GE::KT + GE::unit_off(1) + wc * (16 * NA) * 128;
-#pragma unroll
-      for (int ni = 0; ni < NA; ++ni) {
-        Bf0[0][ni] = *(const bf16x8*)(base + ni * 2048 + rdo0);
-        Bf0[1][ni] = *(const bf16x8*)(base + ni * 2048 + rdo1);
-      }
-    } else {
-      const char* base = lds + ((unit >> 2) & 1) * GE::KT + GE::unit_off(2) + wc * 32 * 128;
-#pragma unroll
-      for (int ni = 0; ni < 2; ++ni) {
-        Bf1[0][ni] = *(const bf16x8*)(base + ni * 2048 + rdo0);
-        Bf1[1][ni] = *(const bf16x8*)(base + ni * 2048 + rdo1);
-      }
-    }
-  };
-  auto mma = [&](int mh, int nh, auto kind_c) {
-    asm volatile("s_waitcnt lgkmcnt(0)" ::: "memory");
-    __builtin_amdgcn_sched_barrier(0);
-    if (live_mask & (mh ? 2 : 1)) {
-#pragma unroll
-    for (int ks = 0; ks < 2; ++ks) {
-#pragma unroll
-      for (int mi = 0; mi < 4; ++mi) {
-        if (nh == 0) {
-#pragma unroll
-          for (int ni = 0; ni < NA; ++ni)
-            acc0[mh][mi][ni] = __builtin_amdgcn_mfma_f32_16x16x32_bf16(Bf0[ks][ni], Af[0][ks][mi], acc0[mh][mi][ni], 0, 0, 0);
-        } else {
-#pragma unroll
-          for (int ni = 0; ni < 2; ++ni)
-            acc1[mh][mi][ni] = __builtin_amdgcn_mfma_f32_16x16x32_bf16(Bf1[ks][ni], Af[0][ks][mi], acc1[mh][mi][ni], 0, 0, 0);
-        }
-      }
-    }
-    }
-    __builtin_amdgcn_sched_barrier(0);
-  };
-
-  int g = 0;
-  auto wait_landed = [&]() {
-    int need = g + 2;
-    need = need < nunits - 1 ? need : nunits - 1;
-    const int ok = (u_issue - 1) - need;
-    if (ok == DG_D - 2) dg_wait_imm<GE::INFLIGHT>();
-    else dg_wait_vmcnt(ok > 0 ? young_instr(ok) : 0);
-  };
-
-#define DG_PRO(i) if constexpr ((i) < DG_D) { if (u_issue < nunits) issue_unit(DG_IC((i) & 3)); }
-  DG_PRO(0) DG_PRO(1) DG_PRO(2) DG_PRO(3) DG_PRO(4) DG_PRO(5) DG_PRO(6) DG_PRO(7) DG_PRO(8) DG_PRO(9)
-#undef DG_PRO
-  {
-    const int ok = (u_issue - 1) - 1;
-    dg_wait_vmcnt(ok > 0 ? young_instr(ok) : 0);
-  }
-  if (hi) __builtin_amdgcn_s_barrier();
-  DGT2(1);
-
-  auto ktile = [&](int t, auto steady_c) {
-    constexpr bool STEADY = decltype(steady_c)::value != 0;
-    const int u0 = 4 * t;
-    auto dma = [&](auto kind_c) {
-      if (STEADY || u_issue < nunits) issue_unit(kind_c);
-    };
-    auto landed = [&]() {
-      if constexpr (STEADY) dg_wait_imm<GE::INFLIGHT>();
-      else wait_landed();
-    };
-#define DG_RP(x) do { __builtin_amdgcn_s_setprio(x); } while (0)
-#define DG_R(q, reads) do { DG_RP(2); dma(DG_IC(((q) + DG_D) & 3)); reads; DG_RP(0); } while (0)
-    __builtin_amdgcn_s_barrier();
-    DGT();
-    DG_R(0, readA(0, u0); readB(0, u0 + 1));
-    if (hi) landed();
-    DGT();
-    __builtin_amdgcn_s_barrier();
-    DGT();
-    mma(0, 0, DG_IC((0 + DG_D) & 3));
-    DGT();
-    if (!hi) landed();
-    ++g;
-    __builtin_amdgcn_s_barrier();
-    DGT();
-    DG_R(1, readB(1, u0 + 2));
-    if (hi) landed();
-    DGT();
-    __builtin_amdgcn_s_barrier();
-    DGT();
-    mma(0, 1, DG_IC((1 + DG_D) & 3));
-    DGT();
-    if (!hi) landed();
-    ++g;
-    __builtin_amdgcn_s_barrier();
-    DGT();
-    DG_R(2, readA(1, u0 + 3));
-    if (hi) landed();
-    DGT();
-    __builtin_amdgcn_s_barrier();
-    DGT();
-    mma(1, 1, DG_IC((2 + DG_D) & 3));
-    DGT();
-    if (!hi) landed();
-    ++g;
-    __builtin_amdgcn_s_barrier();
-    DGT();
-    DG_R(3, (void)0);
-    if (hi) landed();
-    DGT();
-    __builtin_amdgcn_s_barrier();
-    DGT();
-    mma(1, 0, DG_IC((3 + DG_D) & 3));
-    DGT();
-    if (!hi) landed();
-    ++g;
-#undef DG_R
-#undef DG_RP
-  };
-  const int t_steady = (nunits - 4 - DG_D) >= 0 ? (nunits - 4 - DG_D) / 4 + 1 : 0;
-  int t = 0;
-#pragma unroll 1
-  for (; t < t_steady; ++t) ktile(t, DG_IC(1));
-#pragma unroll 1
-  for (; t < nkt; ++t) ktile(t, DG_IC(0));
-  if (!hi) __builtin_amdgcn_s_barrier();
-  __builtin_amdgcn_s_barrier();
-  DGT2(2);
-
-  const int rt_lo = 0;
-  auto ACC = [&](int mh, int mi, int j) -> f32x4& { return j < NA ? acc0[mh][mi][j] : acc1[mh][mi][j - NA]; };
-  if (rem_idx >= 0 && a.split > 1) {
-    float* slab = a.slabs + ((int64_t)rem_idx * a.split + part) * (DG_BM * DG_BN);
-    f32x4* sw4 = (f32x4*)slab + (int64_t)wid * (8 * NT) * 64 + lane;
-#pragma unroll
-    for (int mh = 0; mh < 2; ++mh)
-#pragma unroll
-      for (int mi = 0; mi < 4; ++mi) {
-        if (mh * 4 + mi >= rt_hi) continue;
-#pragma unroll
-        for (int j = 0; j < NT; ++j) sw4[((mh * 4 + mi) * NT + j) * 64] = ACC(mh, mi, j);
-      }
-    asm volatile("s_waitcnt vmcnt(0)" ::: "memory");
-    __syncthreads();
-    DGT2(5);
-    int* flag = (int*)lds;
-    if (threadIdx.x == 0) {
-      __builtin_amdgcn_fence(__ATOMIC_RELEASE, "agent");
-      asm volatile("s_waitcnt vmcnt(0)" ::: "memory");
-      const int old = __hip_atomic_fetch_add(a.tickets + rem_idx, 1, __ATOMIC_RELAXED, __HIP_MEMORY_SCOPE_AGENT);
-      flag[0] = (old == a.split - 1) ? 1 : 0;
-      if (old == a.split - 1) {
-        __builtin_amdgcn_fence(__ATOMIC_ACQUIRE, "agent");
-        asm volatile("s_waitcnt vmcnt(0)" ::: "memory");
-        __hip_atomic_store(a.tickets + rem_idx, 0, __ATOMIC_RELAXED, __HIP_MEMORY_SCOPE_AGENT);
-      }
-    }
-    __syncthreads();
-    const int last = flag[0];
-    __syncthreads();
-    if (last == 0) return;
-    DGT2(6);
-    for (int p = 0; p < a.split; ++p) {
-      const f32x4* o4 = (const f32x4*)(a.slabs + ((int64_t)rem_idx * a.split + p) * (DG_BM * DG_BN)) +
-                        (int64_t)wid * (8 * NT) * 64 + lane;
-#pragma unroll
-      for (int mh = 0; mh < 2; ++mh)
-#pragma unroll
-        for (int mi = 0; mi < 4; ++mi) {
-          if (mh * 4 + mi >= rt_hi) continue;
-#pragma unroll
-          for (int j = 0; j < NT; ++j) {
-            const f32x4 o = o4[((mh * 4 + mi) * NT + j) * 64];
-            ACC(mh, mi, j) = p == 0 ? o : ACC(mh, mi, j) + o;
-          }
-        }
-    }
-  }
-
-  if constexpr (NT != 4) {
-    constexpr int SRS = GE::SRS;
-    char* const stg = lds + wid * (GE::EPI_ROWS * SRS);
-    const int er = lane / 10, ech = lane - er * 10;
-    const int n = n0 + wc * GE::WCOLS + ech * 8;
-    const bool nok = n < a.N && lane < 60;
-#pragma unroll
-    for (int mh = 0; mh < 2; ++mh) {
-      if (mh * 4 >= rt_hi) break;
-#pragma unroll
-      for (int j = 0; j < NT; ++j) {
-        const int nl = j * 16 + kg * 4;
-        const int nb = n0 + wc * GE::WCOLS + nl;
-        f32x4 bv = {0, 0, 0, 0};
-        if (a.bias && nb < a.N) bv = *(const f32x4*)(a.bias + nb);
-#pragma unroll
-        for (int mi = 0; mi < 4; ++mi) {
-          if (mh * 4 + mi >= rt_hi) continue;
-          const f32x4 v = ACC(mh, mi, j) + bv;
-          const bf16x4 cb = {(bf16)v[0], (bf16)v[1], (bf16)v[2], (bf16)v[3]};
-          *(bf16x4*)(stg + (mi * 16 + fr) * SRS + nl * 2) = cb;
-        }
-      }
-      asm volatile("s_waitcnt lgkmcnt(0)" ::: "memory");
-#pragma unroll
-      for (int it = 0; it < 11; ++it) {
-        const int row = it * 6 + er;
-        const int m = m0 + wr * 128 + mh * 64 + row;
-        if (row >= 64 || m >= a.M || !nok || mh * 4 + (row >> 4) >= rt_hi) continue;
-        const u32x4 raw = *(const u32x4*)(stg + row * SRS + ech * 16);
-        *(u32x4*)(a.C + (int64_t)m * a.ldc + n) = raw;
-      }
-    }
+  dense_nt_tile<MODE, NT, SKIP>(a, lds, tile, kt_begin, kt_end, part, rem_idx, dead_item);
+}
+
+__global__ __launch_bounds__(512, 1) void dense_nt_adaptive_kernel(DgArgs a) {
+  extern __shared__ __attribute__((aligned(16))) char lds[];
+  static_assert(DgGeom<4>::LDS <= DgGeom<5>::LDS, "the bitmap sits behind the wider tile's ring");
+  dg_trace_start();
+  unsigned long long* const live_bm = (unsigned long long*)(lds + DgGeom<5>::LDS);
+  dg_build_bitmap(a, live_bm);
+  bool narrow, dead_item;
+  int tile;
+  dense_item_adaptive(a.tiles_m, a.tiles_n, a.tiles_n_narrow, a.cus, a.narrow_force, blockIdx.x, live_bm, narrow, tile, dead_item);
+  narrow = __builtin_amdgcn_readfirstlane((int)narrow) != 0;
+  tile = __builtin_amdgcn_readfirstlane(tile);
+  dead_item = __builtin_amdgcn_readfirstlane((int)dead_item) != 0;
+  if (tile < 0) return;
+  const int nkt_all = a.K / DG_BK;
+  if (narrow) {
+    DgArgs b = a;
+    b.tiles_n = a.tiles_n_narrow;
+    dense_nt_tile<DG_PLAIN, 4, true>(b, lds, tile, 0, nkt_all, 0, -1, dead_item);
   } else {
-  constexpr int SRS = GE::SRS;
-  char* const stg = lds + wid * (128 * SRS);
-#pragma unroll
-  for (int j = 0; j < NT; ++j) {
-      const int nl = j * 16 + kg * 4;
-      const int n = n0 + wc * 64 + nl;
-      f32x4 bv = {0, 0, 0, 0};
-      if (a.bias && n < a.N) bv = *(const f32x4*)(a.bias + n);
-#pragma unroll
-      for (int mh = 0; mh < 2; ++mh)
-#pragma unroll
-        for (int mi = 0; mi < 4; ++mi) {
-          if (mh * 4 + mi < rt_lo || mh * 4 + mi >= rt_hi) continue;
-          const f32x4 v = ACC(mh, mi, j) + bv;
-          const bf16x4 cb = {(bf16)v[0], (bf16)v[1], (bf16)v[2], (bf16)v[3]};
-          *(bf16x4*)(stg + (mh * 64 + mi * 16 + fr) * SRS + nl * 2) = cb;
-        }
-    }
-  asm volatile("s_waitcnt lgkmcnt(0)" ::: "memory");
-  const int srow = lane >> 3, sch = lane & 7;
-  const int n = n0 + wc * 64 + sch * 8;
-  const bool nok = n < a.N;
-  f32x4 gm0 = {1, 1, 1, 1}, gm1 = {1, 1, 1, 1};
-  if (MODE == DG_RESID && a.gamma && nok) {
-    gm0 = *(const f32x4*)(a.gamma + n);
-    gm1 = *(const f32x4*)(a.gamma + n + 4);
-  }
-  f32x4 xin[MODE == DG_RESID ? 16 : 1][2];
-  bf16x8 hin[(MODE == DG_DGELU || MODE == DG_DFACT) ? 16 : 1];
-  float csum[8] = {0, 0, 0, 0, 0, 0, 0, 0};
-  if (MODE == DG_RESID || MODE == DG_DGELU || MODE == DG_DFACT) {
-#pragma unroll
-    for (int it = 0; it < 16; ++it) {
-      const int m = m0 + wr * 128 + it * 8 + srow;
-      const bool ok = m < a.M && nok && (it >> 1) >= rt_lo && (it >> 1) < rt_hi;
-      if (MODE == DG_RESID) {
-        const float* xp = a.X + (int64_t)(ok ? m : 0) * a.N + (ok ? n : 0);
-        xin[it][0] = *(const f32x4*)xp;
-        xin[it][1] = *(const f32x4*)(xp + 4);
-      } else {
-        hin[it] = *(const bf16x8*)(a.H + (int64_t)(ok ? m : 0) * a.ldc + (ok ? n : 0));
-      }
-    }
-  }
-#pragma unroll
-  for (int it = 0; it < 16; ++it) {
-    const int row = it * 8 + srow;
-    const int m = m0 + wr * 128 + row;
-    if (m >= a.M || !nok || (it >> 1) < rt_lo || (it >> 1) >= rt_hi) continue;
-    const u32x4 raw = *(const u32x4*)(stg + row * SRS + sch * 16);
-    const bf16x8 cb = __builtin_bit_cast(bf16x8, raw);
-    bf16* cp = a.C + (int64_t)m * a.ldc + n;
-    if (MODE == DG_PLAIN) {
-      *(u32x4*)cp = raw;
-    } else if (MODE == DG_GELU) {
-      *(u32x4*)cp = raw;
-      bf16x8 y;
-#pragma unroll
-      for (int e = 0; e < 8; ++e) y[e] = (bf16)dg_gelu((float)cb[e]);
-      *(bf16x8*)(a.C2 + (int64_t)m * a.ldc + n) = y;
-    } else if (MODE == DG_GELUO) {
-      bf16x8 y;
-#pragma unroll
-      for (int e = 0; e < 8; ++e) y[e] = (bf16)dg_gelu((float)cb[e]);
-      *(bf16x8*)cp = y;
-    } else if (MODE == DG_GELUF) {
-      bf16x8 y, f;
-#pragma unroll
-      for (int e = 0; e < 8; ++e) {
-        float gv, dv;
-        dg_gelu_both((float)cb[e], gv, dv);
-        y[e] = (bf16)gv;
-        f[e] = (bf16)dv;
-      }
-      *(bf16x8*)cp = f;
-      *(bf16x8*)(a.C2 + (int64_t)m * a.ldc + n) = y;
-    } else if (MODE == DG_RESID) {
-      *(u32x4*)cp = raw;
-      const float rsv = a.rs ? a.rs[m / a.rps] : 1.0f;
-      f32x4 x0 = xin[it][0], x1 = xin[it][1];
-#pragma unroll
-      for (int e = 0; e < 4; ++e) {
-        x0[e] += rsv * gm0[e] * (float)cb[e];
-        x1[e] += rsv * gm1[e] * (float)cb[4 + e];
-      }
-      float* op = a.OUT + (int64_t)m * a.N + n;
-      *(f32x4*)op = x0;
-      *(f32x4*)(op + 4) = x1;
-    } else {
-      const bf16x8 h = hin[it];
-      bf16x8 d;
-#pragma unroll
-      for (int e = 0; e < 8; ++e) {
-        d[e] = (bf16)((MODE == DG_DFACT ? (float)h[e] : dg_gelu_grad((float)h[e])) * (float)cb[e]);
-        csum[e] += (float)d[e];
-      }
-      *(bf16x8*)cp = d;
-    }
-  }
-  if ((MODE == DG_DGELU || MODE == DG_DFACT) && a.colsum != nullptr) {
-#pragma unroll
-    for (int e = 0; e < 8; ++e) {
-      float v = csum[e];
-      v += __shfl_xor(v, 8, 64);
-      v += __shfl_xor(v, 16, 64);
-      v += __shfl_xor(v, 32, 64);
-      csum[e] = v;
-    }
-    if (srow == 0 && nok) {
-      float* base = a.colsum + (int64_t)(tm * 2 + wr) * a.N + n;
-      *(f32x4*)base = f32x4{csum[0], csum[1], csum[2], csum[3]};
-      *(f32x4*)(base + 4) = f32x4{csum[4], csum[5], csum[6], csum[7]};
-    }
-  }
-  }
-#ifdef DG_TRACE2
-  DGT2(3);
-  asm volatile("s_waitcnt vmcnt(0)" ::: "memory");
-  DGT2(4);
-#endif
+    dense_nt_tile<DG_PLAIN, 5, true>(a, lds, tile, 0, nkt_all, 0, -1, dead_item);
+  }
 }
 
 template <int MODE>
@@ -931,7 +1001,7 @@
 
 constexpr int DG_TICKET_BYTES = 8192;
 
-static inline int dense_force_nt() { const int v = route(OCTIC_ROUTE_DENSE_TILE); return (v == 4 || v == 5) ? v : 0; }
+static inline int dense_force_nt() { const int v = route(OCTIC_ROUTE_DENSE_TILE) & 15; return (v == 4 || v == 5) ? v : 0; }
 static inline int dense_force_split() { const int v = route(OCTIC_ROUTE_DENSE_SPLIT); return v > 0 ? v : 0; }
 
 inline DgPlan dense_plan(int M, int N, int K, int cus, int mode) {
@@ -982,6 +1052,21 @@
   return t;
 }
 
+struct DgAdaptive { bool eligible; int tiles_n_narrow, grid, max_live, force; };
+inline DgAdaptive dense_plan_adaptive(const DgTokPlan& tp, int N, int mode, int cus, bool masked) {
+  DgAdaptive d;
+  const DgPlan& p = tp.p;
+  d.tiles_n_narrow = (N % 256) == 0 ? N / 256 : 0;
+  d.max_live = d.tiles_n_narrow > 0 ? cus / d.tiles_n_narrow : -1;
+  const int f = (route(OCTIC_ROUTE_DENSE_TILE) >> 4) & 3;
+  d.force = f == 1 || f == 2 ? f : 0;
+  d.eligible = masked && mode == DG_PLAIN && tp.image && p.nt == 5 && p.rem == 0 && p.tail_pad == 0 && p.split == 1 &&
+               p.full <= cus && d.tiles_n_narrow > 0 && p.tiles_m <= kDgMaskCap;
+  const int narrow_tiles = p.tiles_m * d.tiles_n_narrow;
+  d.grid = d.eligible && narrow_tiles > p.grid ? narrow_tiles : p.grid;
+  return d;
+}
+
 }
 
 using namespace octic;
@@ -1032,10 +1117,10 @@
   return 2 * ((M + DG_BM - 1) / DG_BM);
 }
 
-int octic_dense_gemm_nt_tokens_skip(const void* A, const void* B, int M, int N, int K, int64_t lda, int64_t ldb, int mode, void* C,
-                                    void* C2, int64_t ldc, const float* bias, const float* gamma, const float* rs, int64_t rps,
-                                    const float* X, float* OUT, const void* H, float* colsum, const float* sample_scale,
-                                    int rows_per_sample, void* workspace, int tokens, void* stream) {
+static int dense_launch(const void* A, const void* B, int M, int N, int K, int64_t lda, int64_t ldb, int mode, void* C,
+                        void* C2, int64_t ldc, const float* bias, const float* gamma, const float* rs, int64_t rps,
+                        const float* X, float* OUT, const void* H, float* colsum, const float* sample_scale,
+                        int rows_per_sample, void* workspace, int tokens, void* stream, bool adaptive) {
   if (!A || !B || !C) return OCTIC_ENULL;
   if (sample_scale && (rows_per_sample <= 0 || M <= 0 || (M % rows_per_sample) != 0)) return OCTIC_ESHAPE;
   if (sample_scale && (((uintptr_t)sample_scale) & 3)) return OCTIC_EALIGN;
@@ -1082,8 +1167,16 @@
     (void)hipFuncSetAttribute((const void*)dense_nt_kernel<DG_GELUF, 4, true>, hipFuncAttributeMaxDynamicSharedMemorySize, smem + bmb);
     (void)hipFuncSetAttribute((const void*)dense_nt_kernel<DG_DFACT, 4, true>, hipFuncAttributeMaxDynamicSharedMemorySize, smem + bmb);
     (void)hipFuncSetAttribute((const void*)dense_nt_kernel<DG_GELUO, 4, true>, hipFuncAttributeMaxDynamicSharedMemorySize, smem + bmb);
+    (void)hipFuncSetAttribute((const void*)dense_nt_adaptive_kernel, hipFuncAttributeMaxDynamicSharedMemorySize, smem5 + bmb);
     (void)hipGetLastError();
   }
+  const DgAdaptive ad = dense_plan_adaptive(tp, N, mode, dense_cus(), skip);
+  if (adaptive && ad.eligible) {
+    a.tiles_n_narrow = ad.tiles_n_narrow;
+    a.cus = dense_cus();
+    a.narrow_force = ad.force;
+    dense_nt_adaptive_kernel<<<ad.grid, 512, smem5 + bmb, s>>>(a);
+  } else
   if (skip) {
     switch (mode) {
       case DG_PLAIN:
@@ -1131,6 +1224,22 @@
     }
   }
   return launch_status();
+}
+
+int octic_dense_gemm_nt_tokens_skip(const void* A, const void* B, int M, int N, int K, int64_t lda, int64_t ldb, int mode, void* C,
+                                    void* C2, int64_t ldc, const float* bias, const float* gamma, const float* rs, int64_t rps,
+                                    const float* X, float* OUT, const void* H, float* colsum, const float* sample_scale,
+                                    int rows_per_sample, void* workspace, int tokens, void* stream) {
+  return dense_launch(A, B, M, N, K, lda, ldb, mode, C, C2, ldc, bias, gamma, rs, rps, X, OUT, H, colsum, sample_scale,
+                      rows_per_sample, workspace, tokens, stream, false);
+}
+
+int octic_dense_gemm_nt_tokens_adaptive(const void* A, const void* B, int M, int N, int K, int64_t lda, int64_t ldb, int mode,
+                                        void* C, void* C2, int64_t ldc, const float* bias, const float* gamma, const float* rs,
+                                        int64_t rps, const float* X, float* OUT, const void* H, float* colsum,
+                                        const float* sample_scale, int rows_per_sample, void* workspace, int tokens, void* stream) {
+  return dense_launch(A, B, M, N, K, lda, ldb, mode, C, C2, ldc, bias, gamma, rs, rps, X, OUT, H, colsum, sample_scale,
+                      rows_per_sample, workspace, tokens, stream, true);
 }
 
 int octic_dense_gemm_nt_tokens(const void* A, const void* B, int M, int N, int K, int64_t lda, int64_t ldb, int mode, void* C,
@@ -1171,6 +1280,44 @@
   return p.grid;
 }
 
+int octic_dense_gemm_plan_adaptive(int M, int N, int K, int mode, int tokens, int rows_per_sample, int* out) {
+  if (!out) return OCTIC_ENULL;
+  if (rows_per_sample <= 0 || M <= 0 || (M % rows_per_sample) != 0 || N <= 0 || K < 2 * DG_BK) return OCTIC_ESHAPE;
+  const DgTokPlan tp = dense_plan_tokens(M, N, K, dense_cus(), mode, tokens);
+  const DgAdaptive ad = dense_plan_adaptive(tp, N, mode, dense_cus(), mode != DG_RESID);
+  out[0] = ad.eligible ? 1 : 0;
+  out[1] = ad.grid;
+  out[2] = 320;
+  out[3] = 256;
+  out[4] = ad.max_live;
+  return OCTIC_OK;
+}
+
+int octic_dense_gemm_order_adaptive(int M, int N, int K, int mode, int tokens, const float* sample_scale, int rows_per_sample,
+                                    int cap, int* out_tm, int* out_tn, int* out_dead, int* out_width) {
+  if (!sample_scale) return OCTIC_ENULL;
+  if (M <= 0 || N <= 0 || K < 2 * DG_BK || rows_per_sample <= 0 || (M % rows_per_sample) != 0) return OCTIC_ESHAPE;
+  const DgTokPlan tp = dense_plan_tokens(M, N, K, dense_cus(), mode, tokens);
+  const DgPlan p = tp.p;
+  const DgAdaptive ad = dense_plan_adaptive(tp, N, mode, dense_cus(), true);
+  if (!ad.eligible || cap < ad.grid) return OCTIC_ESHAPE;
+  unsigned long long bm[kDgMaskWords] = {};
+  for (int tm = 0; tm < p.tiles_m; ++tm)
+    if (dg_panel_live(sample_scale, rows_per_sample, M, tokens, 1, tm)) bm[tm >> 6] |= 1ull << (tm & 63);
+  bool narrow = false;
+  for (int bid = 0; bid < ad.grid; ++bid) {
+    int tile, tm = -1, tn = -1;
+    bool dead;
+    dense_item_adaptive(p.tiles_m, p.tiles_n, ad.tiles_n_narrow, dense_cus(), ad.force, bid, bm, narrow, tile, dead);
+    if (tile >= 0) dg_tile_panel(p.tiles_m, narrow ? ad.tiles_n_narrow : p.tiles_n, tile, tm, tn);
+    if (out_tm) out_tm[bid] = tm;
+    if (out_tn) out_tn[bid] = tn;
+    if (out_dead) out_dead[bid] = dead ? 1 : 0;
+  }
+  if (out_width) *out_width = narrow ? 256 : 320;
+  return ad.grid;
+}
+
 int octic_dense_gemm_nt(const void* A, const void* B, int M, int N, int K, int64_t lda, int64_t ldb, int mode, void* C,
                         void* C2, int64_t ldc, const float* bias, const float* gamma, const float* rs, int64_t rps,
                         const float* X, float* OUT, const void* H, float* colsum, void* workspace, void* stream) {
diff --git a/octic_vits_amd/functional.py b/octic_vits_amd/functional.py
--- a/octic_vits_amd/functional.py
+++ b/octic_vits_amd/functional.py
@@ -417,6 +417,9 @@
 DENSE_NT_SKIP_DROPPED = _skip_from_env("OCTIC_DENSE_SKIP")
 
 
+DENSE_NARROW_DROPPED = _skip_from_env("OCTIC_DENSE_NARROW")
+
+
 def dense_skip_scale(rs, rps, M, rows_to=None):
     return whole_sample_mask(rs, rps, M, rows_to) if DENSE_NT_SKIP_DROPPED else None
 
diff --git a/octic_vits_amd/ops.py b/octic_vits_amd/ops.py
--- a/octic_vits_amd/ops.py
+++ b/octic_vits_amd/ops.py
@@ -1118,6 +1118,17 @@
     return out[0], out[1], bool(out[2]), out[3]
 
 
+def dense_plan_adaptive(M, N, K, mode, tokens, rows_per_sample):
+    out = (ctypes.c_int * 5)()
+    check(lib().octic_dense_gemm_plan_adaptive(M, N, K, mode, int(tokens), int(rows_per_sample), out))
+    return bool(out[0]), out[1], out[2], out[3], out[4]
+
+
+def _dense_narrow():
+    from . import functional
+    return functional.DENSE_NARROW_DROPPED
+
+
 def dense_gemm_nt(a, b, mode=0, bias=None, gamma=None, rs=None, rps=1, x=None, h=None, name=None, want_colsum=False,
                   tokens=0, sample_scale=None, rows_per_sample=0):
     _require_cuda(a)
@@ -1135,10 +1146,10 @@
     ss, srps = _sample_scale(sample_scale, rows_per_sample, M, a, "dense_gemm_nt")
     cs_rows = dense_plan(M, N, K, mode, tokens)[1] if (mode in (3, 5) and want_colsum) else 0
     cs = torch.empty((cs_rows, N), dtype=torch.float32, device=a.device) if cs_rows else None
-    t = KERNEL_TIMER.start()
-    check(lib().octic_dense_gemm_nt_tokens_skip(_p(a), _p(b), M, N, K, a.stride(0), b.stride(0), mode, _p(c), _p(c2), N, _p(bias),
-                                                _p(gamma), _p(rs), int(rps), _p(x), _p(out), _p(h), _p(cs), _p(ss), srps,
-                                                _p(ws), tokens, _stream(a)))
+    entry = lib().octic_dense_gemm_nt_tokens_adaptive if (ss is not None and _dense_narrow()) else lib().octic_dense_gemm_nt_tokens_skip
+    t = KERNEL_TIMER.start()
+    check(entry(_p(a), _p(b), M, N, K, a.stride(0), b.stride(0), mode, _p(c), _p(c2), N, _p(bias), _p(gamma), _p(rs), int(rps),
+                _p(x), _p(out), _p(h), _p(cs), _p(ss), srps, _p(ws), tokens, _stream(a)))
     if t is not None:
         nb = 2 * (M * K + N * K + M * N * (2 if mode in (1, 3, 4, 5) else 1)) + (8 * M * N if mode == 2 else 0)
         wide = "@320" if dense_plan(M, N, K, mode, tokens)[0] == 320 else ""
```

New measurement: 1219 images/s (median of 6 runs). 1.02x the previous value.
